# intel-aero/aero-optical-flow

Measured on AMD Instinct MI355X. Metric: frame-pairs/s (640x480, 8x8 SAD, +-4 search), higher is better.
Workload: dtype u8

## Files before the change

aero-optical-flow_amd/__init__.py:

```python
from __future__ import annotations

import ctypes as C
import os

import numpy as np

_HERE = os.path.dirname(os.path.abspath(__file__))
LIB_PATH = os.environ.get("AOF_LIB") or os.path.join(_HERE, "csrc", "libaof.so")

GRID_DENSE, GRID_PX4FLOW = 0, 1
SEARCH_EXHAUSTIVE, SEARCH_PRUNED, SEARCH_ADAPTIVE = 0, 1, 2
SAD_SKIPPED = 0xFFFF
FLAG_FLOW_VALID, FLAG_PRED_VALID = 1, 2
K_PYRAMID, K_SEARCH_L1, K_REDUCE_L1, K_SEARCH, K_REDUCE = range(5)

BLOCK_DTYPE = np.dtype([("dx", "i1"), ("dy", "i1"), ("sad", "<u2")])
FLOW_DTYPE = np.dtype([("flow_x", "<f4"), ("flow_y", "<f4"), ("count", "<u4"), ("quality", "u1"),
                       ("flags", "u1"), ("pred_x", "i1"), ("pred_y", "i1")])
assert BLOCK_DTYPE.itemsize == 4 and FLOW_DTYPE.itemsize == 16


class Params(C.Structure):
    _fields_ = [(n, C.c_int32) for n in (
        "width", "height", "tile", "search", "grid_mode", "num_blocks", "feature_threshold",
        "value_threshold", "subpixel", "hist_filter", "pyramid_levels", "mean_subtract",
        "min_valid")]

    def as_dict(self):
        return {n: getattr(self, n) for n, _ in self._fields_}


class IngestParams(C.Structure):
    _fields_ = [(n, C.c_int32) for n in ("camera_width", "camera_height", "crop_width", "crop_height")]


class DerotateParams(C.Structure):
    _fields_ = [(n, C.c_float) for n in ("focal_x", "focal_y", "max_flow", "rate_threshold")]


GYRO_DTYPE = np.dtype([("integ_x", "<f4"), ("integ_y", "<f4"), ("integ_z", "<f4"), ("dt_s", "<f4")])


class SequenceParams(C.Structure):
    _fields_ = [("ingest", IngestParams), ("focal_x", C.c_float), ("focal_y", C.c_float),
                ("output_rate", C.c_int32), ("offset_timestamp_usec", C.c_uint64),
                ("system_id", C.c_uint8), ("component_id", C.c_uint8), ("first_seq", C.c_uint8),
                ("derotate", C.c_uint8), ("derotate_params", DerotateParams)]


class SeqLayout(C.Structure):
    _fields_ = [(n, C.c_size_t) for n in ("total_bytes", "cropped", "exposure", "flows", "derotated", "count",
                                          "records", "frames", "frame_len", "scratch")]


SEQ_RECORD_DTYPE = np.dtype([("frame", "<u4"), ("quality", "<i4"), ("dt_us", "<i4"), ("flow_x", "<f4"),
                             ("flow_y", "<f4"), ("gyro_x", "<f4"), ("gyro_y", "<f4"), ("gyro_z", "<f4")])
SEQ_FRAME_BYTES = 56
SEQ_STATUS_STALLED = 1
assert SEQ_RECORD_DTYPE.itemsize == 32


class BankParams(C.Structure):
    _fields_ = [("n_streams", C.c_int32), ("frame_stride", C.c_int64), ("focal_x", C.c_float), ("focal_y", C.c_float),
                ("output_rate", C.c_int32), ("offset_timestamp_usec", C.c_uint64),
                ("system_id", C.c_uint8), ("component_id", C.c_uint8), ("first_seq", C.c_uint8)]


class BankStream(C.Structure):
    _fields_ = [("focal_x", C.c_float), ("focal_y", C.c_float), ("output_rate", C.c_int32),
                ("system_id", C.c_uint8), ("component_id", C.c_uint8), ("first_seq", C.c_uint8), ("reserved0", C.c_uint8),
                ("offset_timestamp_usec", C.c_uint64), ("reserved1", C.c_uint64)]


BANK_STREAM_DTYPE = np.dtype([("focal_x", "<f4"), ("focal_y", "<f4"), ("output_rate", "<i4"), ("system_id", "u1"),
                              ("component_id", "u1"), ("first_seq", "u1"), ("reserved0", "u1"),
                              ("offset_timestamp_usec", "<u8"), ("reserved1", "<u8")])
assert BANK_STREAM_DTYPE.itemsize == 32 and C.sizeof(BankStream) == 32


class BankSensor(C.Structure):
    _fields_ = [("offset", C.c_uint64), ("pitch", C.c_int32), ("width", C.c_int32), ("height", C.c_int32),
                ("x0", C.c_int32), ("y0", C.c_int32), ("reserved", C.c_uint32)]


BANK_SENSOR_DTYPE = np.dtype([("offset", "<u8"), ("pitch", "<i4"), ("width", "<i4"), ("height", "<i4"), ("x0", "<i4"),
                              ("y0", "<i4"), ("reserved", "<u4")])
assert BANK_SENSOR_DTYPE.itemsize == 32 and C.sizeof(BankSensor) == 32


class BankLayout(C.Structure):
    _fields_ = [(n, C.c_size_t) for n in ("total_bytes", "frames", "state", "scratch")]


class BankCamera(C.Structure):
    _fields_ = [("ingest", IngestParams), ("camera_stride", C.c_int64), ("exposure_interval_us", C.c_uint32),
                ("derotate", C.c_uint8), ("derotate_params", DerotateParams)]


class BankBurst(C.Structure):
    _fields_ = [("n_rounds", C.c_int32), ("round_stride", C.c_int64)]


BANK_BURST_MAX = 16
TICK_HELD, TICK_IDLE = -1, -2
BANK_BIN_MAX = 4
PIXEL_GREY8, PIXEL_LUMA16_LO, PIXEL_LUMA16_HI = 0, 1, 2
TICK_BAD_SENSOR = -5
TICK_DTYPE = np.dtype([("quality", "<i4"), ("dt_us", "<i4"), ("flow_x", "<f4"), ("flow_y", "<f4"),
                       ("gyro_x", "<f4"), ("gyro_y", "<f4"), ("gyro_z", "<f4"), ("frame", "<u4"), ("pixel", FLOW_DTYPE)])
BANK_STATE_BYTES = 64
EXPOSURE_DTYPE = np.dtype([("hist", "<u4", (10,)), ("msv", "<f4"), ("due", "<u4")])
assert TICK_DTYPE.itemsize == 48 and EXPOSURE_DTYPE.itemsize == 48


class ExposureControl(C.Structure):
    _fields_ = [(n, C.c_float) for n in ("msv_target", "exposure_p", "exposure_i", "exposure_d", "gain_p", "gain_i", "gain_d",
                                         "exposure_change_threshold", "exposure_max", "gain_change_threshold", "gain_max")]


EXPOSURE_UPDATED, EXPOSURE_SET_EXPOSURE, EXPOSURE_SET_GAIN = 1, 2, 4
EXPOSURE_STATE_DTYPE = np.dtype([("msv_error_old", "<f4"), ("msv_error_int", "<f4"), ("exposure", "<u2"), ("gain", "u1"),
                                 ("reserved", "u1"), ("updates", "<u4")])
EXPOSURE_COMMAND_DTYPE = np.dtype([("exposure", "<u2"), ("gain", "u1"), ("flags", "u1"), ("msv_error", "<f4"),
                                   ("msv_error_int", "<f4"), ("update", "<u4")])
assert EXPOSURE_STATE_DTYPE.itemsize == 16 and EXPOSURE_COMMAND_DTYPE.itemsize == 16


class ImuParams(C.Structure):
    _fields_ = [("n_streams", C.c_int32), ("n_rounds", C.c_int32), ("max_samples", C.c_int32),
                ("system_id", C.c_uint8), ("component_id", C.c_uint8), ("first_seq", C.c_uint8)]


IMU_SLOTS_MAX = 16
TICK_STALE_GYRO, TICK_NO_OFFSET = -3, -4
IMU_SAMPLE_DTYPE = np.dtype([("time_usec", "<u8"), ("xgyro", "<f4"), ("ygyro", "<f4"), ("zgyro", "<f4"),
                             ("reserved", "<u4")])
IMU_STATE_DTYPE = np.dtype([("gyro_x", "<f8"), ("gyro_y", "<f8"), ("gyro_z", "<f8"), ("prev_time_usec", "<u8"),
                            ("last_taken_time_usec", "<u8"), ("offset_timestamp_usec", "<u8"), ("messages", "<u4"),
                            ("samples_integrated", "<u4"), ("samples_rejected", "<u4"), ("dropped", "<u4")])
assert IMU_SAMPLE_DTYPE.itemsize == 24 and IMU_STATE_DTYPE.itemsize == 64


class MavlinkRxParams(C.Structure):
    _fields_ = [("n_streams", C.c_int32), ("n_rounds", C.c_int32), ("max_bytes", C.c_int32), ("max_samples", C.c_int32)]


MAVLINK_RX_BYTES_MAX = 4096
MAVLINK_RX_STATE_DTYPE = np.dtype([("bytes", "<u8"), ("frames", "<u4"), ("imu_samples", "<u4"), ("bad_check", "<u4"),
                                   ("overflowed", "<u4"), ("skipped", "<u4"), ("rejected_flags", "<u4"),
                                   ("in_progress", "u1", (96,))])
assert MAVLINK_RX_STATE_DTYPE.itemsize == 128


class OutboxLayout(C.Structure):
    _fields_ = [(n, C.c_size_t) for n in ("total_bytes", "messages", "exposures")]


OUTBOX_HEADER_DTYPE = np.dtype([("tag", "<u8"), ("n_messages", "<u4"), ("messages_found", "<u4"), ("n_exposures", "<u4"),
                                ("exposures_found", "<u4"), ("reserved", "u1", (40,))])
OUTBOX_ENTRY_DTYPE = np.dtype([("stream", "<u4"), ("round", "<u2"), ("mavlink_len", "u1"), ("reserved0", "u1"),
                               ("mavlink", "u1", (SEQ_FRAME_BYTES,)), ("record", TICK_DTYPE), ("derotated", "<f4", (2,)),
                               ("reserved1", "u1", (8,))])
OUTBOX_EXPOSURE_DTYPE = np.dtype([("stream", "<u4"), ("round", "<u2"), ("reserved0", "<u2"), ("exposure", EXPOSURE_DTYPE),
                                  ("reserved1", "u1", (8,))])
assert OUTBOX_HEADER_DTYPE.itemsize == 64 and OUTBOX_ENTRY_DTYPE.itemsize == 128 and OUTBOX_EXPOSURE_DTYPE.itemsize == 64


class WsLayout(C.Structure):
    _fields_ = [(n, C.c_size_t) for n in (
        "total_bytes", "sums", "l1_prev", "l1_cur", "l1_blocks", "l1_subdirs", "l1_flows",
        "l0_blocks", "l0_subdirs", "l0_hist", "l1_hist", "hints")]


class StreamStats(C.Structure):
    _fields_ = [("calls", C.c_uint64), ("resident_served", C.c_uint64), ("resident_launches", C.c_uint32),
                ("resident_fallbacks", C.c_uint32), ("resident_lost", C.c_uint32), ("tagged_slow", C.c_uint32),
                ("launch_call_us_max", C.c_float), ("start_latency_us_max", C.c_float),
                ("last_report", C.c_char * 320)]

    def as_dict(self):
        d = {n: getattr(self, n) for n, _ in self._fields_}
        d["last_report"] = d["last_report"].decode(errors="replace")
        return d


class SearchStats(C.Structure):
    _fields_ = [("pruned_launches", C.c_uint64), ("exhaustive_launches", C.c_uint64), ("reports_read", C.c_uint64),
                ("belief", C.c_int32), ("paying_pct", C.c_int32)]

    def as_dict(self):
        return {n: getattr(self, n) for n, _ in self._fields_}


class AofError(RuntimeError):
    def __init__(self, code, text):
        super().__init__(f"aof error {code}: {text}")
        self.code = code


def _load():
    if not os.path.exists(LIB_PATH):
        raise ImportError(
            f"{LIB_PATH} is missing: run `python -c 'import __graft_entry__ as g; g.build()'` "
            "(hipcc --offload-arch=gfx950). There is no CPU fallback.")
    try:
        import torch
    except Exception:
        pass
    lib = C.CDLL(LIB_PATH)
    P, VP, I64 = C.POINTER, C.c_void_p, C.c_int64
    sig = {
        "aof_version": (C.c_int, []),
        "aof_strerror": (C.c_char_p, [C.c_int]),
        "aof_params_default": (C.c_int, [P(Params), C.c_int, C.c_int]),
        "aof_params_px4flow": (C.c_int, [P(Params), C.c_int, C.c_int, C.c_int, C.c_int, C.c_int]),
        "aof_params_check": (C.c_int, [P(Params)]),
        "aof_grid": (C.c_int, [P(Params), C.c_int] + [P(C.c_int32)] * 6),
        "aof_workspace_layout": (C.c_int, [P(Params), I64, P(WsLayout)]),
        "aof_create": (C.c_int, [P(Params), C.c_int, P(VP)]),
        "aof_destroy": (None, [VP]),
        "aof_last_error": (C.c_char_p, [VP]),
        "aof_get_params": (C.c_int, [VP, P(Params)]),
        "aof_search_variant": (C.c_char_p, [VP]),
        "aof_set_force_generic": (C.c_int, [VP, C.c_int]),
        "aof_set_search_mode": (C.c_int, [VP, C.c_int]),
        "aof_get_search_mode": (C.c_int, [VP]),
        "aof_get_search_stats": (C.c_int, [VP, VP]),
        "aof_set_search_belief": (C.c_int, [VP, C.c_int]),
        "aof_set_split_coarse": (C.c_int, [VP, C.c_int]),
        "aof_set_reduce_fusion": (C.c_int, [VP, C.c_int]),
        "aof_flow_batch_device": (C.c_int, [VP, VP, VP, I64, I64, VP, VP, VP, VP, C.c_size_t, VP]),
        "aof_flow_pair_host": (C.c_int, [VP, VP, VP, VP, VP, VP]),
        "aof_stream_push_host": (C.c_int, [VP, VP, VP]),
        "aof_stream_reset": (C.c_int, [VP]),
        "aof_set_stream_graph": (C.c_int, [VP, C.c_int]),
        "aof_set_stream_resident": (C.c_int, [VP, C.c_int]),
        "aof_stream_get_stats": (C.c_int, [VP, P(StreamStats)]),
        "aof_debug_resident_fault": (C.c_int, [VP, C.c_int, C.c_uint32]),
        "aof_set_vote_deadline_us": (C.c_int, [VP, C.c_uint32]),
        "aof_debug_vote_deadline_ticks": (C.c_int, [VP, C.c_uint32]),
        "aof_debug_tile16_verdicts": (C.c_int, [VP, VP, C.c_int]),
        "aof_ingest_batch_device": (C.c_int, [P(IngestParams), VP, I64, I64, VP, I64, VP, VP]),
        "aof_sequence_layout": (C.c_int, [P(Params), P(SequenceParams), I64, P(SeqLayout)]),
        "aof_sequence_device": (C.c_int, [VP, P(SequenceParams), VP, I64, I64, VP, VP, VP, C.c_size_t, VP]),
        "aof_flow_angle": (C.c_float, [C.c_float, C.c_float]),
        "aof_bank_layout": (C.c_int, [P(Params), P(BankParams), P(BankLayout)]),
        "aof_bank_reset_device": (C.c_int, [VP, P(BankParams), VP, VP, C.c_size_t, VP]),
        "aof_bank_push_device": (C.c_int, [VP, P(BankParams), VP, VP, VP, VP, VP, C.c_size_t, VP, VP, VP, VP]),
        "aof_set_bank_path": (C.c_int, [VP, C.c_int]),
        "aof_bank_stream_from_params": (C.c_int, [P(BankParams), P(BankStream)]),
        "aof_set_bank_streams": (C.c_int, [VP, VP, C.c_int32]),
        "aof_set_bank_sensors": (C.c_int, [VP, VP, C.c_int32, C.c_uint64]),
        "aof_bank_sensor_from_camera": (C.c_int, [P(Params), P(BankCamera), C.c_int32, P(BankSensor)]),
        "aof_bank_sensor_centred": (C.c_int, [P(Params), C.c_uint64, C.c_int32, C.c_int32, C.c_int32, P(BankSensor)]),
        "aof_bank_sensor_valid": (C.c_int, [P(BankSensor), C.c_int32, C.c_int32, C.c_uint64, C.c_uint64]),
        "aof_ingest_sensors_device": (C.c_int, [C.c_int32, C.c_int32, VP, C.c_uint64, VP, I64, VP, I64, VP, VP, VP]),
        "aof_set_bank_pixel_formats": (C.c_int, [VP, VP, C.c_int32]),
        "aof_bank_sensor_valid_format": (C.c_int, [P(BankSensor), C.c_uint8, C.c_int32, C.c_int32, C.c_uint64, C.c_uint64]),
        "aof_ingest_sensor_formats_device": (C.c_int, [C.c_int32, C.c_int32, VP, C.c_uint64, VP, VP, I64, VP, I64, VP, VP, VP]),
        "aof_set_bank_binning": (C.c_int, [VP, VP, C.c_int32]),
        "aof_bank_sensor_valid_binned": (C.c_int, [P(BankSensor), C.c_uint8, C.c_uint8, C.c_int32, C.c_int32, C.c_uint64, C.c_uint64]),
        "aof_bank_sensor_centred_binned": (C.c_int, [P(Params), C.c_uint64, C.c_int32, C.c_int32, C.c_int32, C.c_uint8, C.c_uint8,
                                                     P(BankSensor)]),
        "aof_ingest_sensors_binned_device": (C.c_int, [C.c_int32, C.c_int32, VP, C.c_uint64, VP, VP, VP, I64, VP, I64, VP, VP, VP]),
        "aof_bank_camera_layout": (C.c_int, [P(Params), P(BankParams), P(BankCamera), P(BankLayout), P(C.c_size_t)]),
        "aof_bank_push_camera_device": (C.c_int, [VP, P(BankParams), P(BankCamera), VP, VP, VP, VP, VP, C.c_size_t, VP, VP, VP,
                                                  VP, VP, VP]),
        "aof_bank_push_burst_device": (C.c_int, [VP, P(BankParams), P(BankBurst), VP, VP, VP, VP, VP, C.c_size_t, VP, VP, VP, VP]),
        "aof_bank_push_camera_burst_device": (C.c_int, [VP, P(BankParams), P(BankCamera), P(BankBurst), VP, VP, VP, VP, VP,
                                                        C.c_size_t, VP, VP, VP, VP, VP, VP]),
        "aof_outbox_layout": (C.c_int, [C.c_uint32, C.c_uint32, P(OutboxLayout)]),
        "aof_bank_collect_device": (C.c_int, [VP, C.c_int32, C.c_int32, VP, VP, VP, VP, VP, C.c_uint32, C.c_uint32, VP,
                                              C.c_size_t, C.c_uint64, VP, VP]),
        "aof_outbox_alloc_host": (C.c_int, [C.c_size_t, P(VP)]),
        "aof_outbox_free_host": (C.c_int, [VP]),
        "aof_exposure_control_default": (C.c_int, [P(ExposureControl)]),
        "aof_bank_exposure_reset_device": (C.c_int, [VP, C.c_int32, VP, C.c_uint16, C.c_uint8, VP, VP, VP, VP]),
        "aof_bank_exposure_control_device": (C.c_int, [VP, P(ExposureControl), C.c_int32, C.c_int32, VP, VP, VP, VP]),
        "aof_exposure_control_host": (C.c_int, [P(ExposureControl), C.c_int32, C.c_int32, VP, VP, VP]),
        "aof_bank_imu_reset_device": (C.c_int, [VP, C.c_int32, VP, C.c_uint64, VP, VP]),
        "aof_bank_imu_device": (C.c_int, [VP, P(ImuParams), VP, VP, VP, VP, VP, VP, VP, VP, VP]),
        "aof_bank_imu_host": (C.c_int, [P(ImuParams), VP, VP, VP, VP, VP, VP, VP, VP]),
        "aof_bank_mavlink_rx_reset_device": (C.c_int, [VP, C.c_int32, VP, VP, VP]),
        "aof_bank_mavlink_rx_device": (C.c_int, [VP, P(MavlinkRxParams), VP, VP, VP, VP, VP, VP]),
        "aof_bank_mavlink_rx_host": (C.c_int, [P(MavlinkRxParams), VP, VP, VP, VP, VP]),
        "aof_derotate_batch_device": (C.c_int, [P(DerotateParams), VP, VP, I64, VP, VP]),
        "aof_exposure_msv": (C.c_float, [VP]),
        "aof_exposure_bin": (C.c_int, [C.c_int]),
        "aof_set_profiling": (C.c_int, [VP, C.c_int]),
        "aof_set_profiling_mask": (C.c_int, [VP, C.c_uint32]),
        "aof_kernel_ms": (C.c_int, [VP, C.c_int, P(C.c_float)]),
        "aof_profile_count": (C.c_int, [VP, C.c_int]),
        "aof_profile_ms": (C.c_int, [VP, C.c_int, C.c_int, P(C.c_float)]),
    }
    for name, (res, args) in sig.items():
        try:
            fn = getattr(lib, name)
        except AttributeError:
            if os.environ.get("AOF_LIB"):
                continue
            raise
        fn.restype, fn.argtypes = res, args
    return lib, tuple(sig)


lib, EXPORTS = _load()


def default_params(width, height, **overrides) -> Params:
    p = Params()
    lib.aof_params_default(C.byref(p), width, height)
    for k, v in overrides.items():
        if not hasattr(p, k):
            raise AttributeError(k)
        setattr(p, k, int(v))
    return p


def px4flow_params(width, height, search=4, feature_threshold=30, value_threshold=3000,
                   **overrides) -> Params:
    p = Params()
    lib.aof_params_px4flow(C.byref(p), width, height, search, feature_threshold, value_threshold)
    for k, v in overrides.items():
        setattr(p, k, int(v))
    return p


def check_params(p: Params) -> int:
    return lib.aof_params_check(C.byref(p))


def grid(p: Params, level=0):
    v = [C.c_int32() for _ in range(6)]
    rc = lib.aof_grid(C.byref(p), level, *[C.byref(x) for x in v])
    if rc:
        raise AofError(rc, lib.aof_strerror(rc).decode())
    return tuple(x.value for x in v)


def workspace_layout(p: Params, n_pairs: int) -> WsLayout:
    L = WsLayout()
    rc = lib.aof_workspace_layout(C.byref(p), n_pairs, C.byref(L))
    if rc:
        raise AofError(rc, lib.aof_strerror(rc).decode())
    return L


def algorithmic_bytes(p: Params) -> int:
    _, _, _, _, nx, ny = grid(p, 0)
    return 2 * p.width * p.height + 4 * nx * ny + 16


def abs_diffs(p: Params) -> int:
    _, _, _, _, nx, ny = grid(p, 0)
    return nx * ny * (2 * p.search + 1) ** 2 * p.tile ** 2


def ingest_batch(camera, crop_w, crop_h, cropped=None, hist=None, want_hist=True):
    import torch
    n, cam_h, cam_w = camera.shape
    p = IngestParams(cam_w, cam_h, crop_w, crop_h)
    if cropped is None:
        cropped = torch.empty((n, crop_h, crop_w), dtype=torch.uint8, device=camera.device)
    if hist is None and want_hist:
        hist = torch.empty((n, 10), dtype=torch.int32, device=camera.device)
    stream = torch.cuda.current_stream(camera.device).cuda_stream
    rc = lib.aof_ingest_batch_device(C.byref(p), camera.data_ptr(), camera.stride(0), n,
                                     cropped.data_ptr(), cropped.stride(0) if n else crop_w * crop_h,
                                     hist.data_ptr() if hist is not None else None, stream)
    if rc:
        raise AofError(rc, lib.aof_strerror(rc).decode())
    return cropped, hist


def derotate_batch(flows, gyro, focal_x, focal_y, max_flow, rate_threshold):
    import torch
    n = flows.shape[0]
    out = torch.empty((n, 2), dtype=torch.float32, device=flows.device)
    p = DerotateParams(focal_x, focal_y, max_flow, rate_threshold)
    rc = lib.aof_derotate_batch_device(C.byref(p), flows.data_ptr(), gyro.data_ptr(), n, out.data_ptr(),
                                       torch.cuda.current_stream(flows.device).cuda_stream)
    if rc:
        raise AofError(rc, lib.aof_strerror(rc).decode())
    return out


def flow_angle(flow_px: float, focal_px: float) -> float:
    return float(lib.aof_flow_angle(flow_px, focal_px))


def sequence_params(cam_w, cam_h, crop_w, crop_h, focal_x=216.6677, focal_y=216.2457, output_rate=15,
                    offset_timestamp_usec=0, system_id=1, component_id=100, first_seq=0, derotate=None) -> SequenceParams:
    sp = SequenceParams()
    sp.ingest = IngestParams(cam_w, cam_h, crop_w, crop_h)
    sp.focal_x, sp.focal_y, sp.output_rate = focal_x, focal_y, output_rate
    sp.offset_timestamp_usec = offset_timestamp_usec
    sp.system_id, sp.component_id, sp.first_seq = system_id, component_id, first_seq & 0xFF
    sp.derotate = 0 if derotate is None else 1
    if derotate is not None:
        sp.derotate_params = DerotateParams(focal_x, focal_y, derotate[0], derotate[1])
    return sp


def sequence_layout(p: Params, sp: SequenceParams, n_frames: int) -> SeqLayout:
    L = SeqLayout()
    rc = lib.aof_sequence_layout(C.byref(p), C.byref(sp), n_frames, C.byref(L))
    if rc:
        raise AofError(rc, lib.aof_strerror(rc).decode())
    return L


def bank_params(n_streams, focal_x=216.6677, focal_y=216.2457, output_rate=15, offset_timestamp_usec=0, system_id=1,
                component_id=100, first_seq=0, frame_stride=0) -> BankParams:
    bp = BankParams()
    bp.n_streams, bp.frame_stride = n_streams, frame_stride
    bp.focal_x, bp.focal_y, bp.output_rate = focal_x, focal_y, output_rate
    bp.offset_timestamp_usec = offset_timestamp_usec
    bp.system_id, bp.component_id, bp.first_seq = system_id, component_id, first_seq & 0xFF
    return bp


def bank_stream_from_params(bp: BankParams, n=None):
    rec = BankStream()
    rc = lib.aof_bank_stream_from_params(C.byref(bp), C.byref(rec))
    if rc:
        raise AofError(rc, lib.aof_strerror(rc).decode())
    one = np.frombuffer(bytes(rec), dtype=BANK_STREAM_DTYPE)[0]
    return one if n is None else np.full(int(n), one, dtype=BANK_STREAM_DTYPE)


def _sensor_record(rec: BankSensor):
    return np.frombuffer(bytes(rec), dtype=BANK_SENSOR_DTYPE)[0]


def bank_sensor_from_camera(p: Params, cam: BankCamera, stream=None, n=None):
    def one(s):
        rec = BankSensor()
        rc = lib.aof_bank_sensor_from_camera(C.byref(p), C.byref(cam), int(s), C.byref(rec))
        if rc:
            raise AofError(rc, lib.aof_strerror(rc).decode())
        return _sensor_record(rec)
    if n is None:
        return one(stream or 0)
    return np.array([one(s) for s in range(int(n))], dtype=BANK_SENSOR_DTYPE)


def bank_sensor_centred(p: Params, offset, pitch, width, height, format=0, bin=1):
    rec = BankSensor()
    if format == 0 and bin == 1:
        rc = lib.aof_bank_sensor_centred(C.byref(p), int(offset), int(pitch), int(width), int(height), C.byref(rec))
    else:
        rc = lib.aof_bank_sensor_centred_binned(C.byref(p), int(offset), int(pitch), int(width), int(height), int(format) & 0xFF,
                                                int(bin) & 0xFF, C.byref(rec))
    if rc:
        raise AofError(rc, lib.aof_strerror(rc).decode())
    return _sensor_record(rec)


def bank_sensor_valid(rec, crop_w, crop_h, camera_bytes, base=0, format=0, bin=1) -> bool:
    r = BankSensor.from_buffer_copy(np.asarray(rec, dtype=BANK_SENSOR_DTYPE).tobytes())
    if bin != 1:
        rc = lib.aof_bank_sensor_valid_binned(C.byref(r), int(format) & 0xFF, int(bin) & 0xFF, int(crop_w), int(crop_h), int(base),
                                              int(camera_bytes))
    elif format == 0:
        rc = lib.aof_bank_sensor_valid(C.byref(r), int(crop_w), int(crop_h), int(base), int(camera_bytes))
    else:
        rc = lib.aof_bank_sensor_valid_format(C.byref(r), int(format) & 0xFF, int(crop_w), int(crop_h), int(base), int(camera_bytes))
    if rc < 0:
        raise AofError(rc, lib.aof_strerror(rc).decode())
    return bool(rc)


def ingest_sensors(camera, sensors, crop_w, crop_h, camera_bytes=None, cropped=None, hist=None, ok=None, want_cropped=True,
                   want_hist=True, want_ok=True, formats=None, bins=None):
    import torch
    assert camera.dtype == torch.uint8 and sensors.dtype == torch.uint8 and sensors.is_contiguous() and sensors.numel() % 32 == 0
    n = sensors.numel() // 32
    assert formats is None or (formats.dtype == torch.uint8 and formats.is_contiguous() and formats.numel() == n)
    assert bins is None or (bins.dtype == torch.uint8 and bins.is_contiguous() and bins.numel() == n)
    dev = camera.device
    if cropped is None and want_cropped:
        cropped = torch.empty((n, crop_h, crop_w), dtype=torch.uint8, device=dev)
    if hist is None and want_hist:
        hist = torch.empty((n, 10), dtype=torch.int32, device=dev)
    if ok is None and want_ok:
        ok = torch.empty((n,), dtype=torch.uint8, device=dev)
    opt = lambda t: t.data_ptr() if t is not None else None
    tail = (n, opt(cropped), cropped.stride(0) if cropped is not None and n else crop_w * crop_h, opt(hist), opt(ok),
            torch.cuda.current_stream(dev).cuda_stream)
    head = (int(crop_w), int(crop_h), camera.data_ptr(), camera.numel() if camera_bytes is None else int(camera_bytes), sensors.data_ptr())
    if bins is not None:
        rc = lib.aof_ingest_sensors_binned_device(*head, opt(formats), bins.data_ptr(), *tail)
    elif formats is None:
        rc = lib.aof_ingest_sensors_device(*head, *tail)
    else:
        rc = lib.aof_ingest_sensor_formats_device(*head, formats.data_ptr(), *tail)
    if rc:
        raise AofError(rc, lib.aof_strerror(rc).decode())
    return cropped, hist, ok


def bank_layout(p: Params, bp: BankParams) -> BankLayout:
    L = BankLayout()
    rc = lib.aof_bank_layout(C.byref(p), C.byref(bp), C.byref(L))
    if rc:
        raise AofError(rc, lib.aof_strerror(rc).decode())
    return L


def bank_camera_params(cam_w, cam_h, crop_w, crop_h, camera_stride=0, exposure_interval_us=200000, derotate=None,
                       focal_x=216.6677, focal_y=216.2457) -> BankCamera:
    cam = BankCamera()
    cam.ingest = IngestParams(cam_w, cam_h, crop_w, crop_h)
    cam.camera_stride, cam.exposure_interval_us = camera_stride, exposure_interval_us
    cam.derotate = 0 if derotate is None else 1
    if derotate is not None:
        cam.derotate_params = DerotateParams(focal_x, focal_y, derotate[0], derotate[1])
    return cam


def bank_burst_params(n_rounds, round_stride=0) -> BankBurst:
    b = BankBurst()
    b.n_rounds, b.round_stride = int(n_rounds), int(round_stride)
    return b


def bank_camera_layout(p: Params, bp: BankParams, cam: BankCamera):
    L, staging = BankLayout(), C.c_size_t()
    rc = lib.aof_bank_camera_layout(C.byref(p), C.byref(bp), C.byref(cam), C.byref(L), C.byref(staging))
    if rc:
        raise AofError(rc, lib.aof_strerror(rc).decode())
    return L, staging.value


def outbox_layout(capacity_messages, capacity_exposures=0) -> OutboxLayout:
    L = OutboxLayout()
    rc = lib.aof_outbox_layout(capacity_messages, capacity_exposures, C.byref(L))
    if rc:
        raise AofError(rc, lib.aof_strerror(rc).decode())
    return L


def outbox_view(buffer, capacity_messages=None, capacity_exposures=0):
    if isinstance(buffer, HostOutbox):
        capacity_messages, capacity_exposures, a = buffer.capacity_messages, buffer.capacity_exposures, buffer.array
    else:
        a = buffer.cpu().numpy() if hasattr(buffer, "cpu") else np.asarray(buffer)
        a = np.ascontiguousarray(a).reshape(-1).view(np.uint8)
    if capacity_messages is None:
        capacity_messages = (a.size - 64 - 64 * capacity_exposures) // 128
    L = outbox_layout(capacity_messages, capacity_exposures)
    assert a.size >= L.total_bytes, (a.size, L.total_bytes)
    header = a[:64].view(OUTBOX_HEADER_DTYPE).reshape(())
    messages = a[L.messages:L.messages + 128 * capacity_messages].view(OUTBOX_ENTRY_DTYPE)[:int(header["n_messages"])]
    exposures = a[L.exposures:L.exposures + 64 * capacity_exposures].view(OUTBOX_EXPOSURE_DTYPE)[:int(header["n_exposures"])]
    return header, messages, exposures


class HostOutbox:

    def __init__(self, capacity_messages, capacity_exposures=0):
        self.capacity_messages, self.capacity_exposures = int(capacity_messages), int(capacity_exposures)
        self.layout = outbox_layout(self.capacity_messages, self.capacity_exposures)
        self.nbytes = self.layout.total_bytes
        p = C.c_void_p()
        rc = lib.aof_outbox_alloc_host(self.nbytes, C.byref(p))
        if rc:
            raise AofError(rc, "aof_outbox_alloc_host failed")
        self.ptr = p.value
        self.array = np.frombuffer((C.c_uint8 * self.nbytes).from_address(self.ptr), dtype=np.uint8)
        self._tag = self.array[:8].view("<u8")

    @property
    def tag(self) -> int:
        return int(self._tag[0])

    def wait(self, tag, timeout_s=2.0) -> bool:
        import time
        deadline = time.perf_counter() + timeout_s
        tagword, tag = self._tag, int(tag)
        while int(tagword[0]) != tag:
            if time.perf_counter() > deadline:
                return False
        return True

    def close(self):
        if getattr(self, "ptr", None) and lib is not None:
            self.array = self._tag = None
            lib.aof_outbox_free_host(self.ptr)
            self.ptr = None

    __del__ = close


def exposure_control_default() -> ExposureControl:
    ec = ExposureControl()
    rc = lib.aof_exposure_control_default(C.byref(ec))
    if rc:
        raise AofError(rc, lib.aof_strerror(rc).decode())
    return ec


def exposure_control_host(records, states, ec: ExposureControl = None):
    ec = exposure_control_default() if ec is None else ec
    records = np.ascontiguousarray(records, dtype=EXPOSURE_DTYPE)
    assert records.ndim in (1, 2)
    K, S = (1, records.shape[0]) if records.ndim == 1 else records.shape
    assert states.dtype == EXPOSURE_STATE_DTYPE and states.shape == (S,) and states.flags.c_contiguous and states.flags.writeable
    commands = np.empty(records.shape, EXPOSURE_COMMAND_DTYPE)
    rc = lib.aof_exposure_control_host(C.byref(ec), S, K, records.ctypes.data, states.ctypes.data, commands.ctypes.data)
    if rc:
        raise AofError(rc, lib.aof_strerror(rc).decode())
    return commands


def imu_params(n_streams, n_rounds, max_samples, system_id=1, component_id=100, first_seq=0) -> ImuParams:
    ip = ImuParams()
    ip.n_streams, ip.n_rounds, ip.max_samples = int(n_streams), int(n_rounds), int(max_samples)
    ip.system_id, ip.component_id, ip.first_seq = int(system_id), int(component_id), int(first_seq)
    return ip


def bank_imu_host(samples, counts, times, records, states, system_id=1, component_id=100, first_seq=0, mavlink=True,
                  records_out=None, fill=0):
    samples = np.ascontiguousarray(samples, dtype=IMU_SAMPLE_DTYPE)
    K, M, S = samples.shape
    times = np.ascontiguousarray(times, dtype=np.uint64)
    assert records.dtype == TICK_DTYPE and records.shape == (K, S) and records.flags.c_contiguous and times.shape == (K, S)
    assert states.dtype == IMU_STATE_DTYPE and states.shape == (S,) and states.flags.c_contiguous and states.flags.writeable
    if counts is not None:
        counts = np.ascontiguousarray(counts, dtype=np.uint8)
        assert counts.shape == (K, S)
    if records_out is None:
        records_out = np.empty((K, S), TICK_DTYPE)
    assert records_out.dtype == TICK_DTYPE and records_out.shape == (K, S) and records_out.flags.c_contiguous
    frames = np.full((K, S, SEQ_FRAME_BYTES), fill, np.uint8) if mavlink else None
    lengths = np.full((K, S), fill, np.uint8) if mavlink else None
    ip = imu_params(S, K, M, system_id, component_id, first_seq)
    rc = lib.aof_bank_imu_host(C.byref(ip), samples.ctypes.data, counts.ctypes.data if counts is not None else None,
                               times.ctypes.data, records.ctypes.data, states.ctypes.data, records_out.ctypes.data,
                               frames.ctypes.data if mavlink else None, lengths.ctypes.data if mavlink else None)
    if rc:
        raise AofError(rc, lib.aof_strerror(rc).decode())
    return records_out, frames, lengths


def imu_states_view(t) -> np.ndarray:
    a = t.cpu().numpy() if hasattr(t, "cpu") else np.asarray(t)
    return np.ascontiguousarray(a).view(IMU_STATE_DTYPE).reshape(a.shape[:-1])


def mavlink_rx_params(n_streams, n_rounds, max_bytes, max_samples) -> MavlinkRxParams:
    rp = MavlinkRxParams()
    rp.n_streams, rp.n_rounds, rp.max_bytes, rp.max_samples = int(n_streams), int(n_rounds), int(max_bytes), int(max_samples)
    return rp


def _aligned_copy(a, align=16):
    raw = np.empty(a.size + align, np.uint8)
    off = -raw.ctypes.data % align
    out = raw[off:off + a.size].reshape(a.shape)
    out[...] = a
    return out


def bank_mavlink_rx_host(data, lengths, states, max_samples, samples=None, counts=None):
    data = np.ascontiguousarray(data, dtype=np.uint8)
    K, S, B = data.shape
    M = int(max_samples)
    if data.ctypes.data % 16:
        data = _aligned_copy(data)
    if lengths is not None:
        lengths = np.ascontiguousarray(lengths, dtype=np.uint16)
        assert lengths.shape == (K, S)
    assert states.dtype == MAVLINK_RX_STATE_DTYPE and states.shape == (S,) and states.flags.c_contiguous and states.flags.writeable
    if samples is None:
        samples = np.zeros((K, M, S), IMU_SAMPLE_DTYPE)
    if counts is None:
        counts = np.zeros((K, S), np.uint8)
    assert samples.dtype == IMU_SAMPLE_DTYPE and samples.shape == (K, M, S) and samples.flags.c_contiguous
    assert counts.dtype == np.uint8 and counts.shape == (K, S) and counts.flags.c_contiguous
    rp = mavlink_rx_params(S, K, B, M)
    rc = lib.aof_bank_mavlink_rx_host(C.byref(rp), data.ctypes.data, lengths.ctypes.data if lengths is not None else None,
                                      states.ctypes.data, samples.ctypes.data, counts.ctypes.data)
    if rc:
        raise AofError(rc, lib.aof_strerror(rc).decode())
    return samples, counts


def mavlink_rx_states_view(t) -> np.ndarray:
    a = t.cpu().numpy() if hasattr(t, "cpu") else np.asarray(t)
    return np.ascontiguousarray(a).view(MAVLINK_RX_STATE_DTYPE).reshape(a.shape[:-1])


def exposure_states_view(t) -> np.ndarray:
    a = t.cpu().numpy() if hasattr(t, "cpu") else np.asarray(t)
    return np.ascontiguousarray(a).view(EXPOSURE_STATE_DTYPE).reshape(a.shape[:-1])


def exposure_commands_view(t) -> np.ndarray:
    a = t.cpu().numpy() if hasattr(t, "cpu") else np.asarray(t)
    return np.ascontiguousarray(a).view(EXPOSURE_COMMAND_DTYPE).reshape(a.shape[:-1])


def exposure_view(t) -> np.ndarray:
    a = t.cpu().numpy() if hasattr(t, "cpu") else np.asarray(t)
    return np.ascontiguousarray(a).view(EXPOSURE_DTYPE).reshape(a.shape[0])


def ticks_view(t) -> np.ndarray:
    a = t.cpu().numpy() if hasattr(t, "cpu") else np.asarray(t)
    return np.ascontiguousarray(a).view(TICK_DTYPE).reshape(a.shape[0])


class Bank:

    def __init__(self, bp: BankParams, layout: BankLayout, buffer, camera: BankCamera = None, staging: int = None):
        self.bp, self.layout, self.buffer = bp, layout, buffer
        self.camera, self.staging = camera, staging

    @property
    def n_streams(self) -> int:
        return self.bp.n_streams

    def frames_bytes(self) -> np.ndarray:
        return self.buffer[self.layout.frames:self.layout.state].cpu().numpy()

    def state_bytes(self) -> np.ndarray:
        L = self.layout
        return self.buffer[L.state:L.state + BANK_STATE_BYTES * self.n_streams].cpu().numpy().reshape(self.n_streams, BANK_STATE_BYTES)


def exposure_msv(hist) -> float:
    h = np.ascontiguousarray(np.asarray(hist), dtype=np.uint32)
    assert h.shape == (10,)
    return float(lib.aof_exposure_msv(h.ctypes.data))


class FlowEngine:

    def __init__(self, params: Params, device: int = 0):
        self._ctx = C.c_void_p()
        rc = lib.aof_create(C.byref(params), device, C.byref(self._ctx))
        if rc:
            self._ctx = None
            raise AofError(rc, lib.aof_strerror(rc).decode())
        self.params = params
        self.device = device
        self._ws = None

    def close(self):
        if getattr(self, "_ctx", None) and lib is not None:
            lib.aof_destroy(self._ctx)
            self._ctx = None

    __del__ = close

    def _check(self, rc):
        if rc < 0:
            raise AofError(rc, lib.aof_last_error(self._ctx).decode())
        return rc

    @property
    def variant(self) -> str:
        return lib.aof_search_variant(self._ctx).decode()

    def force_generic(self, on=True):
        self._check(lib.aof_set_force_generic(self._ctx, int(on)))

    def set_search_mode(self, mode):
        self._check(lib.aof_set_search_mode(self._ctx, int(mode)))

    @property
    def search_mode(self) -> int:
        return lib.aof_get_search_mode(self._ctx)

    def search_stats(self) -> dict:
        st = SearchStats()
        self._check(lib.aof_get_search_stats(self._ctx, C.byref(st)))
        return st.as_dict()

    def set_search_belief(self, belief):
        self._check(lib.aof_set_search_belief(self._ctx, int(belief)))

    def set_split_coarse(self, on=True):
        self._check(lib.aof_set_split_coarse(self._ctx, int(on)))

    def set_reduce_fusion(self, on=True):
        if not hasattr(lib, "aof_set_reduce_fusion"):
            return
        self._check(lib.aof_set_reduce_fusion(self._ctx, int(on)))

    def set_profiling(self, on=True, kernels=None):
        if on and kernels is not None:
            mask = 0
            for k in kernels:
                mask |= 1 << k
            self._check(lib.aof_set_profiling_mask(self._ctx, mask))
        else:
            self._check(lib.aof_set_profiling(self._ctx, int(on)))

    def kernel_ms(self, kernel_id) -> float:
        ms = C.c_float()
        self._check(lib.aof_kernel_ms(self._ctx, kernel_id, C.byref(ms)))
        return ms.value

    def profile_ms(self, kernel_id):
        n = self._check(lib.aof_profile_count(self._ctx, kernel_id))
        out = []
        ms = C.c_float()
        for i in range(n):
            self._check(lib.aof_profile_ms(self._ctx, kernel_id, i, C.byref(ms)))
            out.append(ms.value)
        return out

    def grid(self, level=0):
        return grid(self.params, level)

    def nblocks(self, level=0):
        g = self.grid(level)
        return g[4] * g[5]

    def flow_batch(self, prev, cur, blocks=None, subdirs=None, flows=None, workspace=None,
                   pair_stride=None, n_pairs=None):
        import torch
        p = self.params
        if n_pairs is None:
            n_pairs = prev.shape[0]
        if pair_stride is None:
            pair_stride = prev.stride(0) if prev.dim() == 3 else p.width * p.height
        dev = prev.device
        nb = self.nblocks(0)
        if blocks is None:
            blocks = torch.empty((n_pairs, nb), dtype=torch.int32, device=dev)
        if flows is None:
            flows = torch.empty((n_pairs, 16), dtype=torch.uint8, device=dev)
        if subdirs is None and p.subpixel:
            subdirs = torch.empty((n_pairs, nb), dtype=torch.uint8, device=dev)
        L = workspace_layout(p, n_pairs)
        if workspace is None:
            if self._ws is None or self._ws.numel() < L.total_bytes or self._ws.device != dev:
                self._ws = torch.empty(L.total_bytes, dtype=torch.uint8, device=dev)
            workspace = self._ws
        stream = torch.cuda.current_stream(dev).cuda_stream
        self._check(lib.aof_flow_batch_device(
            self._ctx, prev.data_ptr(), cur.data_ptr(), pair_stride, n_pairs, blocks.data_ptr(),
            subdirs.data_ptr() if subdirs is not None else None, flows.data_ptr(),
            workspace.data_ptr(), workspace.numel(), stream))
        return blocks, flows, workspace

    def bind_batch(self, prev, cur, blocks, flows, workspace, subdirs=None, stream=None):
        import torch
        p = self.params
        n_pairs = prev.shape[0]
        stride = prev.stride(0) if prev.dim() == 3 else p.width * p.height
        assert workspace.numel() >= workspace_layout(p, n_pairs).total_bytes
        args = (self._ctx, prev.data_ptr(), cur.data_ptr(), stride, n_pairs, blocks.data_ptr(),
                subdirs.data_ptr() if subdirs is not None else None, flows.data_ptr(),
                workspace.data_ptr(), workspace.numel())
        keep = (prev, cur, blocks, flows, workspace, subdirs)
        fn, dev, current_stream = lib.aof_flow_batch_device, prev.device, torch.cuda.current_stream

        if stream is not None:
            def enqueue():
                rc = fn(*args, stream)
                if rc < 0:
                    self._check(rc)
        else:
            def enqueue():
                rc = fn(*args, current_stream(dev).cuda_stream)
                if rc < 0:
                    self._check(rc)
        enqueue.keep = keep
        return enqueue

    def sequence(self, sp: SequenceParams, camera, time_us, gyro=None, workspace=None):
        import torch
        n = camera.shape[0]
        L = sequence_layout(self.params, sp, n)
        if workspace is None:
            workspace = torch.empty(L.total_bytes, dtype=torch.uint8, device=camera.device)
        assert time_us.dtype == torch.int64 and time_us.numel() == n
        stream = torch.cuda.current_stream(camera.device).cuda_stream
        self._check(lib.aof_sequence_device(self._ctx, C.byref(sp), camera.data_ptr(), camera.stride(0) if n else 0, n,
                                            time_us.data_ptr(), gyro.data_ptr() if gyro is not None else None,
                                            workspace.data_ptr(), workspace.numel(), stream))
        return workspace, L

    def sequence_outputs(self, sp: SequenceParams, workspace, L: SeqLayout, n: int):
        p = self.params
        ws = workspace.cpu().numpy()
        pairs = max(n - 1, 0)
        count = ws[L.count:L.count + 16].view(np.uint32)
        out = {
            "records": ws[L.records:L.records + 32 * int(count[0])].view(SEQ_RECORD_DTYPE),
            "frames_sent": int(count[1]), "status": int(count[2]),
            "cropped": ws[L.cropped:L.cropped + n * p.width * p.height].reshape(n, p.height, p.width),
            "exposure": ws[L.exposure:L.exposure + 40 * n].view(np.uint32).reshape(n, 10),
            "flows": ws[L.flows:L.flows + 16 * pairs].view(FLOW_DTYPE),
            "derotated": ws[L.derotated:L.derotated + 8 * pairs].view(np.float32).reshape(pairs, 2) if sp.derotate else None,
        }
        lens = ws[L.frame_len:L.frame_len + int(count[0])]
        out["mavlink"] = [bytes(ws[L.frames + SEQ_FRAME_BYTES * m:L.frames + SEQ_FRAME_BYTES * m + int(lens[m])])
                          for m in range(int(count[0]))]
        return out

    def bank_create(self, bp: BankParams, device=None, camera: BankCamera = None) -> "Bank":
        import torch
        staging = None
        if camera is None:
            L = bank_layout(self.params, bp)
        else:
            L, staging = bank_camera_layout(self.params, bp, camera)
        dev = torch.device("cuda", self.device) if device is None else device
        bank = Bank(bp, L, torch.zeros(L.total_bytes, dtype=torch.uint8, device=dev), camera, staging)
        self.bank_reset(bank)
        return bank

    def bank_reset(self, bank: "Bank", mask=None):
        import torch
        buf = bank.buffer
        assert mask is None or (mask.dtype == torch.uint8 and mask.numel() == bank.n_streams and mask.is_contiguous())
        self._check(lib.aof_bank_reset_device(self._ctx, C.byref(bank.bp), mask.data_ptr() if mask is not None else None,
                                              buf.data_ptr(), buf.numel(), torch.cuda.current_stream(buf.device).cuda_stream))

    def _bank_push(self, bank, src, times, select, gyro, mavlink, records, out_frames, out_lengths, n_rounds=None,
                   round_stride=0, camera=False, exposure=None, derotated=None, want_exposure=True):
        import torch
        S, buf, cam = bank.n_streams, bank.buffer, bank.camera
        burst = n_rounds is not None
        lead = (int(n_rounds), S) if burst else (S,)
        n = int(n_rounds) * S if burst else S
        dev = buf.device
        if camera:
            assert cam is not None, "bank_create(..., camera=...) makes a bank for sensor frames"
        assert src.dtype == torch.uint8 and (camera or src.is_contiguous())
        assert times.dtype == torch.int64 and times.numel() == n and (not burst or times.is_contiguous())
        if burst:
            assert select is None or (select.dtype == torch.uint8 and select.numel() == S)
            assert gyro is None or gyro.numel() == n * 4
        if records is None:
            records = torch.empty(lead + (48,), dtype=torch.uint8, device=dev)
        if camera and exposure is None and want_exposure:
            exposure = torch.empty(lead + (48,), dtype=torch.uint8, device=dev)
        if camera and derotated is None and cam.derotate:
            derotated = torch.empty(lead + (2,), dtype=torch.float32, device=dev)
        if mavlink:
            if out_frames is None:
                out_frames = torch.zeros(lead + (SEQ_FRAME_BYTES,), dtype=torch.uint8, device=dev)
            if out_lengths is None:
                out_lengths = torch.zeros(lead, dtype=torch.uint8, device=dev)
        else:
            out_frames = out_lengths = None
        opt = lambda t: t.data_ptr() if t is not None else None
        fn = getattr(lib, "aof_bank_push" + ("_camera" if camera else "") + ("_burst" if burst else "") + "_device")
        args = [self._ctx, C.byref(bank.bp)]
        if camera:
            args.append(C.byref(cam))
        if burst:
            args.append(C.byref(bank_burst_params(int(n_rounds), round_stride)))
        args += [src.data_ptr(), times.data_ptr(), opt(select), opt(gyro), buf.data_ptr(), buf.numel(), records.data_ptr()]
        if camera:
            args += [opt(exposure), opt(derotated)]
        self._check(fn(*args, opt(out_frames), opt(out_lengths), torch.cuda.current_stream(dev).cuda_stream))
        return dict(records=records, exposure=exposure, derotated=derotated, frames=out_frames, lengths=out_lengths)

    def bank_push(self, bank: "Bank", frames, times, active=None, gyro=None, mavlink=False, records=None, out_frames=None,
                  out_lengths=None):
        out = self._bank_push(bank, frames, times, active, gyro, mavlink, records, out_frames, out_lengths)
        return (out["records"], out["frames"], out["lengths"]) if mavlink else out["records"]

    def bank_push_camera(self, bank: "Bank", camera, times, active=None, gyro=None, mavlink=False, records=None,
                         exposure=None, derotated=None, out_frames=None, out_lengths=None, want_exposure=True):
        return self._bank_push(bank, camera, times, active, gyro, mavlink, records, out_frames, out_lengths, camera=True,
                               exposure=exposure, derotated=derotated, want_exposure=want_exposure)

    def bank_push_burst(self, bank: "Bank", n_rounds, frames, times, count=None, gyro=None, mavlink=False, records=None,
                        out_frames=None, out_lengths=None, round_stride=0):
        out = self._bank_push(bank, frames, times, count, gyro, mavlink, records, out_frames, out_lengths, n_rounds, round_stride)
        return (out["records"], out["frames"], out["lengths"]) if mavlink else out["records"]

    def bank_push_camera_burst(self, bank: "Bank", n_rounds, camera, times, count=None, gyro=None, mavlink=False,
                               records=None, exposure=None, derotated=None, out_frames=None, out_lengths=None,
                               want_exposure=True, round_stride=0):
        return self._bank_push(bank, camera, times, count, gyro, mavlink, records, out_frames, out_lengths, n_rounds,
                               round_stride, camera=True, exposure=exposure, derotated=derotated, want_exposure=want_exposure)

    def bank_collect(self, records, mavlink=None, lengths=None, exposure=None, derotated=None, capacity_messages=None,
                     capacity_exposures=0, outbox=None, tag=1, tag_tensor=None):
        import torch
        dev = records.device
        assert records.dtype == torch.uint8 and records.is_contiguous() and records.shape[-1] == 48 and records.dim() in (2, 3)
        K, S = (1, records.shape[0]) if records.dim() == 2 else (records.shape[0], records.shape[1])
        n = K * S
        assert mavlink is None or (mavlink.is_contiguous() and mavlink.numel() == n * SEQ_FRAME_BYTES)
        assert lengths is None or (lengths.is_contiguous() and lengths.numel() == n)
        assert exposure is None or (exposure.is_contiguous() and exposure.numel() == n * 48)
        assert derotated is None or (derotated.is_contiguous() and derotated.numel() * derotated.element_size() == n * 8)
        assert tag_tensor is None or (tag_tensor.dtype == torch.int64 and tag_tensor.numel() == 1)
        if capacity_messages is None:
            capacity_messages = outbox.capacity_messages if isinstance(outbox, HostOutbox) else n
        if outbox is None:
            outbox = torch.empty(outbox_layout(capacity_messages, capacity_exposures).total_bytes, dtype=torch.uint8, device=dev)
        ptr, size = (outbox.ptr, outbox.nbytes) if isinstance(outbox, HostOutbox) else (outbox.data_ptr(), outbox.numel())
        opt = lambda t: t.data_ptr() if t is not None else None
        self._check(lib.aof_bank_collect_device(
            self._ctx, S, K, records.data_ptr(), opt(mavlink), opt(lengths), opt(exposure), opt(derotated),
            capacity_messages, capacity_exposures, ptr, size, int(tag), opt(tag_tensor), torch.cuda.current_stream(dev).cuda_stream))
        return outbox

    def bank_exposure_reset(self, state, mask=None, exposure0=1, gain0=1, exposures=None, gains=None):
        import torch
        S = state.numel() // 16
        assert state.dtype == torch.uint8 and state.is_contiguous() and state.numel() == 16 * S
        assert mask is None or (mask.dtype == torch.uint8 and mask.numel() == S and mask.is_contiguous())
        assert exposures is None or (exposures.element_size() == 2 and exposures.numel() == S and exposures.is_contiguous())
        assert gains is None or (gains.dtype == torch.uint8 and gains.numel() == S and gains.is_contiguous())
        opt = lambda t: t.data_ptr() if t is not None else None
        self._check(lib.aof_bank_exposure_reset_device(self._ctx, S, opt(mask), int(exposure0), int(gain0), opt(exposures),
                                                       opt(gains), state.data_ptr(), torch.cuda.current_stream(state.device).cuda_stream))

    def bank_exposure_control(self, exposure, state, commands=None, ec: ExposureControl = None):
        import torch
        dev = exposure.device
        assert exposure.dtype == torch.uint8 and exposure.is_contiguous() and exposure.shape[-1] == 48 and exposure.dim() in (2, 3)
        K, S = (1, exposure.shape[0]) if exposure.dim() == 2 else (exposure.shape[0], exposure.shape[1])
        assert state.dtype == torch.uint8 and state.is_contiguous() and state.numel() == 16 * S
        if commands is None:
            commands = torch.empty(tuple(exposure.shape[:-1]) + (16,), dtype=torch.uint8, device=dev)
        if isinstance(commands, np.ndarray):
            assert commands.dtype == np.uint8 and commands.size == 16 * K * S and commands.flags.c_contiguous
            ptr = commands.ctypes.data
        else:
            assert commands.dtype == torch.uint8 and commands.is_contiguous() and commands.numel() == 16 * K * S
            ptr = commands.data_ptr()
        ec = exposure_control_default() if ec is None else ec
        self._check(lib.aof_bank_exposure_control_device(self._ctx, C.byref(ec), S, K, exposure.data_ptr(), state.data_ptr(), ptr,
                                                         torch.cuda.current_stream(dev).cuda_stream))
        return commands

    def bank_imu_reset(self, state, mask=None, offset0=0):
        import torch
        S = state.numel() // 64
        assert state.dtype == torch.uint8 and state.is_contiguous() and state.numel() == 64 * S
        assert mask is None or (mask.dtype == torch.uint8 and mask.numel() == S and mask.is_contiguous())
        self._check(lib.aof_bank_imu_reset_device(self._ctx, S, mask.data_ptr() if mask is not None else None, int(offset0),
                                                  state.data_ptr(), torch.cuda.current_stream(state.device).cuda_stream))

    def bank_imu(self, samples, times, records, state, counts=None, mavlink=True, records_out=None, out_frames=None,
                 out_lengths=None, system_id=1, component_id=100, first_seq=0):
        import torch
        dev = records.device
        assert records.dtype == torch.uint8 and records.is_contiguous() and records.shape[-1] == 48 and records.dim() in (2, 3)
        K, S = (1, records.shape[0]) if records.dim() == 2 else (records.shape[0], records.shape[1])
        lead = tuple(records.shape[:-1])
        assert samples.dtype == torch.uint8 and samples.is_contiguous() and samples.shape[-1] == 24 and samples.numel() % (24 * K * S) == 0
        M = samples.numel() // (24 * K * S)
        assert times.dtype == torch.int64 and times.is_contiguous() and times.numel() == K * S
        assert state.dtype == torch.uint8 and state.is_contiguous() and state.numel() == 64 * S
        assert counts is None or (counts.dtype == torch.uint8 and counts.is_contiguous() and counts.numel() == K * S)
        if records_out is None:
            records_out = torch.empty_like(records)
        assert records_out.dtype == torch.uint8 and records_out.is_contiguous() and records_out.shape == records.shape
        ptr = lambda t: None if t is None else t.ctypes.data if isinstance(t, np.ndarray) else t.data_ptr()
        if mavlink:
            if out_frames is None:
                out_frames = torch.zeros(lead + (SEQ_FRAME_BYTES,), dtype=torch.uint8, device=dev)
            if out_lengths is None:
                out_lengths = torch.zeros(lead, dtype=torch.uint8, device=dev)
            for t, n in ((out_frames, K * S * SEQ_FRAME_BYTES), (out_lengths, K * S)):
                if isinstance(t, np.ndarray):
                    assert t.dtype == np.uint8 and t.size == n and t.flags.c_contiguous
                else:
                    assert t.dtype == torch.uint8 and t.is_contiguous() and t.numel() == n
        else:
            out_frames = out_lengths = None
        ip = imu_params(S, K, M, system_id, component_id, first_seq)
        self._check(lib.aof_bank_imu_device(self._ctx, C.byref(ip), samples.data_ptr(), ptr(counts), times.data_ptr(),
                                            records.data_ptr(), state.data_ptr(), records_out.data_ptr(), ptr(out_frames),
                                            ptr(out_lengths), torch.cuda.current_stream(dev).cuda_stream))
        return records_out, out_frames, out_lengths

    def bank_mavlink_rx_reset(self, state, mask=None):
        import torch
        S = state.numel() // 128
        assert state.dtype == torch.uint8 and state.is_contiguous() and state.numel() == 128 * S
        assert mask is None or (mask.dtype == torch.uint8 and mask.numel() == S and mask.is_contiguous())
        self._check(lib.aof_bank_mavlink_rx_reset_device(self._ctx, S, mask.data_ptr() if mask is not None else None,
                                                         state.data_ptr(), torch.cuda.current_stream(state.device).cuda_stream))

    def bank_mavlink_rx(self, data, state, max_samples, lengths=None, samples=None, counts=None):
        import torch
        dev = data.device
        assert data.dtype == torch.uint8 and data.is_contiguous() and data.dim() in (2, 3)
        K, S, B = (1,) + tuple(data.shape) if data.dim() == 2 else tuple(data.shape)
# ... 388 lines not shown
```

aero-optical-flow_amd/csrc/aof_batch.cpp:

```cpp
#include <cerrno>

#include "aof_ctx.hpp"

using namespace aof;

namespace {

struct Timed {
    aof_ctx *ctx; int id; hipStream_t s; bool on; int slot;
    Timed(aof_ctx *c, int k, hipStream_t st)
        : ctx(c), id(k), s(st), on(c->prof.on && !c->capturing && ((c->prof.mask >> k) & 1u)),
          slot((int)(c->prof.count[k] % AOF_PROFILE_RING))
    {
        if (on) (void)hipEventRecord(ctx->prof.ev[id][slot][0], s);
    }
    ~Timed() { if (on) { (void)hipEventRecord(ctx->prof.ev[id][slot][1], s); ctx->prof.count[id]++; } }
};

struct BatchView {
    const uint8_t *prev, *cur;
    int64_t stride;
    uint32_t *sums;
    uint8_t *l1_prev, *l1_cur;
    aof_block *blocks1; uint8_t *subdirs1; aof_flow *flows1; uint8_t *hist1;
    aof_block *blocks0; uint8_t *subdirs0; aof_flow *flows; uint8_t *hist0;
    uint32_t *hints;
};

enum SearchKind { SK_TILE16, SK_LANE8_GROUP, SK_LANE8, SK_GENERIC };
enum CoarseKind { COARSE_NONE, COARSE_FUSED, COARSE_K1 };

struct LevelPlan {
    SearchKind kind;
    bool refine;
    SearchArgs a;
    FlowTail tail;
};

struct BatchPlan {
    bool small;
    bool small_class;
    SmallArgs sm;
    CoarseKind coarse;
    bool k1_pass;
    bool sequence;
    CoarseArgs fused;
    PyramidArgs k1;
    LevelPlan level[2];
};

BatchView batch_view(const aof_ctx *ctx, const aof_ws_layout &L, const uint8_t *d_prev, const uint8_t *d_cur,
                     int64_t pair_stride, aof_block *d_blocks, uint8_t *d_subdirs, aof_flow *d_flows, void *d_workspace)
{
    const aof_params &p = ctx->params;
    BatchView v;
    uint8_t *ws = static_cast<uint8_t *>(d_workspace);
    const bool two = p.pyramid_levels == 2, eq = p.mean_subtract != 0;
    v.prev = d_prev; v.cur = d_cur; v.stride = pair_stride;
    v.sums = eq ? reinterpret_cast<uint32_t *>(ws + L.sums) : nullptr;
    v.l1_prev = two ? ws + L.l1_prev : nullptr;
    v.l1_cur = two ? ws + L.l1_cur : nullptr;
    v.blocks1 = reinterpret_cast<aof_block *>(ws + L.l1_blocks);
    v.subdirs1 = p.subpixel ? ws + L.l1_subdirs : nullptr;
    v.flows1 = reinterpret_cast<aof_flow *>(ws + L.l1_flows);
    v.hist1 = ws + L.l1_hist;
    v.blocks0 = d_blocks ? d_blocks : reinterpret_cast<aof_block *>(ws + L.l0_blocks);
    v.subdirs0 = nullptr;
    if (p.subpixel) v.subdirs0 = d_subdirs ? d_subdirs : ws + L.l0_subdirs;
    v.flows = d_flows;
    v.hist0 = ws + L.l0_hist;
    v.hints = p.tile == 16 ? reinterpret_cast<uint32_t *>(ws + L.hints) : nullptr;
    return v;
}

SearchArgs search_args(const aof_ctx *ctx, int level, const uint8_t *prev, const uint8_t *cur, int64_t stride,
                       aof_block *blocks, uint8_t *subdirs, const aof_flow *pred, const uint32_t *sums, int64_t n)
{
    const aof_params &p = ctx->params;
    SearchArgs a;
    a.prev = prev; a.cur = cur; a.pair_stride = stride;
    a.w = p.width >> level; a.h = p.height >> level;
    a.tile = p.tile; a.search = p.search;
    a.grid = level ? ctx->g1 : ctx->g0;
    a.feature_threshold = p.feature_threshold;
    a.value_threshold = value_threshold_u16(p);
    a.subpixel = p.subpixel;
    a.blocks = blocks; a.subdirs = p.subpixel ? subdirs : nullptr;
    a.pred = pred; a.sums = sums; a.level = level; a.n_pairs = n;
    a.hist_range = level_range(p, level);
    a.prune = ctx->search_mode;
    a.hints = nullptr;
    return a;
}

SearchKind search_kind(const aof_ctx *ctx, SearchArgs *a)
{
    if (ctx->force_generic) return SK_GENERIC;
    if (tile16_supported(*a)) return SK_TILE16;
    SearchArgs x = *a;
    x.prune = 0;
    if (a->prune && tile16_supported(x)) {
        a->prune = 0;
        return SK_TILE16;
    }
    if (lane8_supported(*a)) return lane8_group(*a) > 0 ? SK_LANE8_GROUP : SK_LANE8;
    return SK_GENERIC;
}

constexpr int64_t kSmallMaxPairs = 128;

FlowTail flow_tail(const aof_ctx *ctx, int level, aof_flow *flows, const aof_flow *pred)
{
    const aof_params &p = ctx->params;
    FlowTail t;
    t.nblocks = (level ? ctx->g1 : ctx->g0).blocks(); t.range = level_range(p, level);
    t.hist_filter = p.hist_filter; t.min_valid = p.min_valid;
    t.flows = flows; t.pred = pred; t.emit_predictor = level ? 1 : 0;
    return t;
}

LevelPlan plan_level(const aof_ctx *ctx, SearchArgs a, const FlowTail &tail)
{
    const SearchKind kind = search_kind(ctx, &a);
    return {kind, kind == SK_TILE16 && a.subpixel && !tile16_refines(a), a, tail};
}

BatchPlan plan_batch(const aof_ctx *ctx, const BatchView &v, int64_t n, bool k1_ready)
{
    const aof_params &p = ctx->params;
    const bool two = p.pyramid_levels == 2, eq = p.mean_subtract != 0;
    const int64_t frame = (int64_t)p.width * p.height, l1_frame = (int64_t)(p.width / 2) * (p.height / 2);
    BatchPlan P = {};
    const SmallArgs &sm = P.sm = {search_args(ctx, 0, v.prev, v.cur, v.stride, v.blocks0, v.subdirs0, nullptr, v.sums, n),
                                  search_args(ctx, 1, v.l1_prev, v.l1_cur, l1_frame, v.blocks1, v.subdirs1, nullptr, v.sums, n),
                                  flow_tail(ctx, 0, v.flows, two ? v.flows1 : nullptr), flow_tail(ctx, 1, v.flows1, nullptr),
                                  v.sums, two ? 2 : 1};
    SearchArgs a0 = sm.l0;
    a0.pred = sm.t0.pred;
    a0.hints = v.hints;
    P.level[0] = plan_level(ctx, a0, sm.t0);

    P.small_class = !ctx->force_generic && !ctx->split_coarse && P.level[0].kind == SK_LANE8_GROUP &&
                    (!two || plan_level(ctx, sm.l1, sm.t1).kind == SK_LANE8_GROUP) && flow_small_supported(sm);
    P.small = P.small_class && n <= kSmallMaxPairs;
    if (P.small || (!two && !eq)) return P;

    CoarseArgs &c = P.fused;
    c.prev = v.prev; c.cur = v.cur; c.pair_stride = v.stride;
    c.w = p.width; c.h = p.height; c.tile = p.tile; c.search = p.search; c.subpixel = p.subpixel;
    c.grid = ctx->g1;
    c.feature_threshold = p.feature_threshold;
    c.value_threshold = value_threshold_u16(p);
    c.sums = v.sums; c.blocks = v.blocks1; c.tail = sm.t1; c.n_pairs = n;
    c.first_generation = ctx->cus; c.stagger_groups = 0; c.stagger_ticks = 0;
    if (two && !ctx->force_generic && !ctx->split_coarse && coarse_fused_supported(P.fused)) {
        P.coarse = COARSE_FUSED;
        return P;
    }
    P.coarse = COARSE_K1;
    const bool seq = P.sequence = v.cur - v.prev == frame && v.stride == frame && v.l1_cur >= v.l1_prev;
    P.k1 = {v.prev, seq ? nullptr : v.cur, v.stride, p.width, p.height, v.l1_prev, seq ? nullptr : v.l1_cur, v.sums,
            seq ? n + 1 : n, seq ? 1 : 0};
    P.k1_pass = !(P.sequence && k1_ready);
    if (two) {
        SearchArgs a1 = sm.l1;
        if (P.sequence) a1.cur = v.l1_prev + l1_frame;
        a1.hints = v.hints;
        P.level[1] = plan_level(ctx, a1, sm.t1);
    }
    return P;
}


constexpr uint32_t kPayingPct = 40;
constexpr int kProbeEvery = 16;

bool adaptive_lane8_prunes(AdaptiveSearch &st, const SearchArgs &a)
{
    if (a.level != 0 || !st.slots || lane8_chunks(a) < kPruneMinChunks) return false;
    if (st.expected) {
        const uint32_t tag = st.launch_no & 0xFFFFu;
        uint32_t arrived = 0, paying = 0, seen = 0;
        for (uint32_t i = 0; i < st.expected && i < (uint32_t)kPruneSlots; i++) {
            const uint32_t w = __atomic_load_n(st.slots + i, __ATOMIC_RELAXED);
            if ((w >> 16) != tag) continue;
            arrived++;
            paying += (w >> 8) & 0xFFu;
            seen += w & 0xFFu;
        }
        if (arrived * 4 >= st.expected && seen) {
            st.stats.paying_pct = (int32_t)(paying * 100u / seen);
            st.belief = paying * 100u >= seen * kPayingPct ? 1 : 0;
            st.stats.belief = st.belief;
            st.stats.reports_read++;
        }
    }
    if (st.belief != 0) return true;
    if (++st.since_probe >= kProbeEvery) {
        st.since_probe = 0;
        return true;
    }
    return false;
}

enum Capture { CAPTURE_NONE, CAPTURE_ACTIVE, CAPTURE_UNKNOWN };

struct Lane8Launch {
    int prune;
    bool cols;
    bool fused;
    PruneReport rep;
};

VoteMem vote_mem(const aof_ctx *ctx) { return {ctx->votes.mem, kVoteStride, ctx->h_fault, ctx->votes.deadline_ticks}; }

Lane8Launch choose_lane8(aof_ctx *ctx, const SearchArgs &a, Capture cap)
{
    Lane8Launch l = {a.prune, false, false, {nullptr, 0, 1, 0}};
    if (l.prune && ctx->search_mode == AOF_SEARCH_ADAPTIVE) {
        AdaptiveSearch &st = ctx->adapt;
        if (!adaptive_lane8_prunes(st, a)) {
            l.prune = 0;
            st.stats.exhaustive_launches++;
        } else {
            l.prune = st.belief == 1 ? 1 : 2;
            if (++st.launch_no % 0x10000u == 0) st.launch_no++;
            l.rep.slots = st.slots;
            l.rep.launch_no = st.launch_no & 0xFFFFu;
            st.stats.pruned_launches++;
        }
    }
    SearchArgs x = a;
    x.prune = l.prune;
    l.cols = l.prune && lane8_cols_supported(x);
    const VoteMem vm = vote_mem(ctx);
    const bool fits = l.cols ? lane8_cols_votes_supported(x, vm, ctx->votes.pairs)
                             : (!l.prune && lane8_votes_supported(x, vm, ctx->votes.pairs));
    l.fused = fits && !ctx->votes.separate && (cap == CAPTURE_ACTIVE || (cap == CAPTURE_NONE && !ctx->votes.captured));
    return l;
}

int launch_lane8(aof_ctx *ctx, SearchArgs a, const FlowTail &tail, hipStream_t s, bool *reduced)
{
    hipStreamCaptureStatus status = hipStreamCaptureStatusNone;
    const Capture cap = hipStreamIsCapturing(s, &status) != hipSuccess ? CAPTURE_UNKNOWN
                        : status == hipStreamCaptureStatusNone         ? CAPTURE_NONE
                                                                       : CAPTURE_ACTIVE;
    Lane8Launch l = choose_lane8(ctx, a, cap);
    a.prune = l.prune;
    const bool eager = cap == CAPTURE_NONE;
    if (l.fused && eager && ctx->votes.used && ctx->votes.stream != s && hipStreamWaitEvent(s, ctx->votes.done, 0) != hipSuccess)
        return fail(ctx, -EIO, "cannot order the launch behind the context's previous one");
    const VoteMem vm = vote_mem(ctx);
    const FlowTail *t = l.fused ? &tail : nullptr;
    const VoteMem *m = l.fused ? &vm : nullptr;
    PruneReport *rep = l.prune ? &l.rep : nullptr;
    int rc = l.cols ? launch_search_lane8_cols(a, s, rep, t, m) : launch_search_lane8(a, s, t, m, rep);
    if (!rc && l.fused && eager) {
        rc = (int)hipEventRecord(ctx->votes.done, s);
        ctx->votes.stream = s;
        ctx->votes.used = true;
    } else if (!rc && l.fused) {
        ctx->votes.captured = true;
    }
    *reduced = l.fused;
    if (rep && l.rep.slots) ctx->adapt.expected = l.rep.expected;
    return rc;
}


int enqueue_level(aof_ctx *ctx, const LevelPlan &l, uint8_t *hist, int kid_search, int kid_reduce, hipStream_t s)
{
    bool reduced = l.kind == SK_LANE8_GROUP;
    {
        Timed t(ctx, kid_search, s);
        int rc;
        switch (l.kind) {
        case SK_TILE16:
            rc = launch_search_tile16(l.a, s, ctx->tile16_verdicts);
            if (!rc && l.refine) rc = launch_refine(l.a, s);
            break;
        case SK_LANE8_GROUP:
            rc = launch_flow_lane8(l.a, l.tail, s);
            break;
        case SK_LANE8:
            rc = launch_lane8(ctx, l.a, l.tail, s, &reduced);
            if (rc < 0) return rc;
            break;
        default:
            rc = launch_search_generic(l.a, s);
        }
        if (rc) return fail(ctx, -EIO, "search launch: %s", hipGetErrorString((hipError_t)rc));
    }
    if (reduced) return 0;
    const ReduceArgs r = {l.a.blocks, l.a.subdirs, value_threshold_u16(ctx->params), l.tail, l.a.n_pairs, nullptr, 0,
                          reinterpret_cast<uint32_t *>(hist)};
    Timed t(ctx, kid_reduce, s);
    const int rc = launch_reduce(r, s);
    if (rc) return fail(ctx, -EIO, "reduce launch: %s", hipGetErrorString((hipError_t)rc));
    return 0;
}

int flow_batch(aof_ctx *ctx, const uint8_t *d_prev, const uint8_t *d_cur, int64_t pair_stride, int64_t n_pairs,
               aof_block *d_blocks, uint8_t *d_subdirs, aof_flow *d_flows, void *d_workspace, size_t workspace_bytes,
               void *stream, bool k1_ready)
{
    if (!ctx) return -EINVAL;
    if (n_pairs < 0 || (n_pairs > 0 && (!d_prev || !d_cur || !d_flows)))
        return fail(ctx, -EINVAL, "null frame or flow pointer");
    if (int sticky = sticky_error(ctx)) return sticky;
    if (n_pairs == 0) return 0;
    const aof_params &p = ctx->params;
    if (pair_stride < (int64_t)p.width * p.height && n_pairs > 1)
        return fail(ctx, -EINVAL, "pair_stride smaller than a frame");
    aof_ws_layout L;
    int rc = aof_workspace_layout(&p, n_pairs, &L);
    if (rc) return fail(ctx, rc, "bad workspace layout");
    if (!d_workspace || workspace_bytes < L.total_bytes)
        return fail(ctx, -ENOSPC, "workspace %zu B < required %zu B", workspace_bytes, L.total_bytes);
    if (!aligned(d_workspace, 256))
        return fail(ctx, -EINVAL, "workspace must be 256-byte aligned");
    if (!aligned(d_blocks, 4) || !aligned(d_flows, 4))
        return fail(ctx, -EINVAL, "block and flow records must be 4-byte aligned");
    if ((rc = device_check(ctx))) return rc;
    const BatchView v = batch_view(ctx, L, d_prev, d_cur, pair_stride, d_blocks, d_subdirs, d_flows, d_workspace);
    const BatchPlan P = plan_batch(ctx, v, n_pairs, k1_ready);
    const hipStream_t s = static_cast<hipStream_t>(stream);
    if (P.small) {
        Timed t(ctx, AOF_K_SEARCH, s);
        if ((rc = launch_flow_small(P.sm, s))) return fail(ctx, -EIO, "small-pair launch: %s", hipGetErrorString((hipError_t)rc));
        return 0;
    }
    if (P.coarse == COARSE_FUSED) {
        Timed t(ctx, AOF_K_PYRAMID, s);
        if ((rc = launch_coarse_fused(P.fused, s))) return fail(ctx, -EIO, "coarse launch: %s", hipGetErrorString((hipError_t)rc));
    }
    if (P.k1_pass) {
        Timed t(ctx, AOF_K_PYRAMID, s);
        if ((rc = launch_pyramid(P.k1, s))) return fail(ctx, -EIO, "pyramid launch: %s", hipGetErrorString((hipError_t)rc));
    }
    if (P.coarse == COARSE_K1 && p.pyramid_levels == 2 && (rc = enqueue_level(ctx, P.level[1], v.hist1, AOF_K_SEARCH_L1, AOF_K_REDUCE_L1, s))) return rc;
    return enqueue_level(ctx, P.level[0], v.hist0, AOF_K_SEARCH, AOF_K_REDUCE, s);
}

}

namespace aof {

bool plan_small_pair(const aof_ctx *ctx, const uint8_t *prev, const uint8_t *cur, aof_flow *flow, SmallArgs *sm)
{
    const aof_params &p = ctx->params;
    aof_ws_layout L;
    aof_workspace_layout(&p, 1, &L);
    const BatchView v = batch_view(ctx, L, prev, cur, (int64_t)p.width * p.height, ctx->host.d_blocks, ctx->host.d_subdirs,
                                   flow, ctx->host.d_ws);
    const BatchPlan P = plan_batch(ctx, v, 1, false);
    *sm = P.sm;
    return P.small;
}

bool plan_small_batch(const aof_ctx *ctx, const uint8_t *prev, const uint8_t *cur, int64_t stride, int64_t n, aof_flow *flows,
                      void *d_workspace, SmallArgs *sm)
{
    aof_ws_layout L;
    if (n < 1 || aof_workspace_layout(&ctx->params, n, &L)) return false;
    const BatchView v = batch_view(ctx, L, prev, cur, stride, nullptr, nullptr, flows, d_workspace);
    const BatchPlan P = plan_batch(ctx, v, n, false);
    *sm = P.sm;
    return P.small_class;
}

int bank_path(const aof_ctx *ctx) { return ctx->bank_path; }
void set_bank_path(aof_ctx *ctx, int path) { ctx->bank_path = path; }
const aof_bank_stream *bank_streams(const aof_ctx *ctx, int32_t *n_streams)
{
    *n_streams = ctx->bank_streams_n;
    return ctx->bank_streams;
}
void set_bank_streams(aof_ctx *ctx, const aof_bank_stream *d_streams, int32_t n_streams)
{
    ctx->bank_streams = d_streams;
    ctx->bank_streams_n = d_streams ? n_streams : 0;
}
const aof_bank_sensor *bank_sensors(const aof_ctx *ctx, int32_t *n_streams, uint64_t *camera_bytes)
{
    *n_streams = ctx->bank_sensors_n;
    *camera_bytes = ctx->bank_camera_bytes;
    return ctx->bank_sensors;
}
void set_bank_sensors(aof_ctx *ctx, const aof_bank_sensor *d_sensors, int32_t n_streams, uint64_t camera_bytes)
{
    ctx->bank_sensors = d_sensors;
    ctx->bank_sensors_n = d_sensors ? n_streams : 0;
    ctx->bank_camera_bytes = d_sensors ? camera_bytes : 0;
}
const uint8_t *bank_pixel_formats(const aof_ctx *ctx, int32_t *n_streams)
{
    *n_streams = ctx->bank_formats_n;
    return ctx->bank_formats;
}
void set_bank_pixel_formats(aof_ctx *ctx, const uint8_t *d_formats, int32_t n_streams)
{
    ctx->bank_formats = d_formats;
    ctx->bank_formats_n = d_formats ? n_streams : 0;
}
const uint8_t *bank_binning(const aof_ctx *ctx, int32_t *n_streams)
{
    *n_streams = ctx->bank_bins_n;
    return ctx->bank_bins;
}
void set_bank_binning(aof_ctx *ctx, const uint8_t *d_bins, int32_t n_streams)
{
    ctx->bank_bins = d_bins;
    ctx->bank_bins_n = d_bins ? n_streams : 0;
}

bool sequence_runs_k1(aof_ctx *ctx, const uint8_t *d_frames, int64_t n_pairs, void *d_workspace)
{
    const aof_params &p = ctx->params;
    aof_ws_layout L;
    if (n_pairs < 1 || aof_workspace_layout(&p, n_pairs, &L)) return false;
    const int64_t frame = (int64_t)p.width * p.height;
    const BatchView v = batch_view(ctx, L, d_frames, d_frames + frame, frame, nullptr, nullptr, nullptr, d_workspace);
    return plan_batch(ctx, v, n_pairs, false).k1_pass;
}

int flow_sequence(aof_ctx *ctx, const uint8_t *d_frames, int64_t n_pairs, aof_flow *d_flows, void *d_workspace,
                  size_t workspace_bytes, void *stream, bool k1_ready)
{
    const int64_t frame = (int64_t)ctx->params.width * ctx->params.height;
    return flow_batch(ctx, d_frames, d_frames + frame, frame, n_pairs, nullptr, nullptr, d_flows, d_workspace,
                      workspace_bytes, stream, k1_ready);
}

}

extern "C" {

int aof_flow_batch_device(aof_ctx *ctx, const uint8_t *d_prev, const uint8_t *d_cur, int64_t pair_stride, int64_t n_pairs,
                          aof_block *d_blocks, uint8_t *d_subdirs, aof_flow *d_flows, void *d_workspace,
                          size_t workspace_bytes, void *stream)
{
    return flow_batch(ctx, d_prev, d_cur, pair_stride, n_pairs, d_blocks, d_subdirs, d_flows, d_workspace,
                      workspace_bytes, stream, false);
}

const char *aof_search_variant(const aof_ctx *ctx)
{
    if (!ctx) return "";
    BatchView v = {};
    v.stride = (int64_t)ctx->params.width * ctx->params.height;
    switch (plan_batch(ctx, v, 1, false).level[0].kind) {
    case SK_TILE16: return "tile16_lds";
    case SK_GENERIC: return "generic";
    default: return "lane8";
    }
}

}
```

aero-optical-flow_amd/csrc/aof_capi.hip:

```cpp
#include <cerrno>
#include <cstdarg>
#include <cstdio>
#include <cstring>
#include <new>
#include <thread>

#include "aof_ctx.hpp"

using namespace aof;

namespace aof {

int fail(aof_ctx *ctx, int code, const char *fmt, ...)
{
    if (ctx) {
        va_list ap;
        va_start(ap, fmt);
        vsnprintf(ctx->err, sizeof(ctx->err), fmt, ap);
        va_end(ap);
    }
    return code;
}

double seconds_since(std::chrono::steady_clock::time_point t0)
{
    return std::chrono::duration<double>(std::chrono::steady_clock::now() - t0).count();
}

template <class Query>
hipError_t wait_bounded(Query query, double seconds)
{
    const auto t0 = std::chrono::steady_clock::now();
    for (;;) {
        const hipError_t e = query();
        if (e != hipErrorNotReady) return e;
        const double t = seconds_since(t0);
        if (t > seconds) return hipErrorNotReady;
        if (t > 200e-6) std::this_thread::sleep_for(std::chrono::microseconds(t > 5e-3 ? 500 : 20));
    }
}

hipError_t drain_bounded(hipStream_t s, double seconds) { return wait_bounded([s] { return hipStreamQuery(s); }, seconds); }

int wedge(aof_ctx *ctx, const char *what, hipError_t e)
{
    const char *why = e == hipErrorNotReady ? "the device did not finish within the time limit" : hipGetErrorString(e);
    ctx->wedged = true;
    std::fprintf(stderr, "aof: %s: %s -- the context is disabled\n", what, why);
    return fail(ctx, e == hipErrorNotReady ? -ETIMEDOUT : -EIO, "%s: %s", what, why);
}

int sticky_error(aof_ctx *ctx)
{
    if (ctx->wedged) return -EIO;
    if (ctx->h_fault) {
        const uint32_t code = __atomic_load_n(ctx->h_fault, __ATOMIC_ACQUIRE);
        if (code)
            return fail(ctx, -EIO, "a reduction inside a search launch gave up waiting for the votes of pair %u of its "
                                   "launch (device-side deadline): that record carries quality 0 and no valid flag; "
                                   "the context's vote memory is no longer trusted -- create a new context", code - 1);
    }
    return 0;
}

int device_check(aof_ctx *ctx)
{
    int cur_dev = -1;
    if (hipGetDevice(&cur_dev) != hipSuccess || cur_dev != ctx->device)
        return fail(ctx, -EINVAL, "context was created for device %d but the calling thread's current "
                                  "device is %d", ctx->device, cur_dev);
    return 0;
}

int precheck(aof_ctx *ctx)
{
    if (int sticky = sticky_error(ctx)) return sticky;
    return device_check(ctx);
}

int ctx_fail(aof_ctx *ctx, int code, const char *what) { return fail(ctx, code, "%s", what); }

}

namespace {

void kernel_choice_changes(aof_ctx *ctx, bool changes)
{
    { DeviceGuard guard(ctx->device); (void)resident_stop(ctx); }
    if (changes) drop_push_graphs(ctx);
}

}

extern "C" {

int aof_create(const aof_params *p, int device, aof_ctx **out)
{
    if (!out) return -EINVAL;
    *out = nullptr;
    int rc = aof_params_check(p);
    if (rc) return rc;
    int ndev = 0;
    if (hipGetDeviceCount(&ndev) != hipSuccess || device < 0 || device >= ndev) return -ENODEV;
    hipDeviceProp_t prop;
    if (hipGetDeviceProperties(&prop, device) != hipSuccess) return -ENODEV;
    if (std::strncmp(prop.gcnArchName, "gfx950", 6) != 0) return -ENODEV;

    aof_ctx *ctx = new (std::nothrow) aof_ctx();
    if (!ctx) return -ENOMEM;
    ctx->params = *p;
    ctx->device = device;
    ctx->cus = prop.multiProcessorCount > 0 ? prop.multiProcessorCount : 256;
    grid_for_level(*p, 0, &ctx->g0);
    if (p->pyramid_levels == 2) grid_for_level(*p, 1, &ctx->g1);
    std::snprintf(ctx->err, sizeof(ctx->err), "ok");
    if (p->tile == 8 && p->search == 4) {
        DeviceGuard guard(device);
        const size_t bytes = (size_t)kVotePairs * kVoteStride * sizeof(uint32_t);
        if (hipMalloc((void **)&ctx->votes.mem, bytes) != hipSuccess || hipMemset(ctx->votes.mem, 0, bytes) != hipSuccess ||
            hipEventCreateWithFlags(&ctx->votes.done, hipEventDisableTiming) != hipSuccess ||
            hipHostMalloc((void **)&ctx->h_fault, 64 + kPruneSlots * sizeof(uint32_t), hipHostMallocMapped | hipHostMallocCoherent) != hipSuccess ||
            hipDeviceSynchronize() != hipSuccess) {
            aof_destroy(ctx);
            return -EIO;
        }
        std::memset(ctx->h_fault, 0, 64 + kPruneSlots * sizeof(uint32_t));
        ctx->adapt.slots = ctx->h_fault + 16;
        ctx->votes.pairs = kVotePairs;
    }
    {
        DeviceGuard guard(device);
        if (hipMalloc((void **)&ctx->outbox_counter, sizeof(OutboxCounter)) != hipSuccess ||
            hipMemset(ctx->outbox_counter, 0, sizeof(OutboxCounter)) != hipSuccess || hipDeviceSynchronize() != hipSuccess) {
            aof_destroy(ctx);
            return -EIO;
        }
    }
    ctx->votes.deadline_ticks = kVoteDeadlineTicks;
    ctx->res.stop_wait_s = 1.0;
    ctx->votes.separate = true;
    ctx->search_mode = AOF_SEARCH_ADAPTIVE;
    ctx->adapt.belief = -1;
    ctx->adapt.stats.belief = -1;

    *out = ctx;
    return 0;
}

void aof_destroy(aof_ctx *ctx)
{
    if (!ctx) return;
    DeviceGuard guard(ctx->device);
    (void)resident_stop(ctx);
    bool leak = ctx->res.lost || ctx->wedged;
    hipError_t e = hipSuccess;
    if (!leak && ctx->host.stream && (e = drain_bounded(ctx->host.stream, kDrainS)) != hipSuccess) leak = true;
    if (!leak && ctx->votes.done && ctx->votes.used && (e = wait_bounded([ctx] { return hipEventQuery(ctx->votes.done); }, kDrainS)) != hipSuccess)
        leak = true;
    if (ctx->prof.ev) {
        for (hipEvent_t *ev = *ctx->prof.ev[0], *end = ev + AOF_K_COUNT * AOF_PROFILE_RING * 2; ev != end; ev++)
            if (*ev) (void)hipEventDestroy(*ev);
        delete[] ctx->prof.ev;
    }
    if (leak) {
        std::fprintf(stderr, "aof: destroying a context whose device work has not drained (%s): its device memory, pinned "
                             "memory and streams are leaked, not freed\n",
                     ctx->res.lost ? "resident kernel lost" : ctx->wedged ? ctx->err : hipGetErrorString(e));
        delete ctx;
        return;
    }
    free_host_state(ctx);
    if (ctx->res.k.stream) (void)hipStreamDestroy(ctx->res.k.stream);
    if (ctx->res.k.box) (void)hipHostFree(ctx->res.k.box);
    if (ctx->votes.done) (void)hipEventDestroy(ctx->votes.done);
    if (ctx->votes.mem) (void)hipFree(ctx->votes.mem);
    if (ctx->outbox_counter) (void)hipFree(ctx->outbox_counter);
    if (ctx->h_fault) (void)hipHostFree(ctx->h_fault);
    delete ctx;
}

const char *aof_last_error(const aof_ctx *ctx) { return ctx ? ctx->err : "null context"; }

int aof_get_search_mode(const aof_ctx *ctx) { return ctx ? ctx->search_mode : -EINVAL; }

int aof_get_search_stats(const aof_ctx *ctx, aof_search_stats *out)
{
    if (!ctx || !out) return -EINVAL;
    *out = ctx->adapt.stats;
    return 0;
}

int aof_set_search_belief(aof_ctx *ctx, int belief)
{
    if (!ctx || belief < -1 || belief > 1) return -EINVAL;
    ctx->adapt.belief = belief;
    ctx->adapt.stats.belief = belief;
    ctx->adapt.since_probe = 0;
    ctx->adapt.expected = 0;
    return 0;
}

int aof_get_params(const aof_ctx *ctx, aof_params *out)
{
    if (!ctx || !out) return -EINVAL;
    *out = ctx->params;
    return 0;
}

int aof_set_force_generic(aof_ctx *ctx, int on)
{
    if (!ctx) return -EINVAL;
    kernel_choice_changes(ctx, (on != 0) != ctx->force_generic);
    ctx->force_generic = on != 0;
    return 0;
}

int aof_set_search_mode(aof_ctx *ctx, int mode)
{
    if (!ctx || mode < AOF_SEARCH_EXHAUSTIVE || mode > AOF_SEARCH_ADAPTIVE) return -EINVAL;
    kernel_choice_changes(ctx, mode != ctx->search_mode);
    ctx->search_mode = mode;
    return 0;
}

int aof_set_split_coarse(aof_ctx *ctx, int on)
{
    if (!ctx) return -EINVAL;
    kernel_choice_changes(ctx, (on != 0) != ctx->split_coarse);
    ctx->split_coarse = on != 0;
    return 0;
}

int aof_set_reduce_fusion(aof_ctx *ctx, int on)
{
    if (!ctx) return -EINVAL;
    ctx->votes.separate = on == 0;
    return 0;
}

int aof_set_vote_deadline_us(aof_ctx *ctx, uint32_t microseconds)
{
    if (!ctx) return -EINVAL;
    if (microseconds < 100u) return fail(ctx, -EINVAL, "vote deadline of %u us: at least 100 us", microseconds);
    ctx->votes.deadline_ticks = microseconds > 10000000u ? 1000000000u : microseconds * 100u;
    return 0;
}

int aof_debug_vote_deadline_ticks(aof_ctx *ctx, uint32_t ticks)
{
    if (!ctx) return -EINVAL;
    ctx->votes.deadline_ticks = ticks;
    return 0;
}

int aof_debug_tile16_verdicts(aof_ctx *ctx, const uint8_t *verdicts, int count)
{
    if (!ctx) return -EINVAL;
    if (ctx->params.tile != 16) return fail(ctx, -EINVAL, "verdicts of the 16x16 search on a %dx%d context", ctx->params.tile, ctx->params.tile);
    if (count < 0 || count > kMaxForcedVerdicts) return fail(ctx, -EINVAL, "%d verdicts: 0 .. %d", count, kMaxForcedVerdicts);
    if (count > 0 && !verdicts) return fail(ctx, -EINVAL, "null verdicts");
    Tile16Verdicts f = {};
    for (int i = 0; i < count; i++) {
        if (verdicts[i] > 4) return fail(ctx, -EINVAL, "verdict %d of %u: 0 .. 4", i, verdicts[i]);
        f.v[i] = verdicts[i];
    }
    f.count = count;
    const bool changes = f.count != ctx->tile16_verdicts.count ||
                         std::memcmp(f.v, ctx->tile16_verdicts.v, sizeof f.v) != 0;
    kernel_choice_changes(ctx, changes);
    ctx->tile16_verdicts = f;
    return 0;
}

int aof_set_profiling(aof_ctx *ctx, int on)
{
    if (!ctx) return -EINVAL;
    DeviceGuard guard(ctx->device);
    Profiling &pr = ctx->prof;
    if (on && !pr.ev) {
        pr.ev = new (std::nothrow) hipEvent_t[AOF_K_COUNT][AOF_PROFILE_RING][2]();
        if (!pr.ev) return fail(ctx, -ENOMEM, "event ring");
        for (hipEvent_t *ev = *pr.ev[0], *end = ev + AOF_K_COUNT * AOF_PROFILE_RING * 2; ev != end; ev++)
            HIP_TRY(ctx, hipEventCreateWithFlags(ev, hipEventDisableSystemFence));
    }
    pr.on = on != 0;
    pr.mask = 0xFFFFFFFFu;
    if (on) for (int k = 0; k < AOF_K_COUNT; k++) pr.count[k] = 0;
    return 0;
}

int aof_set_profiling_mask(aof_ctx *ctx, uint32_t mask)
{
    int rc = aof_set_profiling(ctx, mask != 0);
    if (rc) return rc;
    ctx->prof.mask = mask;
    return 0;
}

int aof_profile_count(const aof_ctx *ctx, int kernel_id)
{
    if (!ctx || kernel_id < 0 || kernel_id >= AOF_K_COUNT) return -EINVAL;
    const int64_t n = ctx->prof.count[kernel_id];
    return (int)(n < AOF_PROFILE_RING ? n : AOF_PROFILE_RING);
}

int aof_profile_ms(aof_ctx *ctx, int kernel_id, int index, float *ms)
{
    if (!ctx || !ms) return -EINVAL;
    const int kept = aof_profile_count(ctx, kernel_id);
    if (kept < 0 || index < 0 || index >= kept)
        return fail(ctx, -EINVAL, "kernel %d has no timed launch %d", kernel_id, index);
    const int64_t n = ctx->prof.count[kernel_id];
    const int slot = (int)((n - kept + index) % AOF_PROFILE_RING);
    HIP_TRY(ctx, hipEventSynchronize(ctx->prof.ev[kernel_id][slot][1]));
    HIP_TRY(ctx, hipEventElapsedTime(ms, ctx->prof.ev[kernel_id][slot][0], ctx->prof.ev[kernel_id][slot][1]));
    return 0;
}

int aof_kernel_ms(aof_ctx *ctx, int kernel_id, float *ms)
{
    const int kept = ctx ? aof_profile_count(ctx, kernel_id) : -EINVAL;
    if (kept < 0) return -EINVAL;
    if (kept == 0) return fail(ctx, -EINVAL, "kernel %d was not timed", kernel_id);
    return aof_profile_ms(ctx, kernel_id, kept - 1, ms);
}

int aof_ingest_batch_device(const aof_ingest_params *p, const uint8_t *d_camera,
                            int64_t camera_stride, int64_t n_frames, uint8_t *d_cropped,
                            int64_t cropped_stride, uint32_t *d_hist, void *stream)
{
    if (!p || n_frames < 0) return -EINVAL;
    if (p->crop_width < 1 || p->crop_height < 1 || p->crop_width > p->camera_width ||
        p->crop_height > p->camera_height)
        return -EINVAL;
    if (n_frames == 0) return 0;
    if (!d_camera || (!d_cropped && !d_hist)) return -EINVAL;
    if (camera_stride < (int64_t)p->camera_width * p->camera_height && n_frames > 1) return -EINVAL;
    if (d_cropped && cropped_stride < (int64_t)p->crop_width * p->crop_height && n_frames > 1) return -EINVAL;
    if (n_frames * ((p->crop_height + 15) / 16) > 0x7FFFFFFF) return -EINVAL;
    return launch_ingest(*p, d_camera, camera_stride, n_frames, d_cropped, cropped_stride, d_hist, stream)
               ? -EIO : 0;
}

int aof_derotate_batch_device(const aof_derotate_params *p, const aof_flow *d_flows,
                              const aof_gyro *d_gyro, int64_t n, float *d_out, void *stream)
{
    if (!p || n < 0) return -EINVAL;
    if (n == 0) return 0;
    if (!d_flows || !d_gyro || !d_out || (n + 255) / 256 > 0x7FFFFFFF) return -EINVAL;
    return launch_derotate(*p, d_flows, d_gyro, n, d_out, stream) ? -EIO : 0;
}

}
```

aero-optical-flow_amd/csrc/aof_cols8_kernels.hpp:

```cpp
#pragma once

#include <type_traits>

#include "aof_cols8_plan.hpp"
#include "aof_device.hpp"
#include "aof_internal.hpp"
#include "aof_lane8.hpp"
#include "aof_reduce.hpp"
#include "aof_refine.hpp"

namespace aof {

namespace {

template <bool SUBPIXEL, bool VOTE>
__device__ __forceinline__ void cols_walk(const SearchArgs &a, const ColsPlan &plan, const PruneReport &report, const VoteMem *votes)
{
    const uint32_t wg = blockIdx.x;
    const uint32_t unit0 = wg * blockDim.x + threadIdx.x;
    const bool in_tail = (uint32_t)__builtin_amdgcn_readfirstlane((int)unit0) >= plan.head_units;
    const ColsSegments sg = in_tail ? plan.tail : plan.head;
    const uint32_t unit = in_tail ? unit0 - plan.head_units : unit0;
    const uint32_t pair = (in_tail ? plan.head_pairs : 0u) + (uint32_t)__builtin_amdgcn_readfirstlane((int)fast_div(unit, sg.div_units));
    if (pair >= (uint32_t)a.n_pairs) return;
    const uint32_t local = unit - (pair - (in_tail ? plan.head_pairs : 0u)) * sg.units_per_pair;
    const uint32_t seg = fast_div(local, plan.div_nx), bx = local - __umul24(seg, (uint32_t)a.grid.nx);
    const bool live = local < (uint32_t)(sg.segs * a.grid.nx);
    const int by0 = (int)seg * sg.len;
    const int W = a.w;
    constexpr int m = SUBPIXEL ? 1 : 0;

    const uint64_t span = a.n_pairs > 1 ? (uint64_t)(a.n_pairs - pair) * (uint64_t)a.pair_stride : (uint64_t)a.w * (uint64_t)a.h;
    const uint32_t records = span > 0xFFFFFFFFull ? 0xFFFFFFFFu : (uint32_t)span;
    const int64_t base = (int64_t)pair * a.pair_stride;
    const __amdgpu_buffer_rsrc_t rs_prev = __builtin_amdgcn_make_buffer_rsrc(const_cast<uint8_t *>(a.prev) + base, 0, records, kRawBuffer);
    const __amdgpu_buffer_rsrc_t rs_cur = __builtin_amdgcn_make_buffer_rsrc(const_cast<uint8_t *>(a.cur) + base, 0, records, kRawBuffer);
    typedef const __attribute__((address_space(4))) uint32_t *const_u32;
    int px = 0, py = 0, delta = 0;
    if (a.pred) {
        const uint32_t w3 = ((const_u32)(a.pred + pair))[3];
        px = (int8_t)(w3 >> 16); py = (int8_t)(w3 >> 24);
    }
    if (a.sums) {
        const uint32_t npix = (uint32_t)(a.w * a.h);
        const const_u32 sm = (const_u32)(a.sums + (size_t)pair * 4);
        delta = (int)((sm[a.level] + npix / 2) / npix) - (int)((sm[2 + a.level] + npix / 2) / npix);
    }
    const int i = a.grid.x0 + __mul24((int)bx, a.grid.step_x);
    const int wx0 = i + px - 4;
    const bool column_inside = live && wx0 - m >= 0 && wx0 + 16 + m <= a.w;
    uint32_t *const slots = reinterpret_cast<uint32_t *>(a.blocks) + (size_t)pair * (size_t)a.grid.blocks();
    uint8_t *const dirs = SUBPIXEL ? a.subdirs + (size_t)pair * (size_t)a.grid.blocks() : nullptr;

    const uint32_t mis = plan.aligned ? (uint32_t)__builtin_amdgcn_readfirstlane(wx0 & 3) : 0u;
    const bool lonely = (threadIdx.x & 63u) == 63u || bx + 1u == (uint32_t)a.grid.nx;
    auto shifted_rows = [&](uint32_t off, uint4 *dst) {
        u32x4 v[8];
        uint32_t e[8];
#pragma unroll
        for (int s = 0; s < 8; s++) v[s] = __builtin_amdgcn_raw_buffer_load_b128(rs_cur, off - mis, s * W, 0);
        if (lonely) {
#pragma unroll
            for (int s = 0; s < 8; s++) e[s] = __builtin_amdgcn_raw_buffer_load_b32(rs_cur, off - mis + 16u, s * W, 0);
        }
#pragma unroll
        for (int s = 0; s < 8; s++) {
            const uint32_t next = (uint32_t)__builtin_amdgcn_update_dpp(0, (int)v[s].z, 0x130, 0xF, 0xF, false);
            const uint32_t tail = lonely ? e[s] : next;
            dst[s] = make_uint4(__builtin_amdgcn_alignbyte(v[s].y, v[s].x, mis), __builtin_amdgcn_alignbyte(v[s].z, v[s].y, mis),
                                __builtin_amdgcn_alignbyte(v[s].w, v[s].z, mis), __builtin_amdgcn_alignbyte(tail, v[s].w, mis));
        }
    };
    uint4 win[16];
    {
        const int wy0 = a.grid.y0 + by0 * a.grid.step_y + py - 4;
        const uint32_t off_cur = (uint32_t)(__mul24(wy0, W) + wx0);
        if (mis != 0) {
            shifted_rows(off_cur, win);
        } else if (live) {
#pragma unroll
            for (int s = 0; s < 8; s++) {
                const u32x4 v = __builtin_amdgcn_raw_buffer_load_b128(rs_cur, off_cur, s * W, 0);
                win[s] = make_uint4(v.x, v.y, v.z, v.w);
            }
        }
        if (live && delta != 0) {
#pragma unroll
            for (int s = 0; s < 8; s++) win[s] = sat_add_u8x16(win[s], delta);
        }
    }
    int start_row = a.pred ? 4 : -1, prune_pays = a.prune == 2 ? 0 : 1;
    int seen = 0, paying = 0;
    std::conditional_t<VOTE && !SUBPIXEL, WalkVotes, NoWalkVotes> pending;
    pending.init();
    for (int step = 0; step < sg.len; step++) {
        const int by = by0 + step;
        const bool act = live && by < a.grid.ny;
        if (__ballot(act) == 0) break;
        const int j = a.grid.y0 + by * a.grid.step_y;
        const int wy0 = j + py - 4;
        const bool inside = act && column_inside && wy0 - m >= 0 && wy0 + 16 + m <= a.h;
        const uint32_t off_prev = (uint32_t)(__mul24(j, W) + i);
        const uint32_t off_cur8 = (uint32_t)(__mul24(wy0 + 8, W) + wx0);
        uint32_t ref[8][2];
        if (act) {
#pragma unroll
            for (int r = 0; r < 8; r++) {
                const u32x2 v = __builtin_amdgcn_raw_buffer_load_b64(rs_prev, off_prev, r * W, 2);
                ref[r][0] = v.x; ref[r][1] = v.y;
            }
            if (mis == 0) {
#pragma unroll
                for (int s = 8; s < 16; s++) {
                    const u32x4 v = __builtin_amdgcn_raw_buffer_load_b128(rs_cur, off_cur8, (s - 8) * W, 0);
                    win[s] = make_uint4(v.x, v.y, v.z, v.w);
                }
            }
        }
        if (mis != 0 && __ballot(act) != 0) shifted_rows(off_cur8, win + 8);
        if (act) {
            asm volatile("" : "+v"(win[15].w));
        }
        if (act && delta != 0) {
#pragma unroll
            for (int s = 8; s < 16; s++) win[s] = sat_add_u8x16(win[s], delta);
        }
        uint32_t gradient = 0;
        if (inside) gradient = gradient_gate(ref);
        const bool need = inside && gradient >= (uint32_t)a.feature_threshold;
        aof_block rec;
        rec.dx = 0; rec.dy = 0; rec.sad = AOF_SAD_SKIPPED;
        uint32_t best = 0xFFFFFFFFu;
        const unsigned long long needing = __ballot(need);
        if (needing != 0) {
            const int src = __ffsll((long long)needing) - 1;
            if (prune_pays == 0) {
                int droppable = 0;
                best = exhaustive_search_judged(win, ref, needing, droppable);
                prune_pays = __builtin_amdgcn_readfirstlane(droppable >= kJudgedRowsToPrune ? 1 : 0);
            } else {
                if (start_row < 0) start_row = __builtin_amdgcn_readfirstlane(vote_start_row(win, ref, needing));
                const int dropped = pruned_search(win, ref, needing, start_row, best);
                prune_pays = __builtin_amdgcn_readfirstlane(dropped >= 2 ? 1 : 0);
            }
            start_row = (int)((uint32_t)__builtin_amdgcn_readlane((int)best, src) & 0xFFFFu) / 9;
        }
        seen++;
        paying += prune_pays;
        int subdir = 8;
        if (need) {
            const int idx = (int)(best & 0xFFFFu);
            const int dyi = idx / 9, dxi = idx - 9 * dyi;
            rec.dx = (int8_t)(px + dxi - 4);
            rec.dy = (int8_t)(py + dyi - 4);
            rec.sad = (uint16_t)(best >> 16);
            if constexpr (SUBPIXEL) {
                if ((uint32_t)rec.sad < (uint32_t)a.value_threshold) {
                    const unsigned long long refining = __ballot(true);
                    const int udy = __builtin_amdgcn_readlane(dyi, __ffsll((long long)refining) - 1);
                    const bool have_ring = dyi == udy && udy >= 1 && udy <= 7 && dxi >= 1 && dxi <= 7;
                    RefineState<2> st;
                    st.init();
                    if (have_ring) refine_from_window(win, udy, dxi - 1, ref, st, (uint32_t)rec.sad);
                    if (!have_ring && rec.sad != 0) {
                        const uint32_t ring = off_cur8 + (uint32_t)((dyi - 9) * W + (dxi - 1));
                        uint32_t rows[10][3];
                        load_ring(rs_cur, ring, W, records, rows);
                        for_rows<-1, 8>([&](auto yc) {
                            constexpr int Y = decltype(yc)::value;
                            uint32_t d[3] = {rows[Y + 1][0], rows[Y + 1][1], rows[Y + 1][2]};
                            if (delta != 0) {
#pragma unroll
                                for (int q = 0; q < 3; q++) d[q] = sat_add_u8x4(d[q], delta);
                            }
                            st.template row<Y>(d, ref);
                        });
                    }
                    subdir = st.direction(rec.sad);
                }
            }
        }
        if (act) {
            const uint32_t slot = (uint32_t)(by * a.grid.nx) + bx;
            slots[slot] = __builtin_bit_cast(uint32_t, rec);
            if constexpr (SUBPIXEL) dirs[slot] = (uint8_t)subdir;
        }
        if constexpr (VOTE) {
            const bool ok = act && (uint32_t)rec.sad < (uint32_t)a.value_threshold;
            int hx = 0, hy = 0;
            if constexpr (SUBPIXEL) {
                hx = (subdir == 0 || subdir == 1 || subdir == 7) ? 1 : ((subdir == 3 || subdir == 4 || subdir == 5) ? -1 : 0);
                hy = (subdir == 1 || subdir == 2 || subdir == 3) ? 1 : ((subdir == 5 || subdir == 6 || subdir == 7) ? -1 : 0);
            }
            const int centre = 2 * a.hist_range + 1;
            if constexpr (SUBPIXEL) vote_and_arrive(*votes, a.hist_range, pair, act, ok, 2 * rec.dx + hx + centre, 2 * rec.dy + hy + centre);
            else pending.step(*votes, a.hist_range, pair, act, ok, 2 * rec.dx + hx + centre, 2 * rec.dy + hy + centre);
        }
#pragma unroll
        for (int s = 0; s < 8; s++) win[s] = win[s + 8];
    }
    if constexpr (VOTE) pending.flush(*votes, a.hist_range, pair);
    if (report.slots && threadIdx.x == 0 && wg % report.stride == 0)
        __hip_atomic_store(report.slots + wg / report.stride, (report.launch_no << 16) | ((uint32_t)paying << 8) | (uint32_t)seen,
                           __ATOMIC_RELAXED, __HIP_MEMORY_SCOPE_SYSTEM);
}

template <bool SUBPIXEL>
__global__ __launch_bounds__(kColsThreads, 4) void k_search_lane8_cols(SearchArgs a, ColsPlan plan, PruneReport report)
{
    cols_walk<SUBPIXEL, false>(a, plan, report, nullptr);
}

template <bool SUBPIXEL>
__global__ __launch_bounds__(kColsThreads, 4) void k_flow_lane8_cols(SearchArgs a, ColsPlan plan, PruneReport report, ColsVotes cv)
{
    if (blockIdx.x >= cv.search_wgs) {
        const uint32_t pair = (blockIdx.x - cv.search_wgs) * (blockDim.x >> 6) + (threadIdx.x >> 6);
        if (pair < (uint32_t)a.n_pairs) await_votes_and_finalise(cv.votes, cv.tail, pair);
        return;
    }
    cols_walk<SUBPIXEL, true>(a, plan, report, &cv.votes);
}

}

}
```

aero-optical-flow_amd/csrc/aof_cols8_plan.hpp:

```cpp
#pragma once

#include <cstdint>

#include "aof_internal.hpp"

namespace aof {

struct ColsSegments {
    int32_t segs, len;
    uint32_t units_per_pair;
    FastDiv div_units;
};
struct ColsPlan {
    ColsSegments head, tail;
    uint32_t head_pairs, head_units;
    FastDiv div_nx;
    uint32_t aligned;
};
struct ColsVotes {
    uint32_t search_wgs;
    FlowTail tail;
    VoteMem votes;
};


constexpr int kColsThreads = 256;
constexpr int kColsMaxRows = 8, kColsMinRows = 2;
constexpr int64_t kColsWavesWanted = 3072;
constexpr int64_t kWaveSlots = 4096;
constexpr int64_t kColsMaxUnits = 0x7FFF0000ll;

struct ColsLaunch {
    ColsPlan plan;
    int64_t per;
    int64_t pairs;
    int64_t tail_pairs;
    int64_t units, wgs;
};

inline ColsSegments cols_segments(const Grid &g, int len)
{
    ColsSegments s;
    s.len = len > g.ny ? g.ny : len;
    s.segs = (g.ny + s.len - 1) / s.len;
    s.units_per_pair = (uint32_t)((s.segs * g.nx + 63) / 64 * 64);
    s.div_units = fastdiv_make(s.units_per_pair);
    return s;
}

inline ColsLaunch cols_plan_make(const Grid &g, int w, int h, int64_t pair_stride, uintptr_t cur, int64_t n_pairs, int64_t done = 0)
{
    auto waves = [&](int len) { return n_pairs * (int64_t)(cols_segments(g, len).units_per_pair / 64); };
    int len = kColsMaxRows;
    while (len > kColsMinRows && waves(len) < kColsWavesWanted) len--;
    ColsLaunch l;
    ColsPlan &plan = l.plan;
    plan.head = cols_segments(g, len);
    plan.tail = cols_segments(g, len / 2 < kColsMinRows ? kColsMinRows : len / 2);
    plan.div_nx = fastdiv_make((uint32_t)g.nx);
    plan.aligned = (g.step_x == 8 && w % 4 == 0 && pair_stride % 4 == 0 && cur % 4 == 0 && ((int64_t)w * h) % 4 == 0) ? 1u : 0u;
    l.per = kColsMaxUnits / plan.tail.units_per_pair;
    l.pairs = n_pairs - done < l.per ? n_pairs - done : l.per;
    const int64_t wpp = plan.head.units_per_pair / 64, all = l.pairs * wpp, rest = all % kWaveSlots;
    l.tail_pairs = 0;
    if (rest != 0 && rest * 5 < kWaveSlots * 4 && plan.tail.len < plan.head.len && all > kWaveSlots) l.tail_pairs = (rest + wpp - 1) / wpp;
    plan.head_pairs = (uint32_t)(l.pairs - l.tail_pairs);
    plan.head_units = plan.head_pairs * plan.head.units_per_pair;
    l.units = (int64_t)plan.head_units + l.tail_pairs * plan.tail.units_per_pair;
    l.wgs = (l.units + kColsThreads - 1) / kColsThreads;
    return l;
}

}
```

aero-optical-flow_amd/csrc/aof_ctx.hpp:

```cpp
#pragma once

#include <hip/hip_runtime.h>
#include <chrono>
#include "aof_internal.hpp"

namespace aof {

struct HostState {
    bool ready;
    hipStream_t stream;
    uint8_t *d_frames[2];
    uint8_t *d_pair[2];
    int cur_slot;
    bool have_prev;
    aof_block *d_blocks; uint8_t *d_subdirs; aof_flow *d_flow;
    void *d_ws; size_t ws_bytes;
    uint8_t *h_frame;
    uint8_t *h_frames[2];
    bool zero_copy;
    aof_flow *h_flow;
    uint32_t *h_tag;
    hipGraphExec_t push_graph[2];
    bool push_tagged[2];
};

struct Resident {
    bool on;
    bool lost;
    bool deaf;
    double stop_wait_s;
    uint32_t seq;
    uint32_t frame_req[2];
    struct Kernel {
        ResidentBox *box;
        hipStream_t stream;
        uint32_t launches;
    } k;
};

constexpr int64_t kVotePairs = 2048;
constexpr uint32_t kVoteStride = 128;
constexpr uint32_t kVoteDeadlineTicks = 5000000;
struct InLaunchReduce {
    uint32_t *mem;
    int64_t pairs;
    uint32_t deadline_ticks;
    bool separate;
    hipEvent_t done;
    hipStream_t stream;
    bool used;
    bool captured;
};

struct AdaptiveSearch {
    uint32_t *slots;
    uint32_t launch_no;
    uint32_t expected;
    int belief;
    int since_probe;
    aof_search_stats stats;
};

struct Profiling {
    bool on;
    uint32_t mask;
    hipEvent_t (*ev)[AOF_PROFILE_RING][2];
    int64_t count[AOF_K_COUNT];
};

constexpr double kDrainS = 2.0;

struct DeviceGuard {
    int prev;
    explicit DeviceGuard(int device) : prev(-1)
    {
        if (hipGetDevice(&prev) != hipSuccess) prev = -1;
        if (prev != device) (void)hipSetDevice(device);
        else prev = -1;
    }
    ~DeviceGuard() { if (prev >= 0) (void)hipSetDevice(prev); }
};

int fail(aof_ctx *ctx, int code, const char *fmt, ...) __attribute__((format(printf, 3, 4)));
double seconds_since(std::chrono::steady_clock::time_point t0);
hipError_t drain_bounded(hipStream_t s, double seconds);
int wedge(aof_ctx *ctx, const char *what, hipError_t e);
int sticky_error(aof_ctx *ctx);
int device_check(aof_ctx *ctx);
bool plan_small_pair(const aof_ctx *ctx, const uint8_t *prev, const uint8_t *cur, aof_flow *flow, SmallArgs *sm);
bool resident_stop(aof_ctx *ctx);
void drop_push_graphs(aof_ctx *ctx);
void free_host_state(aof_ctx *ctx);

#define HIP_TRY(ctx, expr)                                                              \
    do {                                                                                \
        hipError_t e_ = (expr);                                                         \
        if (e_ != hipSuccess)                                                           \
            return fail(ctx, -EIO, "%s: %s", #expr, hipGetErrorString(e_));             \
    } while (0)

}

struct aof_ctx {
    aof_params params;
    aof::Grid g0, g1;
    int device;
    int cus;
    char err[256];
    int search_mode;
    bool force_generic;
    bool split_coarse;
    int bank_path;
    const aof_bank_stream *bank_streams;
    int32_t bank_streams_n;
    const aof_bank_sensor *bank_sensors;
    int32_t bank_sensors_n;
    uint64_t bank_camera_bytes;
    const uint8_t *bank_formats;
    int32_t bank_formats_n;
    const uint8_t *bank_bins;
    int32_t bank_bins_n;
    bool graph_disabled;
    bool capturing;
    bool wedged;
    uint32_t *h_fault;
    aof::HostState host;
    aof::Resident res;
    aof::InLaunchReduce votes;
    aof::OutboxCounter *outbox_counter;
    aof::AdaptiveSearch adapt;
    aof::Tile16Verdicts tile16_verdicts;
    aof::Profiling prof;
    aof_stream_stats stats;
};
```

aero-optical-flow_amd/csrc/aof_internal.hpp:

```cpp
#pragma once

#include <cstddef>
#include <cstdint>

#include "aof.h"

#if defined(__HIPCC__)
#define AOF_HD __host__ __device__
#else
#define AOF_HD
#endif

namespace aof {

struct FastDiv {
    uint32_t mul, shift;
};
inline FastDiv fastdiv_make(uint32_t d)
{
    FastDiv f = {0u, 0u};
    if (d == 0) return f;
    uint32_t l = 0;
    while ((1ull << l) < d) l++;
    f.mul = (uint32_t)(((1ull << 32) * ((1ull << l) - d)) / d + 1);
    f.shift = l;
    return f;
}

inline bool aligned(const void *p, uintptr_t n) { return reinterpret_cast<uintptr_t>(p) % n == 0; }

inline float limiter_period_us(int output_rate) { return output_rate > 0 ? 1.0e6f / (float)output_rate : 0.0f; }

struct Grid {
    int32_t x0, y0, step_x, step_y, nx, ny;
    AOF_HD int32_t blocks() const { return nx * ny; }
};

int grid_for_level(const aof_params &p, int level, Grid *g);
int level_range(const aof_params &p, int level);
int value_threshold_u16(const aof_params &p);
int reduce_chunks(int nblocks);
size_t hist_bytes_per_pair(const aof_params &p, int level);

struct FlowTail {
    int32_t nblocks;
    int32_t range;
    int32_t hist_filter;
    int32_t min_valid;
    aof_flow *flows;
    const aof_flow *pred;
    int32_t emit_predictor;
};

struct VoteMem {
    uint32_t *base;
    uint32_t stride;
    uint32_t *fault;
    uint32_t deadline_ticks;
};

constexpr int kPruneSlots = 256;
struct PruneReport {
    uint32_t *slots;
    uint32_t launch_no;
    uint32_t stride;
    uint32_t expected;
};

struct SearchArgs {
    const uint8_t *prev;
    const uint8_t *cur;
    int64_t pair_stride;
    int32_t w, h;
    int32_t tile, search;
    Grid grid;
    int32_t feature_threshold;
    int32_t value_threshold;
    int32_t subpixel;
    aof_block *blocks;
    uint8_t *subdirs;
    const aof_flow *pred;
    const uint32_t *sums;
    int32_t level;
    int64_t n_pairs;
    int32_t hist_range;
    int32_t prune;
    uint32_t *hints;
    FastDiv div_nb, div_nx;
};

struct ReduceArgs {
    const aof_block *blocks;
    const uint8_t *subdirs;
    int32_t value_threshold;
    FlowTail tail;
    int64_t n_pairs;
    const uint32_t *parts;
    int32_t nstrips;
    uint32_t *chunk_parts;
};

struct CoarseArgs {
    const uint8_t *prev, *cur;
    int64_t pair_stride;
    int32_t w, h;
    int32_t tile, search, subpixel;
    Grid grid;
    int32_t feature_threshold;
    int32_t value_threshold;
    uint32_t *sums;
    aof_block *blocks;
    FlowTail tail;
    int64_t n_pairs;
    FastDiv div_nb, div_nx, div_chunks;
    int32_t first_generation;
    int32_t stagger_groups, stagger_ticks;
    int32_t rows_per_sweep;
};

struct SmallArgs {
    SearchArgs l0, l1;
    FlowTail t0, t1;
    uint32_t *sums;
    int32_t levels;
};

struct PyramidArgs {
    const uint8_t *prev, *cur;
    int64_t pair_stride;
    int32_t w, h;
    uint8_t *l1_prev, *l1_cur;
    uint32_t *sums;
    int64_t n_pairs;
    int32_t sequence;
};

int launch_pyramid(const PyramidArgs &a, void *stream);
int launch_zero_words(uint32_t *words, int64_t count, void *stream);
bool coarse_fused_supported(const CoarseArgs &a);
int launch_coarse_fused(const CoarseArgs &a, void *stream);
int launch_search_generic(const SearchArgs &a, void *stream);
int launch_refine(const SearchArgs &a, void *stream);
bool lane8_supported(const SearchArgs &a);
bool lane8_votes_supported(const SearchArgs &a, const VoteMem &votes, int64_t capacity_pairs);
int launch_search_lane8(const SearchArgs &a, void *stream, const FlowTail *tail = nullptr,
                        const VoteMem *votes = nullptr, PruneReport *report = nullptr);
int64_t lane8_chunks(const SearchArgs &a);
bool lane8_cols_supported(const SearchArgs &a);
bool lane8_cols_votes_supported(const SearchArgs &a, const VoteMem &votes, int64_t capacity_pairs);
int launch_search_lane8_cols(const SearchArgs &a, void *stream, PruneReport *report = nullptr, const FlowTail *tail = nullptr,
                             const VoteMem *votes = nullptr);
constexpr int64_t kPruneMinChunks = 2048;
int lane8_group(const SearchArgs &a);
int launch_flow_lane8(const SearchArgs &a, const FlowTail &tail, void *stream);
bool tile16_supported(const SearchArgs &a);
bool tile16_refines(const SearchArgs &a);
constexpr int kMaxForcedVerdicts = 8;
struct Tile16Verdicts {
    uint8_t v[kMaxForcedVerdicts];
    int32_t count;
};
int launch_search_tile16(const SearchArgs &a, void *stream, const Tile16Verdicts &forced);
bool flow_small_supported(const SmallArgs &a);
int launch_flow_small(const SmallArgs &a, void *stream);
int launch_flow_small_tagged(const SmallArgs &a, aof_flow *host_record, const uint32_t *tag, void *stream);
struct ResidentBox {
    unsigned long long word;
    uint32_t pad0[14];
    uint32_t done;
    uint32_t running;
    uint32_t exited;
    uint32_t started;
    uint32_t pad1[12];
};
static_assert(sizeof(ResidentBox) == 128, "two cache lines: host -> device, device -> host");
constexpr unsigned long long kResidentStopBit = 1ull << 63;
inline unsigned long long resident_word(uint32_t request, int slot, uint32_t prev_request)
{
    const unsigned long long prev = prev_request ? (unsigned long long)(prev_request & 0x3FFFFFFFu) + 1ull : 0ull;
    return (unsigned long long)request | ((unsigned long long)(slot & 1) << 32) | (prev << 33);
}
int launch_flow_resident(const SmallArgs &a, ResidentBox *box, aof_flow *host_record, const uint8_t *frame_a,
                         const uint8_t *frame_b, uint32_t served, uint32_t launch_no, uint64_t idle_ticks,
                         uint64_t life_ticks, bool deaf, void *stream);
constexpr int64_t kLimitScanFrames = 4096;
struct SequenceArgs {
    int64_t n_frames;
    const uint64_t *time_us;
    const aof_gyro *gyro;
    const aof_flow *flows;
    int32_t output_rate;
    float period_us;
    float focal_x, focal_y;
    uint64_t offset_timestamp_usec;
    uint8_t system_id, component_id, first_seq;
    uint32_t *jump[2], *hops[2];
    uint8_t *reached;
    uint32_t *rank;
    uint32_t *count;
    uint32_t *status;
    aof_seq_record *records;
    uint8_t *frames;
    uint8_t *frame_len;
};
inline int sequence_rounds(int64_t n_frames)
{
    int r = 0;
    while ((1ll << (2 * r)) <= n_frames) r++;
    return r;
}
int launch_sequence_output(const SequenceArgs &a, void *stream);
struct BankState {
    uint32_t has_prev;
    uint32_t time_last_pub;
    float sum_flow_x, sum_flow_y;
    int32_t sum_flow_quality, valid_frame_count;
    double gyro_x, gyro_y, gyro_z;
    uint32_t messages;
    uint32_t frames;
    uint64_t next_exposure_us;
};
static_assert(sizeof(BankState) == 64, "one bank state record is 64 bytes");
struct BankCamera {
    const uint8_t *camera;
    int64_t camera_stride;
    int32_t pitch, origin;
    int32_t crop_w, crop_h;
    int32_t mx0, my0, mx1, my1;
    const uint32_t *hist;
    aof_exposure_record *exposure;
    uint32_t interval_us;
    float *derotated;
    aof_derotate_params derotate;
};
struct BankArgs {
    int32_t n_streams;
    int64_t frame_stride, frame_bytes;
    const uint8_t *frames;
    const uint64_t *time_us;
    const uint8_t *active;
    const aof_gyro *gyro;
    uint8_t *bank_frames;
    BankState *state;
    const aof_flow *flows;
    int32_t output_rate;
    float period_us;
    float focal_x, focal_y;
    uint64_t offset_timestamp_usec;
    uint8_t system_id, component_id, first_seq;
    const aof_bank_stream *streams;
    aof_tick_record *records;
    uint8_t *mavlink;
    uint8_t *mavlink_len;
    BankCamera cam;
};
struct BankSensors {
    const aof_bank_sensor *recs;
    uint64_t camera_bytes, camera_base;
    const uint8_t *formats;
    const uint8_t *bins;
};
int launch_bank_tick(const SmallArgs &sm, const BankArgs &a, void *stream, const BankSensors &sen = BankSensors{nullptr, 0, 0, nullptr, nullptr});
int launch_bank_commit(const BankArgs &a, void *stream, const uint8_t *count = nullptr, int32_t round = 0,
                       const BankSensors &sen = BankSensors{nullptr, 0, 0, nullptr, nullptr});
struct BankBurst {
    int32_t n_rounds;
    int64_t round_stride;
    const uint8_t *count;
};
int launch_bank_burst(const SmallArgs &sm, const BankArgs &a, const BankBurst &b, void *stream,
                      const BankSensors &sen = BankSensors{nullptr, 0, 0, nullptr, nullptr});
int launch_bank_reset(BankState *state, const uint8_t *mask, int32_t n_streams, void *stream);
constexpr uint32_t kOutboxTile = 1024;
struct OutboxCounter {
    uint32_t arrivals;
    uint32_t pad;
    unsigned long long found;
};
struct OutboxArgs {
    uint32_t n, n_streams;
    const uint8_t *records;
    const uint8_t *mavlink;
    const uint8_t *mavlink_len;
    const uint8_t *exposure;
    const uint8_t *derotated;
    uint32_t cap_messages, cap_exposures;
    uint8_t *outbox;
    uint8_t *messages, *exposures;
    unsigned long long tag;
    const unsigned long long *d_tag;
    OutboxCounter *counter;
};
int launch_bank_outbox(const OutboxArgs &a, void *stream);
struct ExposureArgs {
    aof_exposure_control ec;
    uint32_t n_streams, n_rounds;
    const uint8_t *records;
    aof_exposure_state *state;
    aof_exposure_command *commands;
};
int launch_bank_exposure(const ExposureArgs &a, void *stream);
int launch_bank_exposure_reset(aof_exposure_state *state, const uint8_t *mask, uint32_t n_streams, uint16_t exposure0,
                               uint8_t gain0, const uint16_t *d_exposure0, const uint8_t *d_gain0, void *stream);
struct ImuArgs {
    uint32_t n_streams, n_rounds, max_samples;
    uint8_t system_id, component_id, first_seq;
    const aof_bank_stream *streams;
    const uint8_t *samples;
    const uint8_t *sample_count;
    const uint64_t *time_us;
    const uint8_t *records_in;
    uint8_t *records_out;
    aof_imu_state *state;
    uint8_t *mavlink, *mavlink_len;
};
int launch_bank_imu(const ImuArgs &a, void *stream);
int launch_bank_imu_reset(aof_imu_state *state, const uint8_t *mask, uint32_t n_streams, uint64_t offset0, void *stream);
struct MavlinkRxArgs {
    uint32_t n_streams, n_rounds, max_bytes, max_samples;
    const uint8_t *bytes;
    const uint16_t *len;
    aof_mavlink_rx_state *state;
    uint8_t *samples;
    uint8_t *sample_count;
};
int launch_bank_mavlink_rx(const MavlinkRxArgs &a, void *stream);
int launch_bank_mavlink_rx_reset(aof_mavlink_rx_state *state, const uint8_t *mask, uint32_t n_streams, void *stream);
bool plan_small_batch(const aof_ctx *ctx, const uint8_t *prev, const uint8_t *cur, int64_t stride, int64_t n, aof_flow *flows,
                      void *d_workspace, SmallArgs *sm);
int bank_path(const aof_ctx *ctx);
void set_bank_path(aof_ctx *ctx, int path);
const aof_bank_stream *bank_streams(const aof_ctx *ctx, int32_t *n_streams);
void set_bank_streams(aof_ctx *ctx, const aof_bank_stream *d_streams, int32_t n_streams);
const aof_bank_sensor *bank_sensors(const aof_ctx *ctx, int32_t *n_streams, uint64_t *camera_bytes);
void set_bank_sensors(aof_ctx *ctx, const aof_bank_sensor *d_sensors, int32_t n_streams, uint64_t camera_bytes);
const uint8_t *bank_pixel_formats(const aof_ctx *ctx, int32_t *n_streams);
void set_bank_pixel_formats(aof_ctx *ctx, const uint8_t *d_formats, int32_t n_streams);
const uint8_t *bank_binning(const aof_ctx *ctx, int32_t *n_streams);
void set_bank_binning(aof_ctx *ctx, const uint8_t *d_bins, int32_t n_streams);
int precheck(aof_ctx *ctx);
int ctx_fail(aof_ctx *ctx, int code, const char *what);
bool sequence_runs_k1(aof_ctx *ctx, const uint8_t *d_frames, int64_t n_pairs, void *d_workspace);
int flow_sequence(aof_ctx *ctx, const uint8_t *d_frames, int64_t n_pairs, aof_flow *d_flows, void *d_workspace,
                  size_t workspace_bytes, void *stream, bool k1_ready);
int launch_reduce(const ReduceArgs &a, void *stream);
int launch_derotate(const aof_derotate_params &p, const aof_flow *flows, const aof_gyro *gyro,
                    int64_t n, float *out, void *stream);
struct IngestSensors {
    const aof_bank_sensor *recs;
    uint64_t base, camera_bytes;
    uint8_t *ok;
    const uint8_t *formats;
    const uint8_t *bins;
};
int launch_ingest(const aof_ingest_params &p, const uint8_t *camera, int64_t camera_stride,
                  int64_t n_frames, uint8_t *cropped, int64_t cropped_stride, uint32_t *hist,
                  void *stream, const IngestSensors &sensors = IngestSensors{nullptr, 0, 0, nullptr, nullptr, nullptr});
bool ingest_pyramid_supported(const aof_ingest_params &p, const uint8_t *cropped, int64_t cropped_stride);
int launch_ingest_pyramid(const aof_ingest_params &p, const uint8_t *camera, int64_t camera_stride, int64_t n_frames,
                          uint8_t *cropped, int64_t cropped_stride, uint32_t *hist, uint8_t *l1, uint32_t *sums, void *stream);

}
```

aero-optical-flow_amd/csrc/aof_lane8_launch.hpp:

```cpp
#pragma once

#include <cstdint>

#include "aof_internal.hpp"

namespace aof {

struct ColsPlan;
struct ColsVotes;

int launch_k_search_lane8_ff(const SearchArgs &a, uint32_t items, uint32_t wgs, int threads, void *stream);
int launch_k_search_lane8_ft(const SearchArgs &a, uint32_t items, uint32_t wgs, int threads, void *stream);
int launch_k_search_lane8_tf(const SearchArgs &a, uint32_t items, uint32_t wgs, int threads, void *stream);
int launch_k_search_lane8_tt(const SearchArgs &a, uint32_t items, uint32_t wgs, int threads, void *stream);
int launch_k_flow_lane8_flat_ff(const SearchArgs &a, uint32_t items, uint32_t search_wgs, uint32_t grid, int threads, const FlowTail &t, const VoteMem &v, void *stream);
int launch_k_flow_lane8_flat_ft(const SearchArgs &a, uint32_t items, uint32_t search_wgs, uint32_t grid, int threads, const FlowTail &t, const VoteMem &v, void *stream);
int launch_k_flow_lane8_flat_tf(const SearchArgs &a, uint32_t items, uint32_t search_wgs, uint32_t grid, int threads, const FlowTail &t, const VoteMem &v, void *stream);
int launch_k_flow_lane8_flat_tt(const SearchArgs &a, uint32_t items, uint32_t search_wgs, uint32_t grid, int threads, const FlowTail &t, const VoteMem &v, void *stream);
int launch_k_search_lane8_pruned_f(const SearchArgs &a, uint32_t items, uint32_t wgs, int spw, const PruneReport &rep, void *stream);
int launch_k_search_lane8_pruned_t(const SearchArgs &a, uint32_t items, uint32_t wgs, int spw, const PruneReport &rep, void *stream);
int launch_k_flow_lane8_f(const SearchArgs &a, const FlowTail &t, int ppw, uint32_t wgs, size_t lds, void *stream);
int launch_k_flow_lane8_t(const SearchArgs &a, const FlowTail &t, int ppw, uint32_t wgs, size_t lds, void *stream);
int launch_k_search_lane8_cols_f(const SearchArgs &a, const ColsPlan &plan, const PruneReport &rep, uint32_t wgs, int threads, void *stream);
int launch_k_search_lane8_cols_t(const SearchArgs &a, const ColsPlan &plan, const PruneReport &rep, uint32_t wgs, int threads, void *stream);
int launch_k_flow_lane8_cols_f(const SearchArgs &a, const ColsPlan &plan, const PruneReport &rep, const ColsVotes &cv, uint32_t grid, int threads, void *stream);
int launch_k_flow_lane8_cols_t(const SearchArgs &a, const ColsPlan &plan, const PruneReport &rep, const ColsVotes &cv, uint32_t grid, int threads, void *stream);

}
```

aero-optical-flow_amd/csrc/aof_reduce.hpp:

```cpp
#pragma once

#include "aof_device.hpp"
#include "aof_internal.hpp"

namespace aof {

__device__ __forceinline__ void peak_window(int pos, int n, int *lo, int *hi)
{
    *lo = *hi = pos;
    if (pos > 1 && pos < n - 2) { *lo = pos - 2; *hi = pos + 2; }
    else if (pos == 0) { *hi = pos + 2; }
    else if (pos == n - 1) { *lo = pos - 2; }
    else if (pos == 1) { *lo = pos - 1; *hi = pos + 2; }
    else if (pos == n - 2) { *lo = pos - 2; *hi = pos + 1; }
}

template <typename T>
__device__ __forceinline__ T floor_div(T a, T b)
{
    T q = a / b;
    if ((a % b) < 0) q--;
    return q;
}

__device__ __forceinline__ void write_flow(const FlowTail &a, int64_t pair, int n, uint32_t vx, uint32_t wx, uint32_t vy,
                                           uint32_t wy, const int *sums)
{
#pragma clang fp contract(off)
    const int centre = 2 * a.range + 1;
    aof_flow out;
    out.flow_x = out.flow_y = 0.0f;
    out.count = (uint32_t)sums[2];
    out.quality = 0;
    out.flags = 0;
    out.pred_x = out.pred_y = 0;
    int px = 0, py = 0;
    const long long count = sums[2];
    const bool small = (long long)n * a.nblocks < (1ll << 28);
    if (count > (long long)a.min_valid && count > 0) {
        if (a.hist_filter) {
            out.flow_x = (__fdiv_rn((float)vx, (float)wx) - (float)centre) / 2.0f;
            out.flow_y = (__fdiv_rn((float)vy, (float)wy) - (float)centre) / 2.0f;
            if (small) {
                px = floor_div<int>((int)(2 * vx + wx), (int)(2 * wx)) - centre;
                py = floor_div<int>((int)(2 * vy + wy), (int)(2 * wy)) - centre;
            } else {
                px = (int)(floor_div<long long>(2ll * vx + wx, 2ll * wx) - centre);
                py = (int)(floor_div<long long>(2ll * vy + wy, 2ll * wy) - centre);
            }
        } else {
            out.flow_x = __fdiv_rn((float)sums[0] * 0.5f, (float)count);
            out.flow_y = __fdiv_rn((float)sums[1] * 0.5f, (float)count);
            if (small) {
                px = floor_div<int>(2 * sums[0] + (int)count, 2 * (int)count);
                py = floor_div<int>(2 * sums[1] + (int)count, 2 * (int)count);
            } else {
                px = (int)floor_div<long long>(2ll * sums[0] + count, 2ll * count);
                py = (int)floor_div<long long>(2ll * sums[1] + count, 2ll * count);
            }
        }
        out.quality = small ? (uint8_t)((uint32_t)count * 255u / (uint32_t)a.nblocks)
                            : (uint8_t)((unsigned long long)count * 255ull / (unsigned long long)a.nblocks);
        out.flags |= AOF_FLAG_FLOW_VALID;
    }
    if (a.emit_predictor) {
        out.pred_x = (int8_t)px;
        out.pred_y = (int8_t)py;
    } else if (a.pred) {
        const aof_flow p = a.pred[pair];
        out.pred_x = p.pred_x;
        out.pred_y = p.pred_y;
        if (p.flags & AOF_FLAG_FLOW_VALID) out.flags |= AOF_FLAG_PRED_VALID;
    }
    a.flows[pair] = out;
}

__device__ __forceinline__ void finalise_flow_wave_bins(const FlowTail &a, int64_t pair, uint32_t hx, uint32_t hy,
                                                        int sum2x, int sum2y, int total, aof_flow *record_out = nullptr,
                                                        const aof_flow *pred_rec = nullptr);

__device__ __forceinline__ void finalise_flow_wave(const FlowTail &a, int64_t pair, const uint32_t *hist_x,
                                                   const uint32_t *hist_y, const int *sums, aof_flow *record_out = nullptr,
                                                   const aof_flow *pred_rec = nullptr)
{
    const int n = 2 * (2 * a.range + 1) + 1;
    const int k = (int)(threadIdx.x & 63);
    finalise_flow_wave_bins(a, pair, k < n ? hist_x[k] : 0u, k < n ? hist_y[k] : 0u, sums[0], sums[1], sums[2],
                            record_out, pred_rec);
}

__device__ __forceinline__ void finalise_flow_wave_bins(const FlowTail &a, int64_t pair, uint32_t hx, uint32_t hy,
                                                        int sum2x, int sum2y, int total, aof_flow *record_out,
                                                        const aof_flow *pred_rec)
{
    const int centre = 2 * a.range + 1, n = 2 * centre + 1;
    const int k = (int)(threadIdx.x & 63);
    const int sums[3] = {sum2x, sum2y, total};
    uint32_t mx = hx, my = hy;
#pragma unroll
    for (int o = 32; o >= 1; o >>= 1) {
        const uint32_t ox = (uint32_t)__shfl_xor((int)mx, o, 64), oy = (uint32_t)__shfl_xor((int)my, o, 64);
        mx = ox > mx ? ox : mx;
        my = oy > my ? oy : my;
    }
    const int posx = __ffsll((long long)__ballot(k < n && hx == mx)) - 1;
    const int posy = __ffsll((long long)__ballot(k < n && hy == my)) - 1;
    int lox, hix, loy, hiy;
    peak_window(posx, n, &lox, &hix);
    peak_window(posy, n, &loy, &hiy);
    const bool inx = k >= lox && k <= hix, iny = k >= loy && k <= hiy;
    const uint32_t vx = wave_sum_u32(inx ? (uint32_t)k * hx : 0u), wx = wave_sum_u32(inx ? hx : 0u);
    const uint32_t vy = wave_sum_u32(iny ? (uint32_t)k * hy : 0u), wy = wave_sum_u32(iny ? hy : 0u);
    const bool axis_y = k == 1;
    const uint32_t v = axis_y ? vy : vx, w = axis_y ? wy : wx;
    const int s2 = axis_y ? sums[1] : sums[0];
    const long long count = sums[2];
    const bool valid = count > (long long)a.min_valid && count > 0;
    const bool small = (long long)n * a.nblocks < (1ll << 28);
    float flow = 0.0f;
    int pred = 0;
    if (k < 2 && valid) {
#pragma clang fp contract(off)
        if (a.hist_filter) {
            flow = (__fdiv_rn((float)v, (float)w) - (float)centre) / 2.0f;
            if (a.emit_predictor)
                pred = small ? floor_div<int>((int)(2 * v + w), (int)(2 * w)) - centre
                             : (int)(floor_div<long long>(2ll * v + w, 2ll * w) - centre);
        } else {
            flow = __fdiv_rn((float)s2 * 0.5f, (float)count);
            if (a.emit_predictor)
                pred = small ? floor_div<int>(2 * s2 + (int)count, 2 * (int)count)
                             : (int)floor_div<long long>(2ll * s2 + count, 2ll * count);
        }
    }
    const float flow_y = __shfl(flow, 1, 64);
    const int pred_y = __shfl(pred, 1, 64);
    if (k == 0) {
        aof_flow out;
        out.flow_x = flow; out.flow_y = flow_y;
        out.count = (uint32_t)sums[2];
        out.quality = 0;
        out.flags = 0;
        out.pred_x = out.pred_y = 0;
        if (valid) {
            out.quality = small ? (uint8_t)((uint32_t)count * 255u / (uint32_t)a.nblocks)
                                : (uint8_t)((unsigned long long)count * 255ull / (unsigned long long)a.nblocks);
            out.flags |= AOF_FLAG_FLOW_VALID;
        }
        if (a.emit_predictor) {
            out.pred_x = (int8_t)pred;
            out.pred_y = (int8_t)pred_y;
        } else if (a.pred) {
            const aof_flow p = pred_rec ? *pred_rec : a.pred[pair];
            out.pred_x = p.pred_x;
            out.pred_y = p.pred_y;
            if (p.flags & AOF_FLAG_FLOW_VALID) out.flags |= AOF_FLAG_PRED_VALID;
        }
        a.flows[pair] = out;
        if (record_out) *record_out = out;
    }
}

__device__ __forceinline__ void vote_add_agent(uint32_t *p, uint32_t v)
{
    (void)__hip_atomic_fetch_add(p, v, __ATOMIC_RELAXED, __HIP_MEMORY_SCOPE_AGENT);
}

__device__ __forceinline__ void wave_vote_agent(uint32_t *hist, int bin, bool active)
{
    unsigned long long todo = __ballot(active);
    while (todo) {
        const int leader = __ffsll((long long)todo) - 1;
        const int b = __shfl(bin, leader, 64);
        const unsigned long long same = __ballot(active && bin == b) & todo;
        if ((int)(threadIdx.x & 63) == leader) vote_add_agent(&hist[b], (uint32_t)__popcll(same));
        todo &= ~same;
    }
}

__device__ __forceinline__ void vote_and_arrive(const VoteMem &vm, int range, uint32_t pair, bool member, bool ok,
                                                int bin_x, int bin_y)
{
    const unsigned long long members = __ballot(member);
    if (members == 0) return;
    const int n = 2 * (2 * range + 1) + 1, lane = (int)(threadIdx.x & 63);
    uint32_t *rec = vm.base + (size_t)pair * vm.stride, *hist_x = rec + 2, *hist_y = rec + 2 + n;
    ok = ok && member;
    const unsigned long long voters = __ballot(ok);
    const int head = __ffsll((long long)members) - 1;
    const unsigned long long arrival = ((unsigned long long)__popcll(members) << 32) | (unsigned long long)__popcll(voters);
    bool one_motion = true;
    int k = 0;
    if (voters) {
        const int key = bin_x | (bin_y << 8);
        k = __builtin_amdgcn_readlane(key, __ffsll((long long)voters) - 1);
        one_motion = (__ballot(ok && key == k) & voters) == voters;
    }
    if (one_motion) {
        if (lane == head) {
            if (voters) {
                const uint32_t c = (uint32_t)__popcll(voters);
                vote_add_agent(&hist_x[k & 0xFF], c);
                vote_add_agent(&hist_y[k >> 8], c);
            }
            (void)__hip_atomic_fetch_add(reinterpret_cast<unsigned long long *>(rec), arrival, __ATOMIC_RELAXED,
                                         __HIP_MEMORY_SCOPE_AGENT);
        }
        return;
    }
    wave_vote_agent(hist_x, bin_x, ok);
    wave_vote_agent(hist_y, bin_y, ok);
    if (lane == head)
        (void)__hip_atomic_fetch_add(reinterpret_cast<unsigned long long *>(rec), arrival, __ATOMIC_RELAXED,
                                     __HIP_MEMORY_SCOPE_AGENT);
}

struct NoWalkVotes {
    __device__ __forceinline__ void init() {}
    __device__ __forceinline__ void flush(const VoteMem &, int, uint32_t) {}
    __device__ __forceinline__ void step(const VoteMem &, int, uint32_t, bool, bool, int, int) {}
};
struct WalkVotes {
    int key;
    uint32_t votes, arrivals;

    __device__ __forceinline__ void init() { key = 0; votes = 0; arrivals = 0; }

    __device__ __forceinline__ void flush(const VoteMem &vm, int range, uint32_t pair)
    {
        if (arrivals == 0) return;
        const int n = 2 * (2 * range + 1) + 1;
        uint32_t *rec = vm.base + (size_t)pair * vm.stride, *hist_x = rec + 2, *hist_y = rec + 2 + n;
        if ((threadIdx.x & 63) == 0) {
            if (votes) {
                vote_add_agent(&hist_x[key & 0xFF], votes);
                vote_add_agent(&hist_y[key >> 8], votes);
            }
            (void)__hip_atomic_fetch_add(reinterpret_cast<unsigned long long *>(rec), ((unsigned long long)arrivals << 32) | votes,
                                         __ATOMIC_RELAXED, __HIP_MEMORY_SCOPE_AGENT);
        }
        votes = 0; arrivals = 0;
    }

    __device__ __forceinline__ void step(const VoteMem &vm, int range, uint32_t pair, bool member, bool ok, int bin_x, int bin_y)
    {
        const unsigned long long members = __ballot(member);
        if (members == 0) return;
        ok = ok && member;
        const unsigned long long voters = __ballot(ok);
        const uint32_t nm = (uint32_t)__popcll(members), nv = (uint32_t)__popcll(voters);
        if (voters == 0) { arrivals = (uint32_t)__builtin_amdgcn_readfirstlane((int)(arrivals + nm)); return; }
        const int mine = bin_x | (bin_y << 8);
        const int k = __builtin_amdgcn_readlane(mine, __ffsll((long long)voters) - 1);
        if ((__ballot(ok && mine == k) & voters) == voters) {
            if (votes != 0 && key != k) flush(vm, range, pair);
            key = k;
            votes = (uint32_t)__builtin_amdgcn_readfirstlane((int)(votes + nv));
            arrivals = (uint32_t)__builtin_amdgcn_readfirstlane((int)(arrivals + nm));
            return;
        }
        flush(vm, range, pair);
        const int n = 2 * (2 * range + 1) + 1;
        uint32_t *rec = vm.base + (size_t)pair * vm.stride;
        wave_vote_agent(rec + 2, bin_x, ok);
        wave_vote_agent(rec + 2 + n, bin_y, ok);
        if ((threadIdx.x & 63) == 0)
            (void)__hip_atomic_fetch_add(reinterpret_cast<unsigned long long *>(rec), ((unsigned long long)nm << 32) | nv, __ATOMIC_RELAXED,
                                         __HIP_MEMORY_SCOPE_AGENT);
    }
};

__device__ __forceinline__ void await_votes_and_finalise(const VoteMem &vm, const FlowTail &tail, uint32_t pair)
{
    const uint64_t deadline_ticks = vm.deadline_ticks;
    const int centre = 2 * tail.range + 1, n = 2 * centre + 1, lane = (int)(threadIdx.x & 63);
    uint32_t *rec = vm.base + (size_t)pair * vm.stride, *hist_x = rec + 2, *hist_y = rec + 2 + n;
    const uint64_t t0 = __builtin_amdgcn_s_memrealtime();
    uint32_t hx = 0, hy = 0;
    int total = 0;
    bool complete = false;
    for (;;) {
        uint32_t arrived = 0, announced = 0;
        if (lane < n) {
            hx = __hip_atomic_load(&hist_x[lane], __ATOMIC_RELAXED, __HIP_MEMORY_SCOPE_AGENT);
            hy = __hip_atomic_load(&hist_y[lane], __ATOMIC_RELAXED, __HIP_MEMORY_SCOPE_AGENT);
        } else if (lane == 63) {
            const unsigned long long a = __hip_atomic_load(reinterpret_cast<unsigned long long *>(rec), __ATOMIC_RELAXED,
                                                           __HIP_MEMORY_SCOPE_AGENT);
            arrived = (uint32_t)(a >> 32);
            announced = (uint32_t)a;
        }
        arrived = (uint32_t)__shfl((int)arrived, 63, 64);
        announced = (uint32_t)__shfl((int)announced, 63, 64);
        total = (int)wave_sum_u32(hx);
        complete = arrived == (uint32_t)tail.nblocks && (uint32_t)total == announced && wave_sum_u32(hy) == announced;
        if (complete || __builtin_amdgcn_s_memrealtime() - t0 > deadline_ticks) break;
        __builtin_amdgcn_s_sleep(8);
    }
    if (lane < n) {
        __hip_atomic_store(&hist_x[lane], 0u, __ATOMIC_RELAXED, __HIP_MEMORY_SCOPE_AGENT);
        __hip_atomic_store(&hist_y[lane], 0u, __ATOMIC_RELAXED, __HIP_MEMORY_SCOPE_AGENT);
    } else if (lane == 63) {
        __hip_atomic_store(reinterpret_cast<unsigned long long *>(rec), 0ull, __ATOMIC_RELAXED, __HIP_MEMORY_SCOPE_AGENT);
    }
    if (!complete) {
        if (lane == 0) {
            aof_flow none;
            __builtin_memset(&none, 0, sizeof(none));
            tail.flows[pair] = none;
            __hip_atomic_store(vm.fault, pair + 1u, __ATOMIC_RELEASE, __HIP_MEMORY_SCOPE_SYSTEM);
        }
        return;
    }
    const int sum2x = (int)wave_sum_u32((uint32_t)((lane - centre) * (int)hx));
    const int sum2y = (int)wave_sum_u32((uint32_t)((lane - centre) * (int)hy));
    finalise_flow_wave_bins(tail, (int64_t)pair, hx, hy, sum2x, sum2y, total);
}

__device__ __forceinline__ void finalise_flow(const FlowTail &a, int64_t pair, const uint32_t *hist_x,
                                              const uint32_t *hist_y, const int *sums)
{
    const int centre = 2 * a.range + 1, n = 2 * centre + 1;
    uint32_t vx = 0, wx = 0, vy = 0, wy = 0;
    if (a.hist_filter && sums[2] > a.min_valid && sums[2] > 0) {
        int posx = 0, posy = 0;
        uint32_t maxx = 0, maxy = 0;
        for (int k = 0; k < n; k++) {
            if (hist_x[k] > maxx) { maxx = hist_x[k]; posx = k; }
            if (hist_y[k] > maxy) { maxy = hist_y[k]; posy = k; }
        }
        int lo, hi;
        peak_window(posx, n, &lo, &hi);
        for (int k = lo; k <= hi; k++) { vx += (uint32_t)k * hist_x[k]; wx += hist_x[k]; }
        peak_window(posy, n, &lo, &hi);
        for (int k = lo; k <= hi; k++) { vy += (uint32_t)k * hist_y[k]; wy += hist_y[k]; }
    }
    write_flow(a, pair, n, vx, wx, vy, wy, sums);
}

}
```

aero-optical-flow_amd/csrc/k_reduce.hip:

```cpp
#include "aof_device.hpp"
#include "aof_internal.hpp"
#include "aof_reduce.hpp"

namespace aof {

namespace {

constexpr int kThreads = 256;
constexpr int kMaxHist = 256;
constexpr int64_t kMidPairs = 1024;
constexpr int64_t kWidePairs = 512;

template <int GROUP, int kThreads = 256>
__global__ __launch_bounds__(kThreads) void k_reduce(ReduceArgs a)
{
    constexpr int kGroups = kThreads / GROUP;
    __shared__ uint32_t s_hist[kGroups][2][kMaxHist];
    __shared__ int s_sums[kGroups][3];
    const int grp = (int)threadIdx.x / GROUP, tid = (int)threadIdx.x % GROUP;
    const int64_t pair = (int64_t)blockIdx.x * kGroups + grp;
    if (GROUP < kThreads && pair >= a.n_pairs) return;
    auto sync = [] { if (GROUP == kThreads) __syncthreads(); else __builtin_amdgcn_wave_barrier(); };
    uint32_t (*hist)[kMaxHist] = s_hist[grp];
    int *sums = s_sums[grp];
    const int centre = 2 * a.tail.range + 1, n = 2 * centre + 1;
    for (int k = tid; k < n; k += GROUP) { hist[0][k] = 0; hist[1][k] = 0; }
    if (tid < 3) sums[tid] = 0;
    sync();

    if (a.parts) {
        const uint32_t *parts = a.parts + (size_t)pair * a.nstrips * (size_t)(2 * n);
        for (int k = tid; k < 2 * n; k += GROUP) {
            uint32_t v = 0;
            for (int st = 0; st < a.nstrips; st++) v += parts[(size_t)st * (2 * n) + k];
            const int axis = k >= n, bin = k - axis * n;
            hist[axis][bin] = v;
            if (v) {
                atomicAdd(&sums[axis], (bin - centre) * (int)v);
                if (!axis) atomicAdd(&sums[2], (int)v);
            }
        }
        sync();
    } else {
    const aof_block *blocks = a.blocks + pair * a.tail.nblocks;
    const uint8_t *subdirs = a.subdirs ? a.subdirs + pair * a.tail.nblocks : nullptr;
    int s2x = 0, s2y = 0, cnt = 0;
    auto vote = [&](bool ok, aof_block r, int sd) {
        ok = ok && !(r.sad == AOF_SAD_SKIPPED || (int)r.sad >= a.value_threshold);
        int hx = 0, hy = 0;
        if (ok && subdirs) {
            hx = (sd == 0 || sd == 1 || sd == 7) ? 1 : ((sd == 3 || sd == 4 || sd == 5) ? -1 : 0);
            hy = (sd == 1 || sd == 2 || sd == 3) ? 1 : ((sd == 5 || sd == 6 || sd == 7) ? -1 : 0);
        }
        const int vx = 2 * r.dx + hx, vy = 2 * r.dy + hy;
        wave_vote2(hist[0], hist[1], vx + centre, vy + centre, ok);
        if (ok) { s2x += vx; s2y += vy; cnt++; }
    };
    typedef uint32_t u32_bytes __attribute__((aligned(1)));
    const uint32_t *words = reinterpret_cast<const uint32_t *>(blocks);
    const int quads = a.tail.nblocks / 4;
    const int qrounds = (quads + GROUP - 1) / GROUP;
    auto vote_quad = [&](bool have, const uint32_t (&w)[4], uint32_t sd4) {
        int key[4], weight = 0, first = 0;
        bool ok[4], messy = false;
#pragma unroll
        for (int j = 0; j < 4; j++) {
            const uint32_t sad = w[j] >> 16;
            ok[j] = have && !(sad == AOF_SAD_SKIPPED || (int)sad >= a.value_threshold);
            const int sd = (int)((sd4 >> (8 * j)) & 0xFFu);
            int hx = 0, hy = 0;
            if (subdirs) {
                hx = (sd == 0 || sd == 1 || sd == 7) ? 1 : ((sd == 3 || sd == 4 || sd == 5) ? -1 : 0);
                hy = (sd == 1 || sd == 2 || sd == 3) ? 1 : ((sd == 5 || sd == 6 || sd == 7) ? -1 : 0);
            }
            const int vx = 2 * (int)(int8_t)(w[j] & 0xFFu) + hx, vy = 2 * (int)(int8_t)((w[j] >> 8) & 0xFFu) + hy;
            key[j] = (vx + centre) | ((vy + centre) << 16);
            if (ok[j]) {
                s2x += vx; s2y += vy; cnt++;
                if (weight == 0) first = key[j];
                else if (key[j] != first) messy = true;
                weight++;
            }
        }
        if (__ballot(messy) == 0) {
            wave_vote2_weighted(hist[0], hist[1], first, weight);
        } else {
#pragma unroll
            for (int j = 0; j < 4; j++) wave_vote2(hist[0], hist[1], key[j] & 0xFFFF, key[j] >> 16, ok[j]);
        }
    };
    constexpr int kBatchQ = 3;
    for (int it0 = 0; it0 < qrounds; it0 += kBatchQ) {
        uint32_t rec[kBatchQ][4], sdir[kBatchQ];
#pragma unroll
        for (int k = 0; k < kBatchQ; k++) {
            const int q = (it0 + k) * GROUP + tid;
#pragma unroll
            for (int j = 0; j < 4; j++) rec[k][j] = 0xFFFF0000u;
            sdir[k] = 0x08080808u;
            if (it0 + k < qrounds && q < quads) {
                __builtin_memcpy(rec[k], words + 4 * q, 16);
                if (subdirs) sdir[k] = *reinterpret_cast<const u32_bytes *>(subdirs + 4 * q);
            }
        }
#pragma unroll
        for (int k = 0; k < kBatchQ; k++) {
            if (it0 + k >= qrounds) break;
            const int q = (it0 + k) * GROUP + tid;
            vote_quad(q < quads, rec[k], sdir[k]);
        }
    }
    {
        const int b = 4 * quads + tid;
        const bool in = b < a.tail.nblocks;
        aof_block r;
        r.dx = 0; r.dy = 0; r.sad = AOF_SAD_SKIPPED;
        if (in) r = blocks[b];
        vote(in, r, in && subdirs ? subdirs[b] : 8);
    }
    s2x = (int)wave_sum_u32((uint32_t)s2x);
    s2y = (int)wave_sum_u32((uint32_t)s2y);
    cnt = (int)wave_sum_u32((uint32_t)cnt);
    if ((tid & 63) == 0) {
        atomicAdd(&sums[0], s2x);
        atomicAdd(&sums[1], s2y);
        atomicAdd(&sums[2], cnt);
    }
    sync();
    }
    if (n <= 64) {
        if (tid < 64) finalise_flow_wave(a.tail, pair, hist[0], hist[1], sums);
    } else if (tid == 0) {
        finalise_flow(a.tail, pair, hist[0], hist[1], sums);
    }
}

__global__ __launch_bounds__(kThreads) void k_reduce_chunk(ReduceArgs a, int chunks)
{
    __shared__ uint32_t hist[2][kMaxHist];
    const int chunk = (int)(blockIdx.x % (uint32_t)chunks);
    const int64_t pair = (int64_t)(blockIdx.x / (uint32_t)chunks);
    const int tid = threadIdx.x;
    const int centre = 2 * a.tail.range + 1, n = 2 * centre + 1;
    for (int k = tid; k < n; k += kThreads) { hist[0][k] = 0; hist[1][k] = 0; }
    __syncthreads();
    const int per = (a.tail.nblocks + chunks - 1) / chunks;
    const int b0 = chunk * per, b1 = min(a.tail.nblocks, b0 + per);
    const uint32_t *blocks = reinterpret_cast<const uint32_t *>(a.blocks) + pair * a.tail.nblocks;
    const uint8_t *subdirs = a.subdirs ? a.subdirs + pair * a.tail.nblocks : nullptr;
    for (int base = b0; base < b1; base += kThreads) {
        const int b = base + tid;
        const bool in = b < b1;
        const aof_block r = __builtin_bit_cast(aof_block, in ? blocks[b] : 0xFFFF0000u);
        const int sd = in && subdirs ? subdirs[b] : 8;
        const bool ok = in && !(r.sad == AOF_SAD_SKIPPED || (int)r.sad >= a.value_threshold);
        int hx = 0, hy = 0;
        if (ok && subdirs) {
            hx = (sd == 0 || sd == 1 || sd == 7) ? 1 : ((sd == 3 || sd == 4 || sd == 5) ? -1 : 0);
            hy = (sd == 1 || sd == 2 || sd == 3) ? 1 : ((sd == 5 || sd == 6 || sd == 7) ? -1 : 0);
        }
        wave_vote(hist[0], 2 * r.dx + hx + centre, ok);
        wave_vote(hist[1], 2 * r.dy + hy + centre, ok);
    }
    __syncthreads();
    uint32_t *out = a.chunk_parts + ((size_t)pair * chunks + chunk) * (size_t)(2 * n);
    for (int k = tid; k < 2 * n; k += kThreads) out[k] = k < n ? hist[0][k] : hist[1][k - n];
}

}

int launch_reduce(const ReduceArgs &a, void *stream)
{
    if (a.n_pairs == 0) return 0;
    if (a.n_pairs > 0x7FFFFFFF) return (int)hipErrorInvalidValue;
    const int chunks = a.parts ? 0 : reduce_chunks(a.tail.nblocks);
    if (chunks > 0 && a.chunk_parts && a.n_pairs * chunks <= 0x7FFFFFFF) {
        hipLaunchKernelGGL(k_reduce_chunk, dim3((uint32_t)(a.n_pairs * chunks)), dim3(kThreads), 0,
                           static_cast<hipStream_t>(stream), a, chunks);
        ReduceArgs b = a;
        b.parts = a.chunk_parts;
        b.nstrips = chunks;
        hipLaunchKernelGGL(k_reduce<kThreads>, dim3((uint32_t)a.n_pairs), dim3(kThreads), 0,
                           static_cast<hipStream_t>(stream), b);
        return (int)hipGetLastError();
    }
    if (a.tail.nblocks <= 256 && !a.parts)
        hipLaunchKernelGGL(k_reduce<64>, dim3((uint32_t)((a.n_pairs + 3) / 4)), dim3(kThreads), 0,
                           static_cast<hipStream_t>(stream), a);
    else if (a.n_pairs <= kWidePairs && a.tail.nblocks >= 2048 && !a.parts)
        hipLaunchKernelGGL((k_reduce<1024, 1024>), dim3((uint32_t)a.n_pairs), dim3(1024), 0,
                           static_cast<hipStream_t>(stream), a);
    else if (a.n_pairs <= kMidPairs && a.tail.nblocks >= 2048 && !a.parts)
        hipLaunchKernelGGL((k_reduce<512, 512>), dim3((uint32_t)a.n_pairs), dim3(512), 0,
                           static_cast<hipStream_t>(stream), a);
    else
        hipLaunchKernelGGL(k_reduce<kThreads>, dim3((uint32_t)a.n_pairs), dim3(kThreads), 0,
                           static_cast<hipStream_t>(stream), a);
    return (int)hipGetLastError();
}

}
```

aero-optical-flow_amd/csrc/k_search_cols8.hip:

```cpp
#include <hip/hip_runtime.h>

#include "aof_cols8_plan.hpp"
#include "aof_internal.hpp"
#include "aof_lane8_launch.hpp"

namespace aof {

bool lane8_cols_supported(const SearchArgs &a)
{
    return lane8_supported(a) && a.grid.step_y == 8 && a.grid.nx >= 16 && a.grid.ny >= 2 && a.grid.blocks() > 256;
}

bool lane8_cols_votes_supported(const SearchArgs &a, const VoteMem &votes, int64_t capacity_pairs)
{
    const int n = 2 * (2 * a.hist_range + 1) + 1;
    if (!lane8_cols_supported(a) || !votes.base || !votes.fault || n > 62 || votes.stride < (uint32_t)(2 + 2 * n)) return false;
    return a.n_pairs <= capacity_pairs;
}

int launch_search_lane8_cols(const SearchArgs &a, void *stream, PruneReport *report, const FlowTail *tail, const VoteMem *votes)
{
    if (report) report->expected = 0;
    if (a.n_pairs == 0) return 0;
    if (!lane8_cols_supported(a) || (a.subpixel && !a.subdirs)) return (int)hipErrorInvalidValue;
    const int64_t per = cols_plan_make(a.grid, a.w, a.h, a.pair_stride, reinterpret_cast<uintptr_t>(a.cur), a.n_pairs).per;
    for (int64_t done = 0; done < a.n_pairs; done += per) {
        const ColsLaunch l = cols_plan_make(a.grid, a.w, a.h, a.pair_stride, reinterpret_cast<uintptr_t>(a.cur), a.n_pairs, done);
        const ColsPlan &plan = l.plan;
        SearchArgs s = a;
        s.n_pairs = l.pairs;
        s.prev += done * a.pair_stride;
        s.cur += done * a.pair_stride;
        s.blocks += done * a.grid.blocks();
        if (s.subdirs) s.subdirs += done * a.grid.blocks();
        if (s.pred) s.pred += done;
        if (s.sums) s.sums += done * 4;
        const int threads = kColsThreads;
        const int64_t wgs = l.wgs;
        PruneReport rep = {nullptr, 0, 1, 0};
        if (report && report->slots && done == 0) {
            rep = *report;
            rep.stride = (uint32_t)((wgs + kPruneSlots - 1) / kPruneSlots);
            report->stride = rep.stride;
            report->expected = (uint32_t)((wgs + rep.stride - 1) / rep.stride);
        }
        int rc;
        if (tail && votes) {
            if (done != 0 || s.n_pairs != a.n_pairs) return (int)hipErrorInvalidValue;
            ColsVotes cv;
            cv.search_wgs = (uint32_t)wgs;
            cv.tail = *tail;
            cv.votes = *votes;
            const int64_t finalisers = (s.n_pairs + (threads >> 6) - 1) / (threads >> 6);
            rc = (s.subpixel ? launch_k_flow_lane8_cols_t : launch_k_flow_lane8_cols_f)(s, plan, rep, cv, (uint32_t)(wgs + finalisers), threads, stream);
        } else {
            rc = (s.subpixel ? launch_k_search_lane8_cols_t : launch_k_search_lane8_cols_f)(s, plan, rep, (uint32_t)wgs, threads, stream);
        }
        if (rc) return rc;
    }
    return 0;
}

}
```

include/aof.h:

```cpp
#ifndef AOF_H
#define AOF_H

#include <stddef.h>
#include <stdint.h>

#ifdef __cplusplus
extern "C" {
#endif
#if defined(__GNUC__)
#pragma GCC visibility push(default)
#endif

#define AOF_VERSION 102

#define AOF_GRID_DENSE 0
#define AOF_GRID_PX4FLOW 1

typedef struct aof_params {
    int32_t width, height;
    int32_t tile;
    int32_t search;
    int32_t grid_mode;
    int32_t num_blocks;
    int32_t feature_threshold;
    int32_t value_threshold;
    int32_t subpixel;
    int32_t hist_filter;
    int32_t pyramid_levels;
    int32_t mean_subtract;
    int32_t min_valid;
} aof_params;

typedef struct aof_block {
    int8_t dx, dy;
    uint16_t sad;
} aof_block;

#define AOF_SAD_SKIPPED 0xFFFFu
#define AOF_FLAG_FLOW_VALID 1u
#define AOF_FLAG_PRED_VALID 2u

typedef struct aof_flow {
    float flow_x, flow_y;
    uint32_t count;
    uint8_t quality;
    uint8_t flags;
    int8_t pred_x, pred_y;
} aof_flow;

typedef struct aof_ws_layout {
    size_t total_bytes;
    size_t sums;
    size_t l1_prev;
    size_t l1_cur;
    size_t l1_blocks;
    size_t l1_subdirs;
    size_t l1_flows;
    size_t l0_blocks;
    size_t l0_subdirs;
    size_t l0_hist;
    size_t l1_hist;
    size_t hints;
} aof_ws_layout;

typedef struct aof_ctx aof_ctx;

#define AOF_K_PYRAMID 0
#define AOF_K_SEARCH_L1 1
#define AOF_K_REDUCE_L1 2
#define AOF_K_SEARCH 3
#define AOF_K_REDUCE 4
#define AOF_K_COUNT 5

int aof_version(void);
const char *aof_strerror(int code);

int aof_params_default(aof_params *p, int width, int height);
int aof_params_px4flow(aof_params *p, int width, int height, int search,
                       int feature_threshold, int value_threshold);
int aof_params_check(const aof_params *p);
int aof_grid(const aof_params *p, int level, int32_t *x0, int32_t *y0, int32_t *step_x,
             int32_t *step_y, int32_t *nx, int32_t *ny);
int aof_workspace_layout(const aof_params *p, int64_t n_pairs, aof_ws_layout *out);

int aof_create(const aof_params *p, int device, aof_ctx **out);
void aof_destroy(aof_ctx *ctx);
const char *aof_last_error(const aof_ctx *ctx);
int aof_get_params(const aof_ctx *ctx, aof_params *out);
const char *aof_search_variant(const aof_ctx *ctx);
int aof_set_force_generic(aof_ctx *ctx, int on);
#define AOF_SEARCH_EXHAUSTIVE 0
#define AOF_SEARCH_PRUNED 1
#define AOF_SEARCH_ADAPTIVE 2
int aof_set_search_mode(aof_ctx *ctx, int mode);
int aof_get_search_mode(const aof_ctx *ctx);
typedef struct aof_search_stats {
    uint64_t pruned_launches;
    uint64_t exhaustive_launches;
    uint64_t reports_read;
    int32_t belief;
    int32_t paying_pct;
} aof_search_stats;
int aof_get_search_stats(const aof_ctx *ctx, aof_search_stats *out);
int aof_set_search_belief(aof_ctx *ctx, int belief);

int aof_flow_batch_device(aof_ctx *ctx, const uint8_t *d_prev, const uint8_t *d_cur,
                          int64_t pair_stride, int64_t n_pairs, aof_block *d_blocks,
                          uint8_t *d_subdirs, aof_flow *d_flows, void *d_workspace,
                          size_t workspace_bytes, void *stream);

int aof_set_split_coarse(aof_ctx *ctx, int on);

int aof_set_reduce_fusion(aof_ctx *ctx, int on);
int aof_set_vote_deadline_us(aof_ctx *ctx, uint32_t microseconds);
int aof_debug_vote_deadline_ticks(aof_ctx *ctx, uint32_t ticks);
int aof_debug_tile16_verdicts(aof_ctx *ctx, const uint8_t *verdicts, int count);

int aof_flow_pair_host(aof_ctx *ctx, const uint8_t *prev, const uint8_t *cur, aof_block *blocks,
                       uint8_t *subdirs, aof_flow *flow);
int aof_stream_push_host(aof_ctx *ctx, const uint8_t *frame, aof_flow *flow);
int aof_stream_reset(aof_ctx *ctx);
int aof_set_stream_resident(aof_ctx *ctx, int on);
typedef struct aof_stream_stats {
    uint64_t calls;
    uint64_t resident_served;
    uint32_t resident_launches;
    uint32_t resident_fallbacks;
    uint32_t resident_lost;
    uint32_t tagged_slow;
    float launch_call_us_max;
    float start_latency_us_max;
    char last_report[320];
} aof_stream_stats;
int aof_stream_get_stats(const aof_ctx *ctx, aof_stream_stats *out);
int aof_debug_resident_fault(aof_ctx *ctx, int deaf, uint32_t stop_wait_us);
int aof_set_stream_graph(aof_ctx *ctx, int on);

#define AOF_EXPOSURE_BINS 10
#define AOF_EXPOSURE_MASK_SIZE 128
typedef struct aof_ingest_params {
    int32_t camera_width, camera_height;
    int32_t crop_width, crop_height;
} aof_ingest_params;
int aof_ingest_batch_device(const aof_ingest_params *p, const uint8_t *d_camera,
                            int64_t camera_stride, int64_t n_frames, uint8_t *d_cropped,
                            int64_t cropped_stride, uint32_t *d_hist, void *stream);
float aof_exposure_msv(const uint32_t hist[AOF_EXPOSURE_BINS]);
int aof_exposure_bin(int grey);

typedef struct aof_gyro {
    float integ_x, integ_y, integ_z;
    float dt_s;
} aof_gyro;
typedef struct aof_derotate_params {
    float focal_x, focal_y;
    float max_flow;
    float rate_threshold;
} aof_derotate_params;
int aof_derotate_batch_device(const aof_derotate_params *p, const aof_flow *d_flows,
                              const aof_gyro *d_gyro, int64_t n, float *d_out, void *stream);

typedef struct aof_sequence_params {
    aof_ingest_params ingest;
    float focal_x, focal_y;
    int32_t output_rate;
    uint64_t offset_timestamp_usec;
    uint8_t system_id, component_id;
    uint8_t first_seq;
    uint8_t derotate;
    aof_derotate_params derotate_params;
} aof_sequence_params;

typedef struct aof_seq_record {
    uint32_t frame;
    int32_t quality;
    int32_t dt_us;
    float flow_x, flow_y;
    float gyro_x, gyro_y, gyro_z;
} aof_seq_record;

#define AOF_SEQ_FRAME_BYTES 56
#define AOF_SEQ_STATUS_STALLED 1u

typedef struct aof_seq_layout {
    size_t total_bytes;
    size_t cropped;
    size_t exposure;
    size_t flows;
    size_t derotated;
    size_t count;
    size_t records;
    size_t frames;
    size_t frame_len;
    size_t scratch;
} aof_seq_layout;
int aof_sequence_layout(const aof_params *p, const aof_sequence_params *sp, int64_t n_frames, aof_seq_layout *out);
int aof_sequence_device(aof_ctx *ctx, const aof_sequence_params *sp, const uint8_t *d_camera, int64_t camera_stride,
                        int64_t n_frames, const uint64_t *d_time_us, const aof_gyro *d_gyro, void *d_workspace,
                        size_t workspace_bytes, void *stream);
float aof_flow_angle(float flow_px, float focal_px);

typedef struct aof_bank_params {
    int32_t n_streams;
    int64_t frame_stride;
    float focal_x, focal_y;
    int32_t output_rate;
    uint64_t offset_timestamp_usec;
    uint8_t system_id, component_id, first_seq;
} aof_bank_params;

#define AOF_TICK_HELD (-1)
#define AOF_TICK_IDLE (-2)
typedef struct aof_tick_record {
    int32_t quality;
    int32_t dt_us;
    float flow_x, flow_y;
    float gyro_x, gyro_y, gyro_z;
    uint32_t frame;
    aof_flow pixel;
} aof_tick_record;

struct aof_bank_layout {
    size_t total_bytes;
    size_t frames;
    size_t state;
    size_t scratch;
};
int aof_bank_layout(const aof_params *p, const aof_bank_params *bp, struct aof_bank_layout *out);
int aof_bank_reset_device(aof_ctx *ctx, const aof_bank_params *bp, const uint8_t *d_mask, void *d_bank,
                          size_t bank_bytes, void *stream);
int aof_bank_push_device(aof_ctx *ctx, const aof_bank_params *bp, const uint8_t *d_frames, const uint64_t *d_time_us,
                         const uint8_t *d_active, const aof_gyro *d_gyro, void *d_bank, size_t bank_bytes,
                         aof_tick_record *d_records, uint8_t *d_mavlink, uint8_t *d_mavlink_len, void *stream);
int aof_set_bank_path(aof_ctx *ctx, int path);

typedef struct aof_bank_stream {
    float    focal_x, focal_y;
    int32_t  output_rate;
    uint8_t  system_id, component_id, first_seq, reserved0;
    uint64_t offset_timestamp_usec;
    uint64_t reserved1;
} aof_bank_stream;
int aof_bank_stream_from_params(const aof_bank_params *bp, aof_bank_stream *out);
int aof_set_bank_streams(aof_ctx *ctx, const aof_bank_stream *d_streams, int32_t n_streams);

typedef struct aof_bank_camera {
    aof_ingest_params ingest;
    int64_t camera_stride;
    uint32_t exposure_interval_us;
    uint8_t derotate;
    aof_derotate_params derotate_params;
} aof_bank_camera;

typedef struct aof_exposure_record {
    uint32_t hist[AOF_EXPOSURE_BINS];
    float msv;
    uint32_t due;
} aof_exposure_record;

int aof_bank_camera_layout(const aof_params *p, const aof_bank_params *bp, const aof_bank_camera *cam,
                           struct aof_bank_layout *out, size_t *staging);
int aof_bank_push_camera_device(aof_ctx *ctx, const aof_bank_params *bp, const aof_bank_camera *cam,
                                const uint8_t *d_camera, const uint64_t *d_time_us, const uint8_t *d_active,
                                const aof_gyro *d_gyro, void *d_bank, size_t bank_bytes, aof_tick_record *d_records,
                                aof_exposure_record *d_exposure, float *d_derotated,
                                uint8_t *d_mavlink, uint8_t *d_mavlink_len, void *stream);

#define AOF_BANK_BURST_MAX 16
typedef struct aof_bank_burst {
    int32_t n_rounds;
    int64_t round_stride;
} aof_bank_burst;
int aof_bank_push_burst_device(aof_ctx *ctx, const aof_bank_params *bp, const aof_bank_burst *burst,
                               const uint8_t *d_frames, const uint64_t *d_time_us, const uint8_t *d_count,
                               const aof_gyro *d_gyro, void *d_bank, size_t bank_bytes, aof_tick_record *d_records,
                               uint8_t *d_mavlink, uint8_t *d_mavlink_len, void *stream);
int aof_bank_push_camera_burst_device(aof_ctx *ctx, const aof_bank_params *bp, const aof_bank_camera *cam,
                                      const aof_bank_burst *burst, const uint8_t *d_camera, const uint64_t *d_time_us,
                                      const uint8_t *d_count, const aof_gyro *d_gyro, void *d_bank, size_t bank_bytes,
                                      aof_tick_record *d_records, aof_exposure_record *d_exposure, float *d_derotated,
                                      uint8_t *d_mavlink, uint8_t *d_mavlink_len, void *stream);

#define AOF_TICK_BAD_SENSOR (-5)
typedef struct aof_bank_sensor {
    uint64_t offset;
    int32_t  pitch;
    int32_t  width, height;
    int32_t  x0, y0;
    uint32_t reserved;
} aof_bank_sensor;
int aof_set_bank_sensors(aof_ctx *ctx, const aof_bank_sensor *d_sensors, int32_t n_streams, uint64_t camera_bytes);
int aof_bank_sensor_from_camera(const aof_params *p, const aof_bank_camera *cam, int32_t stream, aof_bank_sensor *out);
int aof_bank_sensor_centred(const aof_params *p, uint64_t offset, int32_t pitch, int32_t width, int32_t height, aof_bank_sensor *out);
int aof_bank_sensor_valid(const aof_bank_sensor *rec, int32_t crop_width, int32_t crop_height, uint64_t base, uint64_t camera_bytes);
int aof_ingest_sensors_device(int32_t crop_width, int32_t crop_height, const uint8_t *d_camera, uint64_t camera_bytes,
                              const aof_bank_sensor *d_sensors, int64_t n_frames, uint8_t *d_cropped, int64_t cropped_stride,
                              uint32_t *d_hist, uint8_t *d_ok, void *stream);

#define AOF_PIXEL_GREY8     0
#define AOF_PIXEL_LUMA16_LO 1
#define AOF_PIXEL_LUMA16_HI 2
int aof_set_bank_pixel_formats(aof_ctx *ctx, const uint8_t *d_formats, int32_t n_streams);
int aof_bank_sensor_valid_format(const aof_bank_sensor *rec, uint8_t format, int32_t crop_width, int32_t crop_height,
                                 uint64_t base, uint64_t camera_bytes);
int aof_ingest_sensor_formats_device(int32_t crop_width, int32_t crop_height, const uint8_t *d_camera, uint64_t camera_bytes,
                                     const aof_bank_sensor *d_sensors, const uint8_t *d_formats, int64_t n_frames,
                                     uint8_t *d_cropped, int64_t cropped_stride, uint32_t *d_hist, uint8_t *d_ok, void *stream);

#define AOF_BANK_BIN_MAX 4
int aof_set_bank_binning(aof_ctx *ctx, const uint8_t *d_bins, int32_t n_streams);
int aof_bank_sensor_valid_binned(const aof_bank_sensor *rec, uint8_t format, uint8_t bin, int32_t crop_width, int32_t crop_height,
                                 uint64_t base, uint64_t camera_bytes);
int aof_bank_sensor_centred_binned(const aof_params *p, uint64_t offset, int32_t pitch, int32_t width, int32_t height,
                                   uint8_t format, uint8_t bin, aof_bank_sensor *out);
int aof_ingest_sensors_binned_device(int32_t crop_width, int32_t crop_height, const uint8_t *d_camera, uint64_t camera_bytes,
                                     const aof_bank_sensor *d_sensors, const uint8_t *d_formats, const uint8_t *d_bins,
                                     int64_t n_frames, uint8_t *d_cropped, int64_t cropped_stride, uint32_t *d_hist, uint8_t *d_ok,
                                     void *stream);

typedef struct aof_outbox_entry {
    uint32_t stream;
    uint16_t round;
    uint8_t  mavlink_len;
    uint8_t  reserved0;
    uint8_t  mavlink[AOF_SEQ_FRAME_BYTES];
    aof_tick_record record;
    float    derotated[2];
    uint8_t  reserved1[8];
} aof_outbox_entry;
typedef struct aof_outbox_exposure {
    uint32_t stream;
    uint16_t round;
    uint16_t reserved0;
    aof_exposure_record exposure;
    uint8_t  reserved1[8];
} aof_outbox_exposure;
typedef struct aof_outbox_header {
    uint64_t tag;
    uint32_t n_messages, messages_found;
    uint32_t n_exposures, exposures_found;
    uint8_t  reserved[40];
} aof_outbox_header;
struct aof_outbox_layout {
    size_t total_bytes;
    size_t messages;
    size_t exposures;
};
int aof_outbox_layout(uint32_t capacity_messages, uint32_t capacity_exposures, struct aof_outbox_layout *out);
int aof_bank_collect_device(aof_ctx *ctx, int32_t n_streams, int32_t n_rounds, const aof_tick_record *d_records,
                            const uint8_t *d_mavlink, const uint8_t *d_mavlink_len, const aof_exposure_record *d_exposure,
                            const float *d_derotated, uint32_t capacity_messages, uint32_t capacity_exposures,
                            void *outbox, size_t outbox_bytes, uint64_t tag, const uint64_t *d_tag, void *stream);
int aof_outbox_alloc_host(size_t bytes, void **out);
int aof_outbox_free_host(void *p);

typedef struct aof_exposure_control {
    float msv_target;
    float exposure_p, exposure_i, exposure_d;
    float gain_p, gain_i, gain_d;
    float exposure_change_threshold, exposure_max;
    float gain_change_threshold, gain_max;
} aof_exposure_control;
int aof_exposure_control_default(aof_exposure_control *ec);

typedef struct aof_exposure_state {
    float msv_error_old, msv_error_int;
    uint16_t exposure;
    uint8_t gain, reserved;
    uint32_t updates;
} aof_exposure_state;

#define AOF_EXPOSURE_UPDATED      1u
#define AOF_EXPOSURE_SET_EXPOSURE 2u
#define AOF_EXPOSURE_SET_GAIN     4u
typedef struct aof_exposure_command {
    uint16_t exposure; uint8_t gain; uint8_t flags;
    float msv_error, msv_error_int;
    uint32_t update;
} aof_exposure_command;

int aof_bank_exposure_reset_device(aof_ctx *ctx, int32_t n_streams, const uint8_t *d_mask, uint16_t exposure0,
                                   uint8_t gain0, const uint16_t *d_exposure0, const uint8_t *d_gain0,
                                   aof_exposure_state *d_state, void *stream);
int aof_bank_exposure_control_device(aof_ctx *ctx, const aof_exposure_control *ec, int32_t n_streams, int32_t n_rounds,
                                     const aof_exposure_record *d_exposure, aof_exposure_state *d_state,
                                     aof_exposure_command *d_commands, void *stream);
int aof_exposure_control_host(const aof_exposure_control *ec, int32_t n_streams, int32_t n_rounds,
                              const aof_exposure_record *records, aof_exposure_state *states,
                              aof_exposure_command *commands);

#define AOF_IMU_SLOTS_MAX 16
#define AOF_TICK_STALE_GYRO (-3)
#define AOF_TICK_NO_OFFSET  (-4)

typedef struct aof_imu_sample {
    uint64_t time_usec; float xgyro, ygyro, zgyro; uint32_t reserved;
} aof_imu_sample;

typedef struct aof_imu_state {
    double gyro_x, gyro_y, gyro_z;
    uint64_t prev_time_usec;
    uint64_t last_taken_time_usec;
    uint64_t offset_timestamp_usec;
    uint32_t messages;
    uint32_t samples_integrated, samples_rejected, dropped;
} aof_imu_state;

typedef struct aof_imu_params {
    int32_t n_streams, n_rounds , max_samples ;
    uint8_t system_id, component_id, first_seq;
} aof_imu_params;

int aof_bank_imu_reset_device(aof_ctx *ctx, int32_t n_streams, const uint8_t *d_mask, uint64_t offset0,
                              aof_imu_state *d_state, void *stream);
int aof_bank_imu_device(aof_ctx *ctx, const aof_imu_params *ip, const aof_imu_sample *d_samples,
                        const uint8_t *d_sample_count, const uint64_t *d_time_us, const aof_tick_record *d_records_in,
// ... 39 lines not shown
```

Before: 7.275 million.

## Accumulate per-wave vote histograms in cols search and reduce strips

Adds a strip-reduction path for the non-subpixel lane8 column search. Each wave accumulates its flow-vote histogram in LDS during the walk and writes a compact per-wave strip, reusing the subdirs workspace region. A small reduce kernel then sums the strips per pair, replacing a reduce that rereads every block record. It is on by default (auto mode) for large batches where fused votes are not used. The cost is extra LDS atomics and ballots inside the search loop.

```diff
diff --git a/aero-optical-flow_amd/__init__.py b/aero-optical-flow_amd/__init__.py
--- a/aero-optical-flow_amd/__init__.py
+++ b/aero-optical-flow_amd/__init__.py
@@ -10,6 +10,7 @@
 
 GRID_DENSE, GRID_PX4FLOW = 0, 1
 SEARCH_EXHAUSTIVE, SEARCH_PRUNED, SEARCH_ADAPTIVE = 0, 1, 2
+REDUCTION_RECORDS, REDUCTION_STRIPS, REDUCTION_IN_LAUNCH = 0, 1, 2
 SAD_SKIPPED = 0xFFFF
 FLAG_FLOW_VALID, FLAG_PRED_VALID = 1, 2
 K_PYRAMID, K_SEARCH_L1, K_REDUCE_L1, K_SEARCH, K_REDUCE = range(5)
@@ -229,6 +230,8 @@
         "aof_set_search_belief": (C.c_int, [VP, C.c_int]),
         "aof_set_split_coarse": (C.c_int, [VP, C.c_int]),
         "aof_set_reduce_fusion": (C.c_int, [VP, C.c_int]),
+        "aof_set_strip_reduction": (C.c_int, [VP, C.c_int]),
+        "aof_get_last_reduction": (C.c_int, [VP]),
         "aof_flow_batch_device": (C.c_int, [VP, VP, VP, I64, I64, VP, VP, VP, VP, C.c_size_t, VP]),
         "aof_flow_pair_host": (C.c_int, [VP, VP, VP, VP, VP, VP]),
         "aof_stream_push_host": (C.c_int, [VP, VP, VP]),
@@ -791,6 +794,14 @@
             return
         self._check(lib.aof_set_reduce_fusion(self._ctx, int(on)))
 
+    def set_strip_reduction(self, mode=-1):
+        if not hasattr(lib, "aof_set_strip_reduction"):
+            return
+        self._check(lib.aof_set_strip_reduction(self._ctx, int(mode)))
+
+    def last_reduction(self) -> int:
+        return self._check(lib.aof_get_last_reduction(self._ctx))
+
     def set_profiling(self, on=True, kernels=None):
         if on and kernels is not None:
             mask = 0
diff --git a/aero-optical-flow_amd/csrc/aof_batch.cpp b/aero-optical-flow_amd/csrc/aof_batch.cpp
--- a/aero-optical-flow_amd/csrc/aof_batch.cpp
+++ b/aero-optical-flow_amd/csrc/aof_batch.cpp
@@ -25,6 +25,7 @@
     aof_block *blocks1; uint8_t *subdirs1; aof_flow *flows1; uint8_t *hist1;
     aof_block *blocks0; uint8_t *subdirs0; aof_flow *flows; uint8_t *hist0;
     uint32_t *hints;
+    uint16_t *strips0;
 };
 
 enum SearchKind { SK_TILE16, SK_LANE8_GROUP, SK_LANE8, SK_GENERIC };
@@ -35,6 +36,7 @@
     bool refine;
     SearchArgs a;
     FlowTail tail;
+    uint16_t *strips;
 };
 
 struct BatchPlan {
@@ -67,6 +69,7 @@
     v.blocks0 = d_blocks ? d_blocks : reinterpret_cast<aof_block *>(ws + L.l0_blocks);
     v.subdirs0 = nullptr;
     if (p.subpixel) v.subdirs0 = d_subdirs ? d_subdirs : ws + L.l0_subdirs;
+    v.strips0 = p.subpixel ? nullptr : reinterpret_cast<uint16_t *>(ws + L.l0_subdirs);
     v.flows = d_flows;
     v.hist0 = ws + L.l0_hist;
     v.hints = p.tile == 16 ? reinterpret_cast<uint32_t *>(ws + L.hints) : nullptr;
@@ -122,7 +125,7 @@
 LevelPlan plan_level(const aof_ctx *ctx, SearchArgs a, const FlowTail &tail)
 {
     const SearchKind kind = search_kind(ctx, &a);
-    return {kind, kind == SK_TILE16 && a.subpixel && !tile16_refines(a), a, tail};
+    return {kind, kind == SK_TILE16 && a.subpixel && !tile16_refines(a), a, tail, nullptr};
 }
 
 BatchPlan plan_batch(const aof_ctx *ctx, const BatchView &v, int64_t n, bool k1_ready)
@@ -139,6 +142,7 @@
     a0.pred = sm.t0.pred;
     a0.hints = v.hints;
     P.level[0] = plan_level(ctx, a0, sm.t0);
+    P.level[0].strips = v.strips0;
 
     P.small_class = !ctx->force_generic && !ctx->split_coarse && P.level[0].kind == SK_LANE8_GROUP &&
                     (!two || plan_level(ctx, sm.l1, sm.t1).kind == SK_LANE8_GROUP) && flow_small_supported(sm);
@@ -209,14 +213,15 @@
     int prune;
     bool cols;
     bool fused;
+    bool strips;
     PruneReport rep;
 };
 
 VoteMem vote_mem(const aof_ctx *ctx) { return {ctx->votes.mem, kVoteStride, ctx->h_fault, ctx->votes.deadline_ticks}; }
 
-Lane8Launch choose_lane8(aof_ctx *ctx, const SearchArgs &a, Capture cap)
-{
-    Lane8Launch l = {a.prune, false, false, {nullptr, 0, 1, 0}};
+Lane8Launch choose_lane8(aof_ctx *ctx, const SearchArgs &a, Capture cap, bool strips_region)
+{
+    Lane8Launch l = {a.prune, false, false, false, {nullptr, 0, 1, 0}};
     if (l.prune && ctx->search_mode == AOF_SEARCH_ADAPTIVE) {
         AdaptiveSearch &st = ctx->adapt;
         if (!adaptive_lane8_prunes(st, a)) {
@@ -237,16 +242,18 @@
     const bool fits = l.cols ? lane8_cols_votes_supported(x, vm, ctx->votes.pairs)
                              : (!l.prune && lane8_votes_supported(x, vm, ctx->votes.pairs));
     l.fused = fits && !ctx->votes.separate && (cap == CAPTURE_ACTIVE || (cap == CAPTURE_NONE && !ctx->votes.captured));
+    l.strips = l.cols && !l.fused && strips_region && ctx->strip_mode != 0 && lane8_cols_strips_fit(x) &&
+               (ctx->strip_mode > 0 || lane8_chunks(x) >= kStripMinChunks);
     return l;
 }
 
-int launch_lane8(aof_ctx *ctx, SearchArgs a, const FlowTail &tail, hipStream_t s, bool *reduced)
+int launch_lane8(aof_ctx *ctx, SearchArgs a, const FlowTail &tail, uint16_t *strips, hipStream_t s, bool *reduced, StripReduceArgs *sr)
 {
     hipStreamCaptureStatus status = hipStreamCaptureStatusNone;
     const Capture cap = hipStreamIsCapturing(s, &status) != hipSuccess ? CAPTURE_UNKNOWN
                         : status == hipStreamCaptureStatusNone         ? CAPTURE_NONE
                                                                        : CAPTURE_ACTIVE;
-    Lane8Launch l = choose_lane8(ctx, a, cap);
+    Lane8Launch l = choose_lane8(ctx, a, cap, strips != nullptr);
     a.prune = l.prune;
     const bool eager = cap == CAPTURE_NONE;
     if (l.fused && eager && ctx->votes.used && ctx->votes.stream != s && hipStreamWaitEvent(s, ctx->votes.done, 0) != hipSuccess)
@@ -255,7 +262,8 @@
     const FlowTail *t = l.fused ? &tail : nullptr;
     const VoteMem *m = l.fused ? &vm : nullptr;
     PruneReport *rep = l.prune ? &l.rep : nullptr;
-    int rc = l.cols ? launch_search_lane8_cols(a, s, rep, t, m) : launch_search_lane8(a, s, t, m, rep);
+    int rc = l.cols ? launch_search_lane8_cols(a, s, rep, t, m, l.strips ? strips : nullptr, l.strips ? sr : nullptr)
+                    : launch_search_lane8(a, s, t, m, rep);
     if (!rc && l.fused && eager) {
         rc = (int)hipEventRecord(ctx->votes.done, s);
         ctx->votes.stream = s;
@@ -272,6 +280,7 @@
 int enqueue_level(aof_ctx *ctx, const LevelPlan &l, uint8_t *hist, int kid_search, int kid_reduce, hipStream_t s)
 {
     bool reduced = l.kind == SK_LANE8_GROUP;
+    StripReduceArgs sr = {};
     {
         Timed t(ctx, kid_search, s);
         int rc;
@@ -284,7 +293,7 @@
             rc = launch_flow_lane8(l.a, l.tail, s);
             break;
         case SK_LANE8:
-            rc = launch_lane8(ctx, l.a, l.tail, s, &reduced);
+            rc = launch_lane8(ctx, l.a, l.tail, l.strips, s, &reduced, &sr);
             if (rc < 0) return rc;
             break;
         default:
@@ -292,7 +301,15 @@
         }
         if (rc) return fail(ctx, -EIO, "search launch: %s", hipGetErrorString((hipError_t)rc));
     }
+    if (kid_reduce == AOF_K_REDUCE) ctx->last_reduction = reduced ? AOF_REDUCTION_IN_LAUNCH : sr.strips ? AOF_REDUCTION_STRIPS : AOF_REDUCTION_RECORDS;
     if (reduced) return 0;
+    if (sr.strips) {
+        sr.tail = l.tail;
+        Timed t(ctx, kid_reduce, s);
+        const int rc = launch_reduce_strips(sr, s);
+        if (rc) return fail(ctx, -EIO, "reduce launch: %s", hipGetErrorString((hipError_t)rc));
+        return 0;
+    }
     const ReduceArgs r = {l.a.blocks, l.a.subdirs, value_threshold_u16(ctx->params), l.tail, l.a.n_pairs, nullptr, 0,
                           reinterpret_cast<uint32_t *>(hist)};
     Timed t(ctx, kid_reduce, s);
@@ -329,6 +346,7 @@
     if (P.small) {
         Timed t(ctx, AOF_K_SEARCH, s);
         if ((rc = launch_flow_small(P.sm, s))) return fail(ctx, -EIO, "small-pair launch: %s", hipGetErrorString((hipError_t)rc));
+        ctx->last_reduction = AOF_REDUCTION_IN_LAUNCH;
         return 0;
     }
     if (P.coarse == COARSE_FUSED) {
diff --git a/aero-optical-flow_amd/csrc/aof_capi.hip b/aero-optical-flow_amd/csrc/aof_capi.hip
--- a/aero-optical-flow_amd/csrc/aof_capi.hip
+++ b/aero-optical-flow_amd/csrc/aof_capi.hip
@@ -139,6 +139,7 @@
     ctx->votes.deadline_ticks = kVoteDeadlineTicks;
     ctx->res.stop_wait_s = 1.0;
     ctx->votes.separate = true;
+    ctx->strip_mode = -1;
     ctx->search_mode = AOF_SEARCH_ADAPTIVE;
     ctx->adapt.belief = -1;
     ctx->adapt.stats.belief = -1;
@@ -231,6 +232,16 @@
     return 0;
 }
 
+int aof_set_strip_reduction(aof_ctx *ctx, int mode)
+{
+    if (!ctx || mode < -1 || mode > 1) return -EINVAL;
+    kernel_choice_changes(ctx, mode != ctx->strip_mode);
+    ctx->strip_mode = mode;
+    return 0;
+}
+
+int aof_get_last_reduction(const aof_ctx *ctx) { return ctx ? ctx->last_reduction : -EINVAL; }
+
 int aof_set_reduce_fusion(aof_ctx *ctx, int on)
 {
     if (!ctx) return -EINVAL;
diff --git a/aero-optical-flow_amd/csrc/aof_cols8_kernels.hpp b/aero-optical-flow_amd/csrc/aof_cols8_kernels.hpp
--- a/aero-optical-flow_amd/csrc/aof_cols8_kernels.hpp
+++ b/aero-optical-flow_amd/csrc/aof_cols8_kernels.hpp
@@ -13,9 +13,11 @@
 
 namespace {
 
-template <bool SUBPIXEL, bool VOTE>
-__device__ __forceinline__ void cols_walk(const SearchArgs &a, const ColsPlan &plan, const PruneReport &report, const VoteMem *votes)
+template <bool SUBPIXEL, bool VOTE, bool STRIPS = false>
+__device__ __forceinline__ void cols_walk(const SearchArgs &a, const ColsPlan &plan, const PruneReport &report, const VoteMem *votes,
+                                          const ColsStrips *strips = nullptr)
 {
+    static_assert(!STRIPS || (!SUBPIXEL && !VOTE), "the strips are the non-subpixel walk's, in place of the vote memory");
     const uint32_t wg = blockIdx.x;
     const uint32_t unit0 = wg * blockDim.x + threadIdx.x;
     const bool in_tail = (uint32_t)__builtin_amdgcn_readfirstlane((int)unit0) >= plan.head_units;
@@ -93,6 +95,11 @@
     int seen = 0, paying = 0;
     std::conditional_t<VOTE && !SUBPIXEL, WalkVotes, NoWalkVotes> pending;
     pending.init();
+    std::conditional_t<STRIPS, StripVotes, NoWalkVotes> strip;
+    if constexpr (STRIPS) {
+        __shared__ uint32_t s_rows[kColsThreads / 64][128];
+        strip.init(s_rows[threadIdx.x >> 6]);
+    }
     for (int step = 0; step < sg.len; step++) {
         const int by = by0 + step;
         const bool act = live && by < a.grid.ny;
@@ -196,10 +203,19 @@
             if constexpr (SUBPIXEL) vote_and_arrive(*votes, a.hist_range, pair, act, ok, 2 * rec.dx + hx + centre, 2 * rec.dy + hy + centre);
             else pending.step(*votes, a.hist_range, pair, act, ok, 2 * rec.dx + hx + centre, 2 * rec.dy + hy + centre);
         }
+        if constexpr (STRIPS) {
+            const int centre = 2 * a.hist_range + 1;
+            strip.step(2 * centre + 1, act && (uint32_t)rec.sad < (uint32_t)a.value_threshold, 2 * rec.dx + centre, 2 * rec.dy + centre);
+        }
 #pragma unroll
         for (int s = 0; s < 8; s++) win[s] = win[s + 8];
     }
     if constexpr (VOTE) pending.flush(*votes, a.hist_range, pair);
+    if constexpr (STRIPS) {
+        const int n = 2 * (2 * a.hist_range + 1) + 1;
+        const uint32_t wave = (uint32_t)__builtin_amdgcn_readfirstlane((int)local) >> 6;
+        strip.store(n, strips->base + ((size_t)pair * strips->per_pair + wave) * (size_t)(2 * n));
+    }
     if (report.slots && threadIdx.x == 0 && wg % report.stride == 0)
         __hip_atomic_store(report.slots + wg / report.stride, (report.launch_no << 16) | ((uint32_t)paying << 8) | (uint32_t)seen,
                            __ATOMIC_RELAXED, __HIP_MEMORY_SCOPE_SYSTEM);
diff --git a/aero-optical-flow_amd/csrc/aof_cols8_plan.hpp b/aero-optical-flow_amd/csrc/aof_cols8_plan.hpp
--- a/aero-optical-flow_amd/csrc/aof_cols8_plan.hpp
+++ b/aero-optical-flow_amd/csrc/aof_cols8_plan.hpp
@@ -22,7 +22,10 @@
     FlowTail tail;
     VoteMem votes;
 };
-
+struct ColsStrips {
+    uint16_t *base;
+    uint32_t per_pair;
+};
 
 constexpr int kColsThreads = 256;
 constexpr int kColsMaxRows = 8, kColsMinRows = 2;
@@ -71,4 +74,24 @@
     return l;
 }
 
+constexpr int kStripMaxBins = 62;
+struct ColsStripsPlan {
+    uint32_t head_waves, tail_waves, per_pair;
+    uint32_t head_pairs;
+    uint32_t row;
+    bool fits;
+};
+inline ColsStripsPlan cols_strips_plan(const ColsLaunch &l, const Grid &g, int hist_range, int64_t n_pairs)
+{
+    ColsStripsPlan s;
+    const int n = 2 * (2 * hist_range + 1) + 1;
+    s.head_waves = l.plan.head.units_per_pair / 64;
+    s.tail_waves = l.plan.tail.units_per_pair / 64;
+    s.per_pair = s.head_waves > s.tail_waves ? s.head_waves : s.tail_waves;
+    s.head_pairs = l.plan.head_pairs;
+    s.row = (uint32_t)(2 * n);
+    s.fits = n <= kStripMaxBins && l.pairs == n_pairs && (int64_t)s.per_pair * s.row * 2 <= (int64_t)g.blocks();
+    return s;
 }
+
+}
diff --git a/aero-optical-flow_amd/csrc/aof_ctx.hpp b/aero-optical-flow_amd/csrc/aof_ctx.hpp
--- a/aero-optical-flow_amd/csrc/aof_ctx.hpp
+++ b/aero-optical-flow_amd/csrc/aof_ctx.hpp
@@ -110,6 +110,8 @@
     int search_mode;
     bool force_generic;
     bool split_coarse;
+    int strip_mode;
+    int last_reduction;
     int bank_path;
     const aof_bank_stream *bank_streams;
     int32_t bank_streams_n;
diff --git a/aero-optical-flow_amd/csrc/aof_internal.hpp b/aero-optical-flow_amd/csrc/aof_internal.hpp
--- a/aero-optical-flow_amd/csrc/aof_internal.hpp
+++ b/aero-optical-flow_amd/csrc/aof_internal.hpp
@@ -148,8 +148,18 @@
 int64_t lane8_chunks(const SearchArgs &a);
 bool lane8_cols_supported(const SearchArgs &a);
 bool lane8_cols_votes_supported(const SearchArgs &a, const VoteMem &votes, int64_t capacity_pairs);
+struct StripReduceArgs {
+    const uint16_t *strips;
+    uint32_t per_pair;
+    uint32_t head_pairs;
+    uint32_t head_waves, tail_waves;
+    FlowTail tail;
+    int64_t n_pairs;
+};
+bool lane8_cols_strips_fit(const SearchArgs &a);
 int launch_search_lane8_cols(const SearchArgs &a, void *stream, PruneReport *report = nullptr, const FlowTail *tail = nullptr,
-                             const VoteMem *votes = nullptr);
+                             const VoteMem *votes = nullptr, uint16_t *strips = nullptr, StripReduceArgs *reduce = nullptr);
+constexpr int64_t kStripMinChunks = 8192;
 constexpr int64_t kPruneMinChunks = 2048;
 int lane8_group(const SearchArgs &a);
 int launch_flow_lane8(const SearchArgs &a, const FlowTail &tail, void *stream);
@@ -344,6 +354,7 @@
 int flow_sequence(aof_ctx *ctx, const uint8_t *d_frames, int64_t n_pairs, aof_flow *d_flows, void *d_workspace,
                   size_t workspace_bytes, void *stream, bool k1_ready);
 int launch_reduce(const ReduceArgs &a, void *stream);
+int launch_reduce_strips(const StripReduceArgs &a, void *stream);
 int launch_derotate(const aof_derotate_params &p, const aof_flow *flows, const aof_gyro *gyro,
                     int64_t n, float *out, void *stream);
 struct IngestSensors {
diff --git a/aero-optical-flow_amd/csrc/aof_lane8_launch.hpp b/aero-optical-flow_amd/csrc/aof_lane8_launch.hpp
--- a/aero-optical-flow_amd/csrc/aof_lane8_launch.hpp
+++ b/aero-optical-flow_amd/csrc/aof_lane8_launch.hpp
@@ -8,6 +8,7 @@
 
 struct ColsPlan;
 struct ColsVotes;
+struct ColsStrips;
 
 int launch_k_search_lane8_ff(const SearchArgs &a, uint32_t items, uint32_t wgs, int threads, void *stream);
 int launch_k_search_lane8_ft(const SearchArgs &a, uint32_t items, uint32_t wgs, int threads, void *stream);
@@ -25,5 +26,7 @@
 int launch_k_search_lane8_cols_t(const SearchArgs &a, const ColsPlan &plan, const PruneReport &rep, uint32_t wgs, int threads, void *stream);
 int launch_k_flow_lane8_cols_f(const SearchArgs &a, const ColsPlan &plan, const PruneReport &rep, const ColsVotes &cv, uint32_t grid, int threads, void *stream);
 int launch_k_flow_lane8_cols_t(const SearchArgs &a, const ColsPlan &plan, const PruneReport &rep, const ColsVotes &cv, uint32_t grid, int threads, void *stream);
+int launch_k_search_lane8_cols_strips(const SearchArgs &a, const ColsPlan &plan, const PruneReport &rep, const ColsStrips &strips, uint32_t wgs,
+                                      int threads, void *stream);
 
 }
diff --git a/aero-optical-flow_amd/csrc/aof_reduce.hpp b/aero-optical-flow_amd/csrc/aof_reduce.hpp
--- a/aero-optical-flow_amd/csrc/aof_reduce.hpp
+++ b/aero-optical-flow_amd/csrc/aof_reduce.hpp
@@ -270,6 +270,55 @@
     }
 };
 
+struct StripVotes {
+    int key;
+    uint32_t votes;
+    uint32_t *row;
+
+    __device__ __forceinline__ void init(uint32_t *lds_row)
+    {
+        key = 0; votes = 0; row = lds_row;
+        const int lane = (int)(threadIdx.x & 63);
+        row[lane] = 0; row[lane + 64] = 0;
+        __builtin_amdgcn_wave_barrier();
+    }
+
+    __device__ __forceinline__ void flush(int n)
+    {
+        if (votes == 0) return;
+        if ((threadIdx.x & 63) == 0) {
+            atomicAdd(&row[key & 0xFF], votes);
+            atomicAdd(&row[n + (key >> 8)], votes);
+        }
+        votes = 0;
+    }
+
+    __device__ __forceinline__ void step(int n, bool ok, int bin_x, int bin_y)
+    {
+        const unsigned long long voters = __ballot(ok);
+        if (voters == 0) return;
+        const int mine = bin_x | (bin_y << 8);
+        const int k = __builtin_amdgcn_readlane(mine, __ffsll((long long)voters) - 1);
+        if ((__ballot(ok && mine == k) & voters) == voters) {
+            if (votes != 0 && key != k) flush(n);
+            key = k;
+            votes = (uint32_t)__builtin_amdgcn_readfirstlane((int)(votes + (uint32_t)__popcll(voters)));
+            return;
+        }
+        flush(n);
+        wave_vote2(row, row + n, bin_x, bin_y, ok);
+    }
+
+    __device__ __forceinline__ void store(int n, uint16_t *strip)
+    {
+        flush(n);
+        __builtin_amdgcn_wave_barrier();
+        const int lane = (int)(threadIdx.x & 63);
+        if (lane < 2 * n) strip[lane] = (uint16_t)row[lane];
+        if (lane + 64 < 2 * n) strip[lane + 64] = (uint16_t)row[lane + 64];
+    }
+};
+
 __device__ __forceinline__ void await_votes_and_finalise(const VoteMem &vm, const FlowTail &tail, uint32_t pair)
 {
     const uint64_t deadline_ticks = vm.deadline_ticks;
diff --git a/aero-optical-flow_amd/csrc/k_reduce.hip b/aero-optical-flow_amd/csrc/k_reduce.hip
--- a/aero-optical-flow_amd/csrc/k_reduce.hip
+++ b/aero-optical-flow_amd/csrc/k_reduce.hip
@@ -167,6 +167,44 @@
     for (int k = tid; k < 2 * n; k += kThreads) out[k] = k < n ? hist[0][k] : hist[1][k - n];
 }
 
+__global__ __launch_bounds__(kThreads) void k_reduce_strips(StripReduceArgs a)
+{
+    const int64_t pair = (int64_t)blockIdx.x * (kThreads / 64) + (int)(threadIdx.x >> 6);
+    if (pair >= a.n_pairs) return;
+    const int centre = 2 * a.tail.range + 1, n = 2 * centre + 1, lane = (int)(threadIdx.x & 63);
+    const int rows = (int)(pair < (int64_t)a.head_pairs ? a.head_waves : a.tail_waves);
+    const uint16_t *strip = a.strips + (size_t)pair * a.per_pair * (size_t)(2 * n);
+    uint32_t hx = 0, hy = 0;
+    if (lane < n) {
+        constexpr int kBatch = 8;
+        for (int r0 = 0; r0 < rows; r0 += kBatch) {
+            uint32_t vx[kBatch], vy[kBatch];
+#pragma unroll
+            for (int k = 0; k < kBatch; k++) {
+                const bool in = r0 + k < rows;
+                vx[k] = in ? strip[(size_t)(r0 + k) * (2 * n) + lane] : 0u;
+                vy[k] = in ? strip[(size_t)(r0 + k) * (2 * n) + n + lane] : 0u;
+            }
+#pragma unroll
+            for (int k = 0; k < kBatch; k++) { hx += vx[k]; hy += vy[k]; }
+        }
+    }
+    const int total = (int)wave_sum_u32(hx);
+    const int sum2x = (int)wave_sum_u32((uint32_t)((lane - centre) * (int)hx));
+    const int sum2y = (int)wave_sum_u32((uint32_t)((lane - centre) * (int)hy));
+    finalise_flow_wave_bins(a.tail, pair, hx, hy, sum2x, sum2y, total);
+}
+
+}
+
+int launch_reduce_strips(const StripReduceArgs &a, void *stream)
+{
+    if (a.n_pairs == 0) return 0;
+    const int n = 2 * (2 * a.tail.range + 1) + 1;
+    if (a.n_pairs > 0x7FFFFFFF || n > 62 || !a.strips) return (int)hipErrorInvalidValue;
+    hipLaunchKernelGGL(k_reduce_strips, dim3((uint32_t)((a.n_pairs + kThreads / 64 - 1) / (kThreads / 64))), dim3(kThreads), 0,
+                       static_cast<hipStream_t>(stream), a);
+    return (int)hipGetLastError();
 }
 
 int launch_reduce(const ReduceArgs &a, void *stream)
diff --git a/aero-optical-flow_amd/csrc/k_search_cols8.hip b/aero-optical-flow_amd/csrc/k_search_cols8.hip
--- a/aero-optical-flow_amd/csrc/k_search_cols8.hip
+++ b/aero-optical-flow_amd/csrc/k_search_cols8.hip
@@ -18,7 +18,15 @@
     return a.n_pairs <= capacity_pairs;
 }
 
-int launch_search_lane8_cols(const SearchArgs &a, void *stream, PruneReport *report, const FlowTail *tail, const VoteMem *votes)
+bool lane8_cols_strips_fit(const SearchArgs &a)
+{
+    if (!lane8_cols_supported(a) || a.subpixel || a.n_pairs < 1) return false;
+    const ColsLaunch l = cols_plan_make(a.grid, a.w, a.h, a.pair_stride, reinterpret_cast<uintptr_t>(a.cur), a.n_pairs);
+    return cols_strips_plan(l, a.grid, a.hist_range, a.n_pairs).fits;
+}
+
+int launch_search_lane8_cols(const SearchArgs &a, void *stream, PruneReport *report, const FlowTail *tail, const VoteMem *votes,
+                             uint16_t *strips, StripReduceArgs *reduce)
 {
     if (report) report->expected = 0;
     if (a.n_pairs == 0) return 0;
@@ -45,7 +53,18 @@
             report->expected = (uint32_t)((wgs + rep.stride - 1) / rep.stride);
         }
         int rc;
-        if (tail && votes) {
+        if (strips) {
+            const ColsStripsPlan sp = cols_strips_plan(l, a.grid, a.hist_range, a.n_pairs);
+            if (!sp.fits || a.subpixel || tail || votes || !reduce) return (int)hipErrorInvalidValue;
+            reduce->strips = strips;
+            reduce->per_pair = sp.per_pair;
+            reduce->head_pairs = sp.head_pairs;
+            reduce->head_waves = sp.head_waves;
+            reduce->tail_waves = sp.tail_waves;
+            reduce->n_pairs = a.n_pairs;
+            const ColsStrips cs = {strips, sp.per_pair};
+            rc = launch_k_search_lane8_cols_strips(s, plan, rep, cs, (uint32_t)wgs, threads, stream);
+        } else if (tail && votes) {
             if (done != 0 || s.n_pairs != a.n_pairs) return (int)hipErrorInvalidValue;
             ColsVotes cv;
             cv.search_wgs = (uint32_t)wgs;
diff --git a/aero-optical-flow_amd/csrc/k_search_cols8_strips.hip b/aero-optical-flow_amd/csrc/k_search_cols8_strips.hip
--- /dev/null
+++ b/aero-optical-flow_amd/csrc/k_search_cols8_strips.hip
@@ -0,0 +1,22 @@
+#include "aof_cols8_kernels.hpp"
+#include "aof_lane8_launch.hpp"
+
+namespace aof {
+
+namespace {
+
+__global__ __launch_bounds__(kColsThreads, 4) void k_search_lane8_cols_strips(SearchArgs a, ColsPlan plan, PruneReport report, ColsStrips strips)
+{
+    cols_walk<false, false, true>(a, plan, report, nullptr, &strips);
+}
+
+}
+
+int launch_k_search_lane8_cols_strips(const SearchArgs &a, const ColsPlan &plan, const PruneReport &rep, const ColsStrips &strips, uint32_t wgs,
+                                      int threads, void *stream)
+{
+    hipLaunchKernelGGL(k_search_lane8_cols_strips, dim3(wgs), dim3(threads), 0, static_cast<hipStream_t>(stream), a, plan, rep, strips);
+    return (int)hipGetLastError();
+}
+
+}
diff --git a/include/aof.h b/include/aof.h
--- a/include/aof.h
+++ b/include/aof.h
@@ -112,6 +112,11 @@
 int aof_set_split_coarse(aof_ctx *ctx, int on);
 
 int aof_set_reduce_fusion(aof_ctx *ctx, int on);
+int aof_set_strip_reduction(aof_ctx *ctx, int mode);
+#define AOF_REDUCTION_RECORDS 0
+#define AOF_REDUCTION_STRIPS 1
+#define AOF_REDUCTION_IN_LAUNCH 2
+int aof_get_last_reduction(const aof_ctx *ctx);
 int aof_set_vote_deadline_us(aof_ctx *ctx, uint32_t microseconds);
 int aof_debug_vote_deadline_ticks(aof_ctx *ctx, uint32_t ticks);
 int aof_debug_tile16_verdicts(aof_ctx *ctx, const uint8_t *verdicts, int count);
```

Result: faster. 7.448 million, median of 6 (+2.4%).
